# jizongFox/Self-paced-Contrastive-Learning

Hardware: AMD Instinct MI355X
Metric: pretrain slices/sec/node (UNet+InfoNCE, 224^2, bs=32/GPU) (higher is better)
Workload: dtype bf16; 1 GPU; BASELINE.json configs[1]: self-paced pretrain step, UNet base (max_channel=256) encoder to Conv5 + ProjectionHead(256,256,256) + SelfPacedSupConLoss(soft, partition labels, correct_grad) fwd+bwd + RAdam; slices_per_gpu=32, images_per_gpu_step=64, image=1x224x224, global_batch=32, parallelism=dp1, params=1311056, hipgraph=epocher, capture_steps=3

## Files before the change

include/spcl_hip.h:

```cpp
#ifndef SPCL_HIP_H
#define SPCL_HIP_H
#include <stddef.h>
#include <stdint.h>
#ifdef __cplusplus
extern "C" {
#endif

#define SPCL_F32 0
#define SPCL_BF16 1

#define SPCL_OK 0
#define SPCL_EINVAL (-1)
#define SPCL_ELAUNCH (-2)
#define SPCL_EUNSUPPORTED (-3)

#define SPCL_ABI_VERSION 24
int spcl_abi_version(void);
const char* spcl_last_error(void);

size_t spcl_supcon_workspace_bytes(int n, int d);
int spcl_supcon_forward(const float* z1, const float* z2, const float* labels, const float* mask, int n, int d,
                        float temperature, int sp_mode, float gamma, int correct_grad, float* ws, float* out,
                        void* stream);
int spcl_supcon_backward(const float* labels, const float* mask, int n, int d, float temperature, int sp_mode,
                         float gamma, const float* ws_fwd, float* ws_bwd, const float* out_fwd,
                         const float* grad_out, float* dz1, float* dz2, void* stream);
size_t spcl_supcon_bwd_workspace_bytes(int n, int d);
int spcl_supcon_unit_gradient_block(int n, int d, size_t* offset_floats, int* row_pitch);
int spcl_supcon_forward_heads(int K, const float* z1, const float* z2, size_t z_stride, const float* labels, int n,
                              int d, float temperature, int sp_mode, const float* gammas, int correct_grad, float* ws,
                              size_t ws_stride, float* out, void* stream);
int spcl_supcon_rows_supported(int n, int d);
int spcl_supcon_forward_rows(int K, const float* o1, const float* o2, size_t o_stride, const float* labels, int n, int d,
                             float temperature, int sp_mode, const float* gammas, int correct_grad, float* ws,
                             size_t ws_stride, float* out, void* stream);
int spcl_supcon_backward_heads(int K, const float* labels, int n, int d, float temperature, int sp_mode,
                               const float* gammas, const float* ws_fwd, size_t ws_stride, float* ws_bwd,
                               size_t wsb_stride, const float* out_fwd, const float* grad_out, float* dz1, float* dz2,
                               size_t z_stride, void* stream);
int spcl_supcon_materialize(const float* labels, const float* mask, int n, int d, float temperature, int sp_mode,
                            float gamma, const float* ws_fwd, float* sim_logits, float* sim_exp, float* pos_mask,
                            float* neg_mask, float* sp_mask, void* stream);

size_t spcl_supcon_xpos_workspace_bytes(int n, int d);
int spcl_supcon_xpos_forward(const float* z1, const float* z2, const float* labels, const float* mask, int n, int d,
                             float temperature, float* ws, float* out, void* stream);
int spcl_supcon_xpos_backward(const float* z1, const float* z2, int n, int d, float temperature, const float* ws,
                              const float* grad_out, float* dz1, float* dz2, void* stream);

size_t spcl_supcon_weighted_workspace_bytes(int n, int d);
int spcl_supcon_weighted_forward(const float* z1, const float* z2, const float* labels, const float* w11,
                                 const float* w22, const float* w12, int blocks, int mask_semantics, int in_mode, int n,
                                 int d, float temperature, float* ws, float* out, void* stream);
int spcl_supcon_weighted_backward(const float* z1, const float* z2, int n, int d, float temperature, float* ws,
                                  const float* grad_out, float* dz1, float* dz2, void* stream);
int spcl_supcon_weighted_materialize(const float* z1, const float* z2, const float* labels, const float* w11,
                                     const float* w22, const float* w12, int blocks, int mask_semantics, int n, int d,
                                     float temperature, float* ws, float* sim_logits, float* sim_exp, float* pos_weight,
                                     float* enable_mask, void* stream);

int spcl_proj_forward(const void* feat, int dtype, int N, int HW, int C, int Cs, const float* w1, const float* b1,
                      const float* w2, const float* b2, int hid, int out_dim, int normalize, float* pooled,
                      float* pre, float* o, float* z, void* stream);
int spcl_proj_backward(const float* dz, int dtype, int N, int HW, int C, int Cs, const float* w1, const float* w2,
                       int hid, int out_dim, int normalize, const float* pooled, const float* pre, const float* o,
                       float* dw1, float* db1, float* dw2, float* db2, float* scratch ,
                       void* dfeat, void* stream);

int spcl_proj_heads_forward(int K, const void* feat, int dtype, int N, int HW, int C, int Cs, const float* const* w1 ,
                            const float* const* b1 , const float* const* w2 , const float* const* b2 ,
                            int hid, int out_dim, int normalize, float* pooled, float* const* pre ,
                            float* const* o , float* const* z , void* stream);
int spcl_proj_heads_backward(int K, const float* const* dz , int dtype, int N, int HW, int C, int Cs,
                             const float* const* w1 , const float* const* w2 , int hid, int out_dim,
                             int normalize, const float* pooled, const float* const* pre ,
                             const float* const* o , float* const* dw1 , float* const* db1 ,
                             float* const* dw2 , float* const* db2 , float* scratch, void* dfeat, void* stream);
int spcl_proj_heads_backward_pooled(int K, const float* const* dz, int dtype, int N, int HW, int C, int Cs,
                                    const float* const* w1, const float* const* w2, int hid, int out_dim, int normalize,
                                    const float* pooled, const float* const* pre, const float* const* o, float* const* dw1,
                                    float* const* db1, float* const* dw2, float* const* db2, float* scratch, void* dfeat_nc,
                                    void* stream);


size_t spcl_conv_packed_elems(int Cin, int Cout, int kind, int dtype);
int spcl_conv_pack_weights(const float* w_oihw, int Cin, int Cout, int kind, int dtype, void* packed, void* stream);
int spcl_conv_pack_weights_both(const float* w_oihw, int Cin, int Cout, int dtype, void* packed_fwd,
                                void* packed_dgrad, void* stream);

int spcl_conv_pack_weights_block(const float* wa_oihw, int CinA, int CoutA, void* a_fwd, void* a_dgrad,
                                 const float* wb_oihw, int CinB, int CoutB, void* b_fwd, void* b_dgrad, int dtype,
                                 void* stream);
int spcl_conv_pack_weights_block_at(const float* wa_oihw, int CinA, int CoutA, void* a_fwd, void* a_dgrad,
                                    const float* wb_oihw, int CinB, int CoutB, void* b_fwd, void* b_dgrad, int dtype,
                                    int H, int W, void* stream);

#define SPCL_PACK_MULTI_MAX 24
typedef struct spcl_pack_item {
  const float* w_oihw;
// ... 72 lines not shown
size_t spcl_conv_wgrad_batched_workspace_bytes(const spcl_wgrad_item* items, int n);
int spcl_conv3x3_wgrad_batched(const spcl_wgrad_item* items, int n, int accumulate, float* partial, void* stream);

#define SPCL_WGRAD_TAILS_MAX 16
typedef struct spcl_wgrad_tail {
  const float* partial;
  float* dw;
  int kind;
  int nsplit, nblk_ci, nblk_co, CIB, COB, Cin, Cout;
} spcl_wgrad_tail;
int spcl_wgrad_tail_capture(spcl_wgrad_tail* slot);
int spcl_conv3x3_wgrad_batched_tails(const spcl_wgrad_item* items, int n, const spcl_wgrad_tail* tails, int ntails,
                                     int accumulate, float* partial, void* stream);
int spcl_bn_finalize(float* stats, int ntiles, int C, int CS, const float* gamma, const float* beta,
                     float momentum, float eps, float* running_mean, float* running_var,
                     int64_t* num_batches_tracked, float* mean, float* invstd, float* scale, float* shift,
                     void* stream);
int spcl_bn_eval_affine(int C, int CS, const float* gamma, const float* beta, const float* running_mean,
                        const float* running_var, float eps, float* mean, float* invstd, float* scale, float* shift,
                        void* stream);
#define SPCL_BN_EVAL_MAX 32
typedef struct {
  const float* gamma;
  const float* beta;
  const float* running_mean;
  const float* running_var;
  float* st;
  int C, CS;
  float eps;
} spcl_bn_eval_item;
int spcl_bn_eval_affine_multi(const spcl_bn_eval_item* items, int n, void* stream);

int spcl_bnrelu_pool_forward(const void* y, int dtype, int N, int H, int W, int CS, const float* scale,
                             const float* shift, void* act_out, void* pool_out, void* stream);
size_t spcl_bnrelu_bwd_workspace_bytes(int N, int H, int W, int CS);
int spcl_bnrelu_pool_backward(const void* y, const void* dact, const void* dpool, int dtype, int N, int H, int W,
                              int C, int CS, const float* mean, const float* invstd, const float* scale,
                              const float* shift, int training, float* ws, float* dgamma, float* dbeta, void* dy,
                              void* stream);
int spcl_bnrelu_up2_forward(const void* y, int dtype, int N, int H, int W, int CS, const float* scale, const float* shift,
                            void* up_out, void* stream);
int spcl_bnrelu_pool_forward_strided(const void* y, int dtype, int N, int H, int W, int CS, const float* scale,
                                     const float* shift, void* act_out, int act_stride, void* pool_out, void* stream);
int spcl_bnrelu_pool_backward_strided(const void* y, const void* dact, int dact_stride, const void* dpool, int dtype, int N,
                                      int H, int W, int C, int CS, const float* mean, const float* invstd,
                                      const float* scale, const float* shift, int training, float* ws, float* dgamma,
                                      float* dbeta, void* dy, void* stream);
int spcl_bnrelu_backward_up2(const void* y, const void* d_up, void* dact, int dtype, int N, int H, int W, int C, int CS,
                             const float* mean, const float* invstd, const float* scale, const float* shift, int training,
                             float* ws, float* dgamma, float* dbeta, void* dy, void* stream);
int spcl_bnrelu_backward_bcast(const void* y, const void* dact_nc, int dtype, int N, int H, int W, int C, int CS,
                               const float* mean, const float* invstd, const float* scale, const float* shift, int training,
                               float* ws, float* dgamma, float* dbeta, void* dy, void* stream);

size_t spcl_bnrelu_image_wgrad_workspace_bytes(int N, int H, int W, int CS);
int spcl_bnrelu_backward_image_wgrad(const void* y, const void* dact, const float* image, int dtype, int N, int H,
                                     int W, int C, int CS, const float* mean, const float* invstd, const float* scale,
                                     const float* shift, int training, float* ws, float* dgamma, float* dbeta,
                                     float* dw, void* stream);

int spcl_conv_dgrad_bnstats_supported(int dtype, int N, int H, int W, int CinK, int CoutS);
int spcl_conv3x3_dgrad_bnstats(const void* dy, int dtype, int N, int H, int W, int CinK, int CoutS, const void* w_packed,
                               void* g, const void* y2, const float* scale2, const float* shift2, const float* mean2,
                               float* rows2, void* stream);

int spcl_image_autocorr_rows(int N, int H, int W);
int spcl_image_autocorr(const float* image, int N, int H, int W, float* out, void* stream);
int spcl_conv_dgrad_bnstats_image_supported(int dtype, int N, int H, int W, int CinK, int CoutS);
int spcl_conv3x3_dgrad_bnstats_image(const void* dy, int dtype, int N, int H, int W, int CinK, int CoutS,
                                     const void* w_packed, void* g, const void* y2, const float* scale2,
                                     const float* shift2, const float* mean2, const float* image, float* rows11,
                                     void* stream);
int spcl_conv16_bwd_fused_supported(int dtype, int N, int H, int W, int CinK, int CoutS);
int spcl_conv16_bwd_fused_splits(int N, int H, int W);
int spcl_conv16_bwd_fused(const void* dy, int dtype, int N, int H, int W, const void* w_packed_dgrad, const void* y2,
                          const float* scale2, const float* shift2, const float* mean2, const float* image,
                          float* rows11, float* partial, float* dw_oihw, int Cin, int Cout, float* wg_rows,
                          const float* acorr, int nacorr, float* acorr16, void* stream);
int spcl_conv16_bwd_fused_image_supported(int dtype, int N, int H, int W, int CinK, int CoutS);
int spcl_conv16_bwd_fused_image(const void* dy, int dtype, int N, int H, int W, const void* w_packed_dgrad,
                                const void* w_packed_image, const float* scale2, const float* shift2, const float* mean2,
                                const float* image, float* rows11, float* partial, float* dw_oihw, int Cin, int Cout,
                                float* wg_rows, const float* acorr, int nacorr, float* acorr16, void* stream);
int spcl_bnrelu_backward_wgrows_image3(const float* wg_rows, int nwg, const float* acorr, int nacorr, const float* w_oihw,
                                       int N, int H, int W, int C, int CS, const float* mean, const float* invstd,
                                       const float* scale, int training, float* ws, float* dgamma, float* dbeta,
                                       float* dw, void* stream);
size_t spcl_bnrelu_image3_workspace_bytes(int CS);
int spcl_bnrelu_backward_rows_image3(const float* rows11, int nrows, const float* acorr, int nacorr, const float* w_oihw,
                                     int N, int H, int W, int C, int CS, const float* mean, const float* invstd,
                                     const float* scale, int training, float* ws, float* dgamma, float* dbeta, float* dw,
                                     void* stream);

int spcl_conv_dgrad_poolstats_supported(int dtype, int N, int H, int W, int CinK, int CoutS, int H2, int W2);
int spcl_conv3x3_dgrad_poolstats(const void* dy, int dtype, int N, int H, int W, int CinK, int CoutS, const void* w_packed,
                                 void* g, const void* y2, int H2, int W2, const float* scale2, const float* shift2,
                                 const float* mean2, float* rows2, void* stream);
int spcl_bnrelu_pool_backward_rows(const void* y, const void* dpool, const float* rows, int nrows, int dtype, int N, int H,
                                   int W, int C, int CS, const float* mean, const float* invstd, const float* scale,
                                   const float* shift, int training, float* ws, float* dgamma, float* dbeta, void* dy,
                                   void* stream);
int spcl_bnrelu_backward_rows(const void* y, const void* dact, const float* image, const float* rows, int nrows, int dtype,
                              int N, int H, int W, int C, int CS, const float* mean, const float* invstd,
                              const float* scale, const float* shift, int training, float* ws, float* dgamma,
                              float* dbeta, void* dy, float* dw, void* stream);


int spcl_conv1x1_forward(const void* x, int dtype, size_t npix, int C, int CS, int K, const float* w, const float* b,
                         float* out, void* stream);
size_t spcl_conv1x1_bwd_workspace_bytes(int C, int K);
int spcl_conv1x1_backward(const void* x, const float* dout, int dtype, size_t npix, int C, int CS, int K, const float* w,
                          void* dx, float* dw, float* db, float* ws, void* stream);
int spcl_conv1x1_forward_bn(const void* y, int dtype, size_t npix, int C, int CS, int K, const float* scale,
                            const float* shift, const float* w, const float* b, float* out, void* stream);
int spcl_conv1x1_bwd_rows(size_t npix);
int spcl_conv1x1_backward_bn(const void* y, const float* dout, int dtype, size_t npix, int C, int CS, int K,
                             const float* scale, const float* shift, const float* mean, const float* w, void* dact,
                             float* dw, float* db, float* ws, float* rows, void* stream);
int spcl_softmax_forward(const float* logits, size_t npix, int K, float* prob, void* stream);
int spcl_softmax_backward(const float* prob, const float* dprob, size_t npix, int K, float* dlogits, void* stream);
size_t spcl_kl_workspace_bytes(void);
int spcl_kl_div_forward(const float* prob, const float* target, size_t npix, int K, float eps, float* ws, float* loss,
                        void* stream);
int spcl_kl_div_backward(const float* prob, const float* target, size_t npix, int K, float eps, const float* grad_loss,
                         float* dprob, void* stream);
int spcl_sup_loss_forward(const float* logits, const int64_t* labels, int B, int per_sample, int K, float eps, float* ws,
                          float* loss, float* dlogits_unit, int64_t* inter_zeroed, int64_t* union_zeroed, void* stream);
int spcl_one_hot(const int64_t* labels, size_t npix, int K, float* out, void* stream);
int spcl_argmax_classes(const float* logits, size_t npix, int K, int64_t* out, void* stream);
int spcl_dice_counts(const int64_t* pred, const int64_t* target, int B, int per_sample, int C, int64_t* inter_zeroed,
                     int64_t* union_zeroed, void* stream);

size_t spcl_surface_workspace_bytes(int B, int H, int W, int n_report);
int spcl_surface_distances(const int64_t* pred, const int64_t* target, int B, int H, int W, int C, const int* report,
                           int n_report, double sy, double sx, double percentile, double* hd, double* mhd, double* asd,
                           uint8_t* empty, void* ws, size_t ws_bytes, void* stream);

size_t spcl_surface_3d_workspace_bytes(int V, int D, int H, int W, int n_report);
int spcl_surface_distances_3d(const int64_t* pred, const int64_t* target, int V, int D, int H, int W, int C, const int* report,
                              int n_report, double sz, double sy, double sx, double percentile, double* hd, double* mhd,
                              double* asd, uint8_t* empty, void* ws, size_t ws_bytes, void* stream);

int spcl_upsample2x_forward(const void* x, void* y, int dtype, int N, int H, int W, int CS, void* stream);
int spcl_upsample2x_backward(const void* dy, void* dx, int dtype, int N, int H, int W, int CS, void* stream);
int spcl_concat2_channels(const void* a, const void* b, void* out, int elem_size, size_t npix, int CA, int CB,
                          void* stream);
int spcl_split2_channels(const void* in, void* a, void* b, int elem_size, size_t npix, int CA, int CB, void* stream);

int spcl_radam_step(float* param, const float* grad, float* exp_avg, float* exp_avg_sq, size_t n, int64_t* step,
                    const float* lr, double beta1, double beta2, double eps, double weight_decay, float* coef,
                    void* stream);
int spcl_radam_step_scalars(float* param, const float* grad, float* exp_avg, float* exp_avg_sq, size_t n, int64_t* step,
                            const float* lr, double beta1, double beta2, double eps, double weight_decay, float* coef,
                            int k, const void* const* src, void* const* dst, const float* count, void* stream);
int spcl_radam_step_scaled(float* param, const float* grad, double grad_scale, float* exp_avg, float* exp_avg_sq, size_t n,
                           int64_t* step, const float* lr, double beta1, double beta2, double eps, double weight_decay,
                           float* coef, int k, const void* const* src, void* const* dst, const float* count, void* stream);
int spcl_radam_apply_staged(float* param, const float* grad, double grad_scale, float* exp_avg, float* exp_avg_sq, size_t n,
                            int64_t* step, const float* coef, double beta1, double beta2, double eps, double weight_decay,
                            int k, const void* const* src, void* const* dst, const float* count, void* stream);

int spcl_adam_step_scaled(float* param, const float* grad, double grad_scale, float* exp_avg, float* exp_avg_sq, size_t n,
                          int64_t* step, const float* lr, double beta1, double beta2, double eps, double weight_decay,
                          int decoupled, float* coef, int k, const void* const* src, void* const* dst, const float* count,
                          void* stream);
int spcl_adam_apply_staged(float* param, const float* grad, double grad_scale, float* exp_avg, float* exp_avg_sq, size_t n,
// ... 184 lines not shown
```

self-paced-contrastive-learning_amd/csrc/bn.hip:

```cpp
#include <mutex>
#include <type_traits>
#include "bn_acc.hpp"
#include "common.hpp"
#include "image_acorr.hpp"

namespace spcl {

typedef __attribute__((ext_vector_type(4))) uint32_t u32x4;
template <typename T> struct Chunk;
template <> struct Chunk<float> { static constexpr int EPC = 4; };
template <> struct Chunk<bf16_t> { static constexpr int EPC = 8; };

template <typename T> __device__ __forceinline__ void unpack(u32x4 raw, float* v);
template <> __device__ __forceinline__ void unpack<float>(u32x4 raw, float* v) {
#pragma unroll
  for (int e = 0; e < 4; ++e) v[e] = __uint_as_float(raw[e]);
}
template <> __device__ __forceinline__ void unpack<bf16_t>(u32x4 raw, float* v) {
#pragma unroll
  for (int e = 0; e < 4; ++e) {
    v[2 * e] = __uint_as_float(raw[e] << 16);
    v[2 * e + 1] = __uint_as_float(raw[e] & 0xffff0000u);
  }
}
template <typename T> __device__ __forceinline__ u32x4 pack(const float* v);
template <> __device__ __forceinline__ u32x4 pack<float>(const float* v) {
  return (u32x4){__float_as_uint(v[0]), __float_as_uint(v[1]), __float_as_uint(v[2]), __float_as_uint(v[3])};
}
template <> __device__ __forceinline__ u32x4 pack<bf16_t>(const float* v) {
  u32x4 o;
#pragma unroll
  for (int e = 0; e < 4; ++e) o[e] = (uint32_t)f32_to_bf16(v[2 * e]) | ((uint32_t)f32_to_bf16(v[2 * e + 1]) << 16);
  return o;
}

constexpr int BN_GROUP_TILES = 256;
constexpr int BN_DIRECT_TILES = 1024;
__host__ __device__ inline int bn_groups(int ntiles) {
  return ntiles <= BN_DIRECT_TILES ? 0 : (ntiles + BN_GROUP_TILES - 1) / BN_GROUP_TILES;
}

struct BnFinalArgs {
  const float* gamma;
  const float* beta;
  float momentum, eps;
  float* running_mean;
  float* running_var;
  int64_t* nbt;
  float* mean;
  float* invstd;
  float* scale;
  float* shift;
};

__device__ __forceinline__ void store_agent(double* p, double v) {
  __hip_atomic_store((unsigned long long*)p, __builtin_bit_cast(unsigned long long, v), __ATOMIC_RELAXED,
                     __HIP_MEMORY_SCOPE_AGENT);
}
__device__ __forceinline__ double load_agent(const double* p) {
  return __builtin_bit_cast(double, __hip_atomic_load((const unsigned long long*)p, __ATOMIC_RELAXED, __HIP_MEMORY_SCOPE_AGENT));
}

struct BnChan { float gamma, beta, rm, rv; };
__device__ __forceinline__ BnChan bn_prefetch_channel(int c, int C, const BnFinalArgs& f) {
  const int cc = c < C ? c : C - 1;
  const float* rm = f.running_mean != nullptr ? f.running_mean : f.gamma;
  const float* rv = f.running_var != nullptr ? f.running_var : f.gamma;
  BnChan ch;
  ch.gamma = f.gamma[cc];
  ch.beta = f.beta[cc];
  ch.rm = rm[cc];
  ch.rv = rv[cc];
  return ch;
}
__device__ __forceinline__ void bn_final_channel(int c, int C, double n, double s1, double s2, const BnFinalArgs& f,
                                                 const BnChan& ch);
__device__ __forceinline__ double shfl_xor_f64(double v, int m) {
  const unsigned long long u = __builtin_bit_cast(unsigned long long, v);
  const unsigned lo = (unsigned)__shfl_xor((int)(unsigned)u, m, 64), hi = (unsigned)__shfl_xor((int)(unsigned)(u >> 32), m, 64);
  return __builtin_bit_cast(double, ((unsigned long long)hi << 32) | lo);
}
template <int CW>
__device__ __forceinline__ void bn_fold_lanes(double& n, double& s1, double& s2, double (*red)[1024 / 64][CW]) {
  static_assert(CW == 16, "four row lanes per wave");
  const int c16 = threadIdx.x % CW, wave = threadIdx.x >> 6, nw = blockDim.x >> 6;
  n += shfl_xor_f64(n, 16); s1 += shfl_xor_f64(s1, 16); s2 += shfl_xor_f64(s2, 16);
  n += shfl_xor_f64(n, 32); s1 += shfl_xor_f64(s1, 32); s2 += shfl_xor_f64(s2, 32);
// ... 52 lines not shown
    if (threadIdx.x == 0) __hip_atomic_store(tickets + blockIdx.x, 0u, __ATOMIC_RELAXED, __HIP_MEMORY_SCOPE_AGENT);
    n = 0.0; s1 = 0.0; s2 = 0.0;
    for (int r = tl; r < (int)gridDim.y; r += TL) {
      const double* p = partial + (size_t)r * 3 * CS + c;
      n += load_agent(p); s1 += load_agent(p + CS); s2 += load_agent(p + 2 * CS);
    }
    __syncthreads();
    bn_fold_lanes<CW>(n, s1, s2, red);
    if (tl == 0) bn_final_channel(c, C, n, s1, s2, f, SPCL_BN_PREFETCH ? ch : bn_prefetch_channel(c, C, f));
    return;
  }
  if (tl != 0) return;
  if (!FINAL) {
    double* q = partial + (size_t)blockIdx.y * 3 * CS + c;
    q[0] = n; q[CS] = s1; q[2 * CS] = s2;
    return;
  }
  bn_final_channel(c, C, n, s1, s2, f, SPCL_BN_PREFETCH ? ch : bn_prefetch_channel(c, C, f));
}

__device__ __forceinline__ void bn_final_channel(int c, int C, double n, double s1, double s2, const BnFinalArgs& f,
                                                 const BnChan& ch) {
  if (c >= C) {
    f.mean[c] = 0.f; f.invstd[c] = 0.f; f.scale[c] = 0.f; f.shift[c] = 0.f;
    return;
  }
  const double mu = s1 / n;
  const double m2 = fmax(s2 - s1 * mu, 0.0);
  const double var = m2 / n;
  const float is = 1.0f / sqrtf((float)var + f.eps);
  const float sc = ch.gamma * is;
  f.mean[c] = (float)mu;
  f.invstd[c] = is;
  f.scale[c] = sc;
  f.shift[c] = ch.beta - (float)mu * sc;
  if (f.running_mean != nullptr) f.running_mean[c] = (1.f - f.momentum) * ch.rm + f.momentum * (float)mu;
  if (f.running_var != nullptr) {
    const double unbiased = n > 1.0 ? m2 / (n - 1.0) : var;
    f.running_var[c] = (1.f - f.momentum) * ch.rv + f.momentum * (float)unbiased;
  }
  if (f.nbt != nullptr && c == 0) f.nbt[0] += 1;
}

__global__ __launch_bounds__(256) void bn_eval_affine_kernel(int C, int CS, const float* __restrict__ gamma,
                                                             const float* __restrict__ beta,
                                                             const float* __restrict__ rm, const float* __restrict__ rv,
                                                             float eps, float* mean, float* invstd, float* scale,
                                                             float* shift) {
  const int c = blockIdx.x * blockDim.x + threadIdx.x;
  if (c >= CS) return;
  if (c >= C) { mean[c] = 0.f; invstd[c] = 0.f; scale[c] = 0.f; shift[c] = 0.f; return; }
  const float is = 1.0f / sqrtf(rv[c] + eps);
  const float sc = gamma[c] * is;
  mean[c] = rm[c];
  invstd[c] = is;
  scale[c] = sc;
  shift[c] = beta[c] - rm[c] * sc;
}

struct BnEvalItems {
  spcl_bn_eval_item it[SPCL_BN_EVAL_MAX];
  int blk_end[SPCL_BN_EVAL_MAX];
};
__global__ __launch_bounds__(256) void bn_eval_affine_multi_kernel(BnEvalItems p, int n) {
  int i = 0;
  for (int k = 0; k < n; ++k) i += (int)blockIdx.x >= p.blk_end[k] ? 1 : 0;
  if (i >= n) return;
  const spcl_bn_eval_item& q = p.it[i];
  const int c = ((int)blockIdx.x - (i > 0 ? p.blk_end[i - 1] : 0)) * 256 + threadIdx.x;
  if (c >= q.CS) return;
  float* mean = q.st;
  float* invstd = q.st + q.CS;
  float* scale = q.st + 2 * q.CS;
  float* shift = q.st + 3 * q.CS;
  if (c >= q.C) { mean[c] = 0.f; invstd[c] = 0.f; scale[c] = 0.f; shift[c] = 0.f; return; }
  const float is = 1.0f / sqrtf(q.running_var[c] + q.eps);
  const float sc = q.gamma[c] * is;
  mean[c] = q.running_mean[c];
  invstd[c] = is;
  scale[c] = sc;
  shift[c] = q.beta[c] - q.running_mean[c] * sc;
}

template <typename T> struct Word;
template <> struct Word<float> {
  static constexpr int EPW = 1;
  static __device__ __forceinline__ float get(uint32_t w, int) { return __uint_as_float(w); }
  static __device__ __forceinline__ uint32_t make(const float* v) { return __float_as_uint(v[0]); }
  static __device__ __forceinline__ uint32_t merge(const uint32_t* s) { return s[0]; }
};
template <> struct Word<bf16_t> {
  static constexpr int EPW = 2;
  static __device__ __forceinline__ float get(uint32_t w, int h) {
    return __uint_as_float(h ? (w & 0xffff0000u) : (w << 16));
  }
  static __device__ __forceinline__ uint32_t make(const float* v) {
    return (uint32_t)f32_to_bf16(v[0]) | ((uint32_t)f32_to_bf16(v[1]) << 16);
  }
  static __device__ __forceinline__ uint32_t merge(const uint32_t* s) { return (s[0] & 0x0000ffffu) | (s[1] & 0xffff0000u); }
};

template <int EPC> __device__ __forceinline__ void load_coef(float* dst, const float* src, int cc) {
#pragma unroll
  for (int e = 0; e < EPC; e += 4) *(f32x4*)&dst[e] = *(const f32x4*)(src + cc * EPC + e);
}

template <int EPC>
__device__ __forceinline__ void acc_coef_fwd(const BnAccFwd& bn, int cc, float* sc, float* sh) {
  __shared__ float cl[2][256];
  const int c = threadIdx.x;
  if (c < bn.CS) {
    BnAccFwdRaw raw;
    raw.load(bn, c);
    float a, b;
    bn_acc_fwd_channel(bn, raw, c, a, b, blockIdx.x == 0);
    cl[0][c] = a;
    cl[1][c] = b;
  }
  __syncthreads();
#pragma unroll
  for (int e = 0; e < EPC; ++e) {
    sc[e] = cl[0][cc * EPC + e];
    sh[e] = cl[1][cc * EPC + e];
  }
}
template <int EPC>
__device__ __forceinline__ void acc_coef_bwd(const BnAccBwd& bw, int cc, float* A, float* B) {
  __shared__ float cl[2][256];
  const int c = threadIdx.x;
  if (c < bw.CS) {
    BnAccBwdRaw raw;
    raw.load(bw, c);
    float a, b;
    bn_acc_bwd_channel(bw, raw, c, a, b, blockIdx.x == 0);
    cl[0][c] = a;
    cl[1][c] = b;
  }
  __syncthreads();
#pragma unroll
  for (int e = 0; e < EPC; ++e) {
    A[e] = cl[0][cc * EPC + e];
    B[e] = cl[1][cc * EPC + e];
  }
}

constexpr int STREAM_UNROLL = 2;
constexpr int IMG_WGRAD_WG = 2048;

template <typename T>
__global__ __launch_bounds__(256, 6) void bnrelu_fwd_lin_kernel(const T* __restrict__ y, size_t npix, int CS,
                                                             const float* __restrict__ scale,
                                                             const float* __restrict__ shift, T* __restrict__ act,
                                                             int AS ,
                                                             BnAccFwd bn = BnAccFwd{}) {
  constexpr int EPC = Chunk<T>::EPC, U = STREAM_UNROLL;
  const int CPC = CS / EPC, PL = 256 / CPC;
  const int cc = threadIdx.x % CPC, pl = threadIdx.x / CPC;
  float sc[EPC], sh[EPC];
  if (bn.acc != nullptr) acc_coef_fwd<EPC>(bn, cc, sc, sh);
  if (pl >= PL) return;
  if (bn.acc == nullptr) {
    load_coef<EPC>(sc, scale, cc);
    load_coef<EPC>(sh, shift, cc);
  }
  const size_t stride = (size_t)gridDim.x * PL;
  for (size_t p = (size_t)blockIdx.x * PL + pl; p < npix; p += U * stride) {
    u32x4 r[U];
#pragma unroll
    for (int u = 0; u < U; ++u)
      if (p + u * stride < npix) r[u] = *(const u32x4*)(y + (p + u * stride) * CS + cc * EPC);
#pragma unroll
    for (int u = 0; u < U; ++u) {
      if (p + u * stride >= npix) break;
      float v[EPC];
      unpack<T>(r[u], v);
#pragma unroll
      for (int e = 0; e < EPC; ++e) v[e] = fmaxf(fmaf(sc[e], v[e], sh[e]), 0.f);
      *(u32x4*)(act + (p + u * stride) * AS + cc * EPC) = pack<T>(v);
    }
  }
}

template <typename T>
// ... 461 lines not shown
    g += (k == best) ? dp : 0.f;
    dz[k] = z[k] > 0.f ? g : 0.f;
  }
}

#ifndef SPCL_BWD_POOL_MAXW
#define SPCL_BWD_POOL_MAXW 0
#endif
#if SPCL_BWD_POOL_MAXW
#define BWD_POOL_WPE __attribute__((amdgpu_waves_per_eu(3, SPCL_BWD_POOL_MAXW)))
#else
#define BWD_POOL_WPE
#endif
template <typename T, bool APPLY, bool FAST, bool ACC = false>
__global__ __launch_bounds__(256, 3) BWD_POOL_WPE void bnrelu_bwd_pool_kernel(const T* __restrict__ y, const T* __restrict__ dact,
                                                              const T* __restrict__ dpool, int N, int H, int W, int CS,
                                                              const float* __restrict__ mean,
                                                              const float* __restrict__ invstd,
                                                              const float* __restrict__ scale,
                                                              const float* __restrict__ shift,
                                                              const float* __restrict__ ab, float* __restrict__ partial,
                                                              T* __restrict__ dy, int GS = 0 ,
                                                              BnAccBwd bw = BnAccBwd{}) {
  constexpr int EPC = Chunk<T>::EPC, EPW = Word<T>::EPW;
  __shared__ float red[APPLY ? 1 : 256][2 * EPC + 1];
  const int CPC = CS / EPC, PL = 256 / CPC;
  const int cc = threadIdx.x % CPC, pl = threadIdx.x / CPC;
  const int PH = (H + 1) / 2, PW = (W + 1) / 2, OH = H / 2, OW = W / 2;
  const bool has_g = !FAST && dact != nullptr;
  float s1[EPC], s2[EPC];
#pragma unroll
  for (int e = 0; e < EPC; ++e) s1[e] = s2[e] = 0.f;
  float c0[EPC], c1[EPC];
  constexpr bool from_acc = APPLY && ACC;
  if (from_acc) acc_coef_bwd<EPC>(bw, cc, c0, c1);
  if (pl < PL) {
    float sc[EPC], sh[EPC];
    load_coef<EPC>(sc, scale, cc);
    load_coef<EPC>(sh, shift, cc);
    if (!from_acc) {
      load_coef<EPC>(c0, APPLY ? ab : mean, cc);
      load_coef<EPC>(c1, APPLY ? ab + CS : invstd, cc);
    }
    const int rows = N * PH;
    for (int r = blockIdx.x; r < rows; r += gridDim.x) {
      const int n = r / PH, oy = r - n * PH;
      const size_t row0 = (size_t)n * H + 2 * oy;
      for (int ox = pl; ox < PW; ox += PL) {
        Window<T> w;
        w.template load<FAST>(y, row0, oy, ox, H, W, CS, cc);
        u32x4 rg[4], rdp = {0u, 0u, 0u, 0u};
        if (has_g) {
          const size_t g00 = (row0 * W + 2 * ox) * GS + cc * EPC;
          const size_t goff[4] = {g00, g00 + GS, g00 + (size_t)W * GS, g00 + (size_t)W * GS + GS};
#pragma unroll
          for (int k = 0; k < 4; ++k) {
            rg[k] = (u32x4){0u, 0u, 0u, 0u};
            if (w.valid[k]) rg[k] = *(const u32x4*)(dact + goff[k]);
          }
        }
        const bool complete = FAST || (dpool != nullptr && oy < OH && ox < OW);
        if (complete) rdp = *(const u32x4*)(dpool + (((size_t)n * OH + oy) * OW + ox) * CS + cc * EPC);
        if (APPLY && FAST) __builtin_amdgcn_sched_barrier(0);
        u32x4 out[4];
#pragma unroll
        for (int wi = 0; wi < 4; ++wi) {
          float o[4][EPW];
#pragma unroll
          for (int h = 0; h < EPW; ++h) {
            const int e = wi * EPW + h;
            if (!APPLY && !has_g) {
              float zb = -1.f, yb = 0.f;
#pragma unroll
              for (int k = 0; k < 4; ++k) {
                const float yv = Word<T>::get(w.ry[k][wi], h);
                pool_first_max(k, w.valid[k] ? fmaf(sc[e], yv, sh[e]) : -1.f, yv, zb, yb);
              }
              const float dzb = (complete && zb > 0.f) ? Word<T>::get(rdp[wi], h) : 0.f;
              s1[e] += dzb;
              s2[e] = fmaf(dzb, yb - c0[e], s2[e]);
              continue;
            }
            if (APPLY && FAST) {
              float yk[4], z[4];
#pragma unroll
              for (int k = 0; k < 4; ++k) {
                yk[k] = Word<T>::get(w.ry[k][wi], h);
                z[k] = fmaf(sc[e], yk[k], sh[e]);
              }
              float m = fmaxf(z[0], 0.f);
              const bool s1 = z[1] > m;
              m = fmaxf(m, z[1]);
              const bool s2 = z[2] > m;
              m = fmaxf(m, z[2]);
              const bool s3 = z[3] > m;
              const bool b[4] = {z[0] > 0.f && !s1 && !s2 && !s3, s1 && !s2 && !s3, s2 && !s3, s3};
              const float dp = Word<T>::get(rdp[wi], h);
#pragma unroll
              for (int k = 0; k < 4; ++k) o[k][h] = fmaf(sc[e], b[k] ? dp : 0.f, fmaf(c0[e], yk[k], c1[e]));
              continue;
            }
            float yk[4], dz[4];
            window_dz<T>(w, rg, has_g, rdp, complete, wi, h, sc[e], sh[e], yk, dz);
#pragma unroll
            for (int k = 0; k < 4; ++k) {
              if (APPLY) o[k][h] = fmaf(sc[e], dz[k], fmaf(c0[e], yk[k], c1[e]));
              else {
                s1[e] += dz[k];
                s2[e] = fmaf(dz[k], yk[k] - c0[e], s2[e]);
              }
            }
          }
          if (APPLY) {
#pragma unroll
            for (int k = 0; k < 4; ++k) out[k][wi] = Word<T>::make(o[k]);
          }
        }
        if (APPLY) {
#pragma unroll
          for (int k = 0; k < 4; ++k)
            if (w.valid[k]) *(u32x4*)(dy + w.off[k]) = out[k];
        }
      }
    }
    if (!APPLY) {
#pragma unroll
      for (int e = 0; e < EPC; ++e) s2[e] *= bw.acc != nullptr ? 1.f : c1[e];
    }
  }
  if (!APPLY) wg_reduce_partials<T, EPC>(s1, s2, CS, CPC, PL, partial, red, const_cast<long long*>(bw.acc));
}

struct Image3Args {
  const float* acorr;
  int nacorr;
  const float* w_oihw;
  float* dw;
};
__device__ __forceinline__ int acorr_index(int a, int b) {
  return a * 9 - a * (a - 1) / 2 + (b - a);
}
__global__ __launch_bounds__(256) void bnrelu_bwd_fin_kernel(const float* __restrict__ partial, int nwg, int C, int CS,
                                                             float M, int training, const float* __restrict__ mean,
                                                             const float* __restrict__ invstd,
                                                             const float* __restrict__ scale,
                                                             float* __restrict__ dgamma, float* __restrict__ dbeta,
                                                             float* __restrict__ ab, float* __restrict__ zero_fill,
                                                             int nzero, int s2_centered, int rs, Image3Args im,
                                                             int transposed = 0) {
  __shared__ float red[11][4];
  __shared__ double racc4[4][64];
  __shared__ double racc[54];
  __shared__ float coef[2];
  const int c = blockIdx.x % CS, grp = blockIdx.x / CS;
  const bool split = gridDim.x == 3u * (unsigned)CS;
  const int t0 = split ? 3 * grp : 0, ntap = split ? 3 : 9;
  if (blockIdx.x == 0)
    for (int z = threadIdx.x; z < nzero; z += 256) zero_fill[z] = 0.f;
  const int lane = threadIdx.x & 63, wave = threadIdx.x >> 6;
  const float c_invstd = invstd[c], c_scale = scale[c], c_mean = mean[c];
  const bool img3 = im.acorr != nullptr;
  __shared__ float wsh[9];
  if (img3 && threadIdx.x < 9 && c < C)
    wsh[threadIdx.x] = bf16_to_f32(f32_to_bf16(im.w_oihw[c * 9 + threadIdx.x]));
  float s1 = 0.f, s2 = 0.f;
  float st[9];
#pragma unroll
  for (int t = 0; t < 9; ++t) st[t] = 0.f;
  auto walk = [&](auto ntap_c) {
    constexpr int NTAP = decltype(ntap_c)::value;
    if (transposed) {
#pragma unroll 4
      for (int w = threadIdx.x; w < nwg; w += 256) {
        s1 += partial[((size_t)0 * CS + c) * nwg + w];
        s2 += partial[((size_t)1 * CS + c) * nwg + w];
#pragma unroll
        for (int t = 0; t < NTAP; ++t) st[t] += partial[((size_t)(2 + t0 + t) * CS + c) * nwg + w];
      }
    } else {
#pragma unroll 4
      for (int w = threadIdx.x; w < nwg; w += 256) {
        s1 += partial[((size_t)w * rs + 0) * CS + c];
// ... 46 lines not shown
    coef[1] = B;
  }
  if (!img3) return;
  __syncthreads();
  __shared__ double wrp[9][9];
  if (threadIdx.x < 81) {
    const int t = threadIdx.x / 9, u = threadIdx.x - 9 * t;
    wrp[t][u] = (double)wsh[u] * racc[u <= t ? acorr_index(u, t) : acorr_index(t, u)];
  }
  __syncthreads();
  if ((int)threadIdx.x >= t0 && (int)threadIdx.x < t0 + ntap && c < C) {
    const int t = threadIdx.x;
    const double S1 = (double)((red[2 + t][0] + red[2 + t][1]) + (red[2 + t][2] + red[2 + t][3]));
    double wr = 0.0;
#pragma unroll
    for (int u = 0; u < 9; ++u) wr += wrp[t][u];
    im.dw[c * 9 + t] = (float)((double)c_scale * S1 + (double)coef[0] * wr + (double)coef[1] * racc[45 + t]);
  }
}

__global__ __launch_bounds__(256) void image_autocorr_kernel(const float* __restrict__ img, int H, int W,
                                                             float* __restrict__ out) {
  image_autocorr_body(img, H, W, out, blockIdx.x);
}

constexpr int ACORR_FOLD = 16;
__global__ __launch_bounds__(256) void bwd_rows_group_kernel(const float* __restrict__ rows, int nrows, int G, int CS,
                                                             float* __restrict__ out, int rs ,
                                                             int nwg = 0x7fffffff,
                                                             const float* __restrict__ acorr_in = nullptr,
                                                             int nacorr = 0, float* __restrict__ acorr_out = nullptr,
                                                             int transposed = 0) {
  if ((int)blockIdx.x >= nwg) {
    const int j = blockIdx.x - nwg, k = threadIdx.x;
    if (k < 64) {
      float s = 0.f;
#pragma unroll 8
      for (int w = j; w < nacorr; w += ACORR_FOLD) s += acorr_in[(size_t)w * 64 + k];
      acorr_out[(size_t)j * 64 + k] = s;
    }
    return;
  }
  const int w = blockIdx.x;
  for (int o = threadIdx.x; o < rs * CS; o += 256) {
    float s = 0.f;
#pragma unroll 8
    for (int k = 0; k < G; ++k) {
      const int r = w * G + k;
      if (r < nrows) s += rows[(size_t)r * rs * CS + o];
    }
    if (transposed) out[(size_t)o * (nwg == 0x7fffffff ? (int)gridDim.x : nwg) + w] = s;
    else out[(size_t)w * rs * CS + o] = s;
  }
}

__global__ __launch_bounds__(256) void bwd_rows_acc_kernel(const float* __restrict__ rows, int nrows, int G, int CS,
                                                           long long* __restrict__ acc) {
  __shared__ float part[256];
  const int w = blockIdx.x, NW4 = 4 * CS;
  const int NP = NW4 >= 256 ? 1 : 256 / NW4;
  for (int o0 = 0; o0 < NW4; o0 += 256) {
    const int o = o0 + (int)(threadIdx.x % (NW4 < 256 ? NW4 : 256)), p = NW4 < 256 ? (int)threadIdx.x / NW4 : 0;
    const int c = o >> 2, which = (o >> 1) & 1, limb = o & 1;
    float s = 0.f;
    if (o < NW4 && p < NP) {
#pragma unroll 8
      for (int k = p; k < G; k += NP) {
        const int r = w * G + k;
        if (r < nrows) s += rows[((size_t)r * 2 + which) * CS + c];
      }
    }
    if (NP > 1) {
      part[threadIdx.x] = s;
      __syncthreads();
      if (p == 0 && o < NW4) {
        for (int q = 1; q < NP; ++q) s += part[q * NW4 + o];
      }
      __syncthreads();
    }
    if (p == 0 && o < NW4) bn_acc_add_word(acc, CS, w & (BN_ACC_REPLICAS - 1), c, which, limb, s);
  }
}

template <typename T>
__global__ __launch_bounds__(256, 6) void bnrelu_bwd_apply_lin_kernel(const T* __restrict__ y, const T* __restrict__ g,
                                                                   size_t npix, int CS,
                                                                   const float* __restrict__ scale,
                                                                   const float* __restrict__ shift,
                                                                   const float* __restrict__ ab, T* __restrict__ dy,
                                                                   int GS, BnAccBwd bw = BnAccBwd{}) {
  constexpr int EPC = Chunk<T>::EPC, EPW = Word<T>::EPW, U = STREAM_UNROLL;
  const int CPC = CS / EPC, PL = 256 / CPC;
  const int cc = threadIdx.x % CPC, pl = threadIdx.x / CPC;
  float sc[EPC], sh[EPC], A[EPC], B[EPC];
  if (bw.acc != nullptr) acc_coef_bwd<EPC>(bw, cc, A, B);
  if (pl >= PL) return;
  load_coef<EPC>(sc, scale, cc);
  load_coef<EPC>(sh, shift, cc);
  if (bw.acc == nullptr) {
    load_coef<EPC>(A, ab, cc);
    load_coef<EPC>(B, ab + CS, cc);
  }
  const size_t stride = (size_t)gridDim.x * PL;
  for (size_t p = (size_t)blockIdx.x * PL + pl; p < npix; p += U * stride) {
    u32x4 ry[U], rg[U];
#pragma unroll
    for (int u = 0; u < U; ++u)
      if (p + u * stride < npix) {
        ry[u] = *(const u32x4*)(y + (p + u * stride) * CS + cc * EPC);
        rg[u] = *(const u32x4*)(g + (p + u * stride) * GS + cc * EPC);
      }
#pragma unroll
    for (int u = 0; u < U; ++u) {
      if (p + u * stride >= npix) break;
      u32x4 out;
#pragma unroll
      for (int wi = 0; wi < 4; ++wi) {
        float o[EPW];
#pragma unroll
        for (int h = 0; h < EPW; ++h) {
          const int e = wi * EPW + h;
          const float yv = Word<T>::get(ry[u][wi], h);
          const float dz = fmaf(sc[e], yv, sh[e]) > 0.f ? Word<T>::get(rg[u][wi], h) : 0.f;
          o[h] = fmaf(sc[e], dz, fmaf(A[e], yv, B[e]));
        }
        out[wi] = Word<T>::make(o);
      }
      *(u32x4*)(dy + (p + u * stride) * CS + cc * EPC) = out;
    }
  }
}

template <typename T> struct Quad;
template <> struct Quad<float> {
  typedef u32x4 raw_t;
  static __device__ __forceinline__ float get(raw_t r, int e) { return __uint_as_float(r[e]); }
};
template <> struct Quad<bf16_t> {
  typedef __attribute__((ext_vector_type(2))) uint32_t raw_t;
  static __device__ __forceinline__ float get(raw_t r, int e) {
    return __uint_as_float((e & 1) ? (r[e >> 1] & 0xffff0000u) : (r[e >> 1] << 16));
  }
};

template <typename T>
__global__ __launch_bounds__(256, 5) void bnrelu_bwd_image_wgrad_kernel(const T* __restrict__ y, const T* __restrict__ g,
                                                                     const float* __restrict__ img, int N, int H,
                                                                     int W, int CS, const float* __restrict__ scale,
                                                                     const float* __restrict__ shift,
                                                                     const float* __restrict__ ab,
                                                                     const float* __restrict__ zrow ,
                                                                     float* __restrict__ wpart ) {
  typedef typename Quad<T>::raw_t raw_t;
  constexpr int U = 2;
  extern __shared__ float redw[];
  const int QPP = CS / 4, PL = 256 / QPP;
  const int q = threadIdx.x % QPP, pl = threadIdx.x / QPP;
  float acc[9][4];
#pragma unroll
  for (int t = 0; t < 9; ++t)
#pragma unroll
    for (int e = 0; e < 4; ++e) acc[t][e] = 0.f;
  float sc[4], sh[4], A[4], B[4];
  load_coef<4>(sc, scale, q);
  load_coef<4>(sh, shift, q);
  load_coef<4>(A, ab, q);
// ... 144 lines not shown
}

enum class BwdWs { Plain, ImageWgrad, Image3 };
struct BwdWsLayout {
  size_t partial = 0, ab, wpart, zrow, afold, total;
  BwdWsLayout(BwdWs kind, int CS, int W = 0) {
    ab = (size_t)BWD_MAX_WG * (kind == BwdWs::Image3 ? 11 : 2) * CS;
    wpart = afold = ab + 2 * (size_t)CS;
    zrow = wpart + (size_t)IMG_WGRAD_WG * 9 * CS;
    total = kind == BwdWs::ImageWgrad ? zrow + (size_t)W : kind == BwdWs::Image3 ? afold + ACORR_FOLD * 64 : wpart;
  }
  size_t bytes() const { return total * sizeof(float); }
};

enum class BnGrad { Full, Pooled, PooledFull, PerImage, Up2 };
enum class BnSums { Reduce, Rows, Filled, Fill };
enum class BnOut { Dy, ImageWgrad };
struct BnBwdArgs {
  const void* y = nullptr;
  int N = 0, H = 0, W = 0, C = 0, CS = 0;
  BnGrad grad = BnGrad::Full;
  const void *dact = nullptr, *dpool = nullptr, *d_up = nullptr;
  int dact_stride = 0;
  BnSums sums = BnSums::Reduce;
  const float* rows = nullptr;
  int nrows = 0, training = 0;
  long long* acc = nullptr;
  float* ws = nullptr;
  const float *mean = nullptr, *invstd = nullptr, *scale = nullptr, *shift = nullptr;
  float *dgamma = nullptr, *dbeta = nullptr;
  BnOut out = BnOut::Dy;
  void* dy = nullptr;
  const float* img = nullptr;
  float* dw = nullptr;
  hipStream_t st = nullptr;

  static BnGrad arrives(const void* dact, const void* dpool) {
    return dpool == nullptr ? BnGrad::Full : dact == nullptr ? BnGrad::Pooled : BnGrad::PooledFull;
  }
  bool pooled() const { return grad == BnGrad::Pooled || grad == BnGrad::PooledFull; }
  bool whole_windows() const { return grad == BnGrad::Pooled && H % 2 == 0 && W % 2 == 0; }
  size_t npix() const { return (size_t)N * H * W; }
  int prows() const { return N * ((H + 1) / 2); }
  int gstride() const { return dact_stride > 0 ? dact_stride : CS; }
  int stream_wg() const { return acc != nullptr ? acc_stream_wg() : STREAM_MAX_WG; }
  double grad_tensors() const { return (grad != BnGrad::Pooled ? 1.0 : 0.0) + (pooled() ? 0.25 : 0.0); }
  BnAccBwd block() const {
    if (acc == nullptr) return BnAccBwd{};
    return BnAccBwd{acc, mean , dgamma, dbeta, (float)npix(), training, C, CS};
  }
};

struct BwdSums {
  const float* fin_src = nullptr;
  int nwg = 0, fin_transposed = 0;
  int bsplit = 1;
};

template <typename T, bool APPLY>
static void bnrelu_bwd_pool_launch(const BnBwdArgs& a, int grid, const float* ab, float* partial, const BnAccBwd& bw) {
  const bool fast = a.whole_windows();
  auto go = [&](auto FAST, auto ACC) {
    SPCL_LAUNCH((bnrelu_bwd_pool_kernel<T, APPLY, decltype(FAST)::value, decltype(ACC)::value>), dim3(grid), dim3(256), 0, a.st,
                (const T*)a.y, (const T*)a.dact, (const T*)a.dpool, a.N, a.H, a.W, a.CS, a.mean, a.invstd, a.scale, a.shift, ab,
                partial, APPLY ? (T*)a.dy : (T*)nullptr, fast ? 0 : a.gstride(), bw);
  };
  if constexpr (APPLY) {
    if (bw.acc != nullptr) return fast ? go(yes, yes) : go(no, yes);
  }
  fast ? go(yes, no) : go(no, no);
}

template <typename T>
static BwdSums bnrelu_bwd_sums(const BnBwdArgs& a, float* partial) {
  constexpr int rs = 2;
  const int PL = 256 / (a.CS / Chunk<T>::EPC);
  const double tb = (double)a.npix() * a.CS * sizeof(T);
  BwdSums s{partial};
  prof_cost(tb + tb * a.grad_tensors(), 0.0);
  if (a.sums == BnSums::Filled) return s;
  if (a.sums == BnSums::Rows) {
    static const int fin_rows = lab_env("SPCL_BWD_FIN_MAX_ROWS", BWD_MAX_WG);
    if (a.acc != nullptr) {
      const int G = (a.nrows + 511) / 512;
      s.nwg = (a.nrows + G - 1) / G;
      SPCL_LAUNCH(bwd_rows_acc_kernel, dim3(s.nwg), dim3(256), 0, a.st, a.rows, a.nrows, G, a.CS, a.acc);
    } else if (a.nrows <= fin_rows) {
      s.fin_src = a.rows;
      s.nwg = a.nrows;
    } else {
      const int G = (a.nrows + BWD_MAX_WG - 1) / BWD_MAX_WG;
      s.nwg = (a.nrows + G - 1) / G;
      SPCL_LAUNCH(bwd_rows_group_kernel, dim3(s.nwg), dim3(256), 0, a.st, a.rows, a.nrows, G, a.CS, partial, rs, s.nwg,
                  (const float*)nullptr, 0, (float*)nullptr, 1);
      s.fin_transposed = 1;
    }
    return s;
  }
  long long* const fill = a.sums == BnSums::Fill ? a.acc : nullptr;
  const int red_wg = fill != nullptr ? a.stream_wg() : BWD_MAX_WG;
  switch (a.grad) {
    case BnGrad::Pooled:
    case BnGrad::PooledFull:
      s.nwg = a.prows() < red_wg ? a.prows() : red_wg;
      bnrelu_bwd_pool_launch<T, false>(a, s.nwg, nullptr, partial, fill != nullptr ? a.block() : BnAccBwd{});
      break;
    case BnGrad::PerImage: {
      static const int env_split = lab_env("SPCL_BCAST_SPLIT_MAX", 4);
      s.bsplit = (a.H * a.W + PL - 1) / PL;
      if (env_split > 0 && s.bsplit > env_split) s.bsplit = env_split;
      while (s.bsplit > 1 && a.N * s.bsplit > BWD_MAX_WG) s.bsplit = (s.bsplit + 1) / 2;
      s.nwg = a.N * s.bsplit;
      prof_cost(tb, 0.0);
      SPCL_LAUNCH((bnrelu_bwd_reduce_bcast_kernel<T>), dim3(s.nwg), dim3(256), 0, a.st, (const T*)a.y, (const T*)a.dact,
                  a.H * a.W, a.CS, s.bsplit, a.mean, a.invstd, a.scale, a.shift, partial, fill);
      break;
    }
    case BnGrad::Up2:
      s.nwg = stream_grid(a.npix(), PL, STREAM_UNROLL, red_wg);
      prof_cost(tb * 6.0, 0.0);
      SPCL_LAUNCH((bnrelu_bwd_reduce_up2_kernel<T>), dim3(s.nwg), dim3(256), 0, a.st, (const T*)a.y, (const T*)a.d_up,
                  (T*)a.dact, a.npix(), a.W, a.CS, a.mean, a.invstd, a.scale, a.shift, partial, fill);
      break;
    case BnGrad::Full:
      s.nwg = stream_grid(a.npix(), PL, STREAM_UNROLL, red_wg);
      SPCL_LAUNCH((bnrelu_bwd_reduce_lin_kernel<T>), dim3(s.nwg), dim3(256), 0, a.st, (const T*)a.y, (const T*)a.dact, a.npix(),
                  a.CS, a.mean, a.invstd, a.scale, a.shift, partial, a.gstride(), fill);
      break;
  }
  return s;
}

static void bnrelu_bwd_finalize(const BnBwdArgs& a, const BwdSums& s, float* ab, float* zrow) {
  if (a.acc != nullptr) return;
  const bool image = a.out == BnOut::ImageWgrad;
  SPCL_LAUNCH(bnrelu_bwd_fin_kernel, dim3(a.CS), dim3(256), 0, a.st, s.fin_src, s.nwg, a.C, a.CS, (float)a.npix(), a.training,
              a.mean, a.invstd, a.scale, a.dgamma, a.dbeta, ab, image ? zrow : (float*)nullptr, image ? a.W : 0,
              a.sums == BnSums::Rows ? 1 : 0, 2, Image3Args{nullptr, 0, nullptr, nullptr}, s.fin_transposed);
}

template <typename T>
static void bnrelu_bwd_apply(const BnBwdArgs& a, const BwdSums& s, const float* ab, float* wpart, const float* zrow) {
  const int PL = 256 / (a.CS / Chunk<T>::EPC);
  const double tb = (double)a.npix() * a.CS * sizeof(T);
  const BnAccBwd bw = a.block();
  prof_cost(2.0 * tb + tb * a.grad_tensors(), 0.0);
  if (a.out == BnOut::ImageWgrad) {
    spcl_wgrad_tail* tail = take_tail_capture();
    static const int want = lab_env("SPCL_IMGWG_WG", 1280);
    const int cap = want < IMG_WGRAD_WG ? (want > 0 ? want : 1) : IMG_WGRAD_WG;
    const int g = a.N * a.H < cap ? a.N * a.H : cap;
    prof_cost(2.0 * tb + (double)a.npix() * 4, 2.0 * 9 * a.npix() * a.C);
    SPCL_LAUNCH((bnrelu_bwd_image_wgrad_kernel<T>), dim3(g), dim3(256), 4 * 9 * a.CS * sizeof(float), a.st, (const T*)a.y,
                (const T*)a.dact, a.img, a.N, a.H, a.W, a.CS, a.scale, a.shift, ab, zrow, wpart);
    if (tail != nullptr) {
      tail->partial = wpart; tail->dw = a.dw; tail->kind = 1; tail->nsplit = g; tail->nblk_ci = tail->nblk_co = 1;
      tail->CIB = 1; tail->COB = a.CS; tail->Cin = 1; tail->Cout = a.C;
    } else {
      SPCL_LAUNCH(image_wgrad_final_kernel, dim3(9), dim3(256), 0, a.st, (const float*)wpart, g, a.C, a.CS, a.dw);
    }
  } else if (a.pooled()) {
    bnrelu_bwd_pool_launch<T, true>(a, a.prows() < a.stream_wg() ? a.prows() : a.stream_wg(), ab, nullptr, bw);
  } else if (a.grad == BnGrad::PerImage) {
    prof_cost(2.0 * tb, 0.0);
    SPCL_LAUNCH((bnrelu_bwd_apply_bcast_kernel<T>), dim3(a.N * s.bsplit), dim3(256), 0, a.st, (const T*)a.y, (const T*)a.dact,
                a.H * a.W, a.CS, s.bsplit, a.scale, a.shift, ab, (T*)a.dy, bw);
  } else {
    SPCL_LAUNCH((bnrelu_bwd_apply_lin_kernel<T>), dim3(stream_grid(a.npix(), PL, STREAM_UNROLL, a.stream_wg())), dim3(256), 0,
                a.st, (const T*)a.y, (const T*)a.dact, a.npix(), a.CS, a.scale, a.shift, ab, (T*)a.dy, a.gstride(), bw);
// ... 443 lines not shown
```

self-paced-contrastive-learning_amd/csrc/bn_acc.hpp:

```cpp
#pragma once
#include "common.hpp"

namespace spcl {

#ifndef SPCL_ACC_REPLICAS
#define SPCL_ACC_REPLICAS 8
#endif
constexpr int BN_ACC_REPLICAS = SPCL_ACC_REPLICAS;
constexpr int BN_ACC_FLAG_WORDS = 4;
constexpr double BN_ACC_HI = 1024.0, BN_ACC_HI_INV = 1.0 / 1024.0;
constexpr double BN_ACC_LO = 1152921504606846976.0 , BN_ACC_LO_INV = 1.0 / 1152921504606846976.0;
constexpr float BN_ACC_MAX = 1099511627776.0f;
#ifndef SPCL_ACC_FWD_TILES
#define SPCL_ACC_FWD_TILES 4096
#endif
constexpr int BN_ACC_MAX_TILES_FWD = SPCL_ACC_FWD_TILES;
constexpr int BN_ACC_MAX_TILES_BWD = 4096;

__host__ __device__ inline size_t bn_acc_words(int CS) { return (size_t)BN_ACC_REPLICAS * CS * 4 + BN_ACC_FLAG_WORDS; }

struct BnAccFwd {
  const long long* acc;
  const float* gamma;
  const float* beta;
  float* running_mean;
  float* running_var;
  long long* nbt;
  float* st;
  float momentum, eps, count;
  int C, CS;
  double inv_count;
};

struct BnAccBwd {
  const long long* acc;
  const float* st;
  float* dgamma;
  float* dbeta;
  float count;
  int training, C, CS;
};

#ifdef __HIPCC__
__device__ __forceinline__ void bn_acc_atomic_add(long long* p, long long v) {
  (void)__hip_atomic_fetch_add(p, v, __ATOMIC_RELAXED, __HIP_MEMORY_SCOPE_AGENT);
}

__device__ __forceinline__ void bn_acc_split(float v, long long& hi, long long& lo, bool& ok) {
  ok = fabsf(v) < BN_ACC_MAX;
  const double d = ok ? (double)v : 0.0;
  const double h = rint(d * BN_ACC_HI);
  const double l = rint(fma(h, -BN_ACC_HI_INV, d) * BN_ACC_LO);
  hi = (long long)h;
  lo = (long long)l;
}

__device__ __forceinline__ void bn_acc_add_row16(long long* acc, int CS, int replica, int cb, int r16, f32x4 s1, f32x4 s2,
                                                 bool active = true) {
  const int q = r16 & 3, which = (r16 >> 2) & 1, limb = r16 >> 3;
  float v = which ? s2[0] : s1[0];
#pragma unroll
  for (int r = 1; r < 4; ++r) v = q == r ? (which ? s2[r] : s1[r]) : v;
  long long hi, lo;
  bool ok;
  bn_acc_split(v, hi, lo, ok);
  if (!active) return;
  long long* row = acc + ((size_t)replica * CS + cb + q) * 4;
  bn_acc_atomic_add(row + which * 2 + limb, limb ? lo : hi);
  if (!ok) bn_acc_atomic_add(acc + (size_t)BN_ACC_REPLICAS * CS * 4, 1);
}

__device__ __forceinline__ void bn_acc_add_word(long long* acc, int CS, int replica, int c, int which, int limb, float v) {
  long long hi, lo;
  bool ok;
  bn_acc_split(v, hi, lo, ok);
  bn_acc_atomic_add(acc + ((size_t)replica * CS + c) * 4 + which * 2 + limb, limb ? lo : hi);
  if (!ok) bn_acc_atomic_add(acc + (size_t)BN_ACC_REPLICAS * CS * 4, 1);
}

typedef __attribute__((ext_vector_type(2))) long long i64x2;
struct BnAccSums {
  long long h1, l1, h2, l2, flag;
  __device__ __forceinline__ void totals(double& t1, double& t2) const {
    t1 = fma((double)l1, BN_ACC_LO_INV, (double)h1 * BN_ACC_HI_INV);
    t2 = fma((double)l2, BN_ACC_LO_INV, (double)h2 * BN_ACC_HI_INV);
    if (flag != 0) t1 = t2 = __builtin_nan("");
  }
};
template <int RPT>
struct BnAccPart {
  i64x2 a[RPT], b[RPT];
  long long flag;
  __device__ __forceinline__ void load(const long long* acc, int CS, int c, int r0) {
#pragma unroll
    for (int r = 0; r < RPT; ++r) {
      const long long* row = acc + ((size_t)(r0 + r) * CS + c) * 4;
      a[r] = *(const i64x2*)row;
      b[r] = *(const i64x2*)(row + 2);
    }
    flag = acc[(size_t)BN_ACC_REPLICAS * CS * 4];
  }
  __device__ __forceinline__ BnAccSums sums() const {
    BnAccSums s{0, 0, 0, 0, flag};
#pragma unroll
    for (int r = 0; r < RPT; ++r) { s.h1 += a[r][0]; s.l1 += a[r][1]; s.h2 += b[r][0]; s.l2 += b[r][1]; }
    return s;
  }
};
typedef BnAccPart<BN_ACC_REPLICAS> BnAccRaw;

struct BnAccFwdParams {
  float g, b, rm, rv;
  __device__ __forceinline__ void load(const BnAccFwd& f, int c) {
    const int cc = c < f.C ? c : f.C - 1;
    g = f.gamma[cc];
    b = f.beta[cc];
    rm = (f.running_mean != nullptr ? f.running_mean : f.gamma)[cc];
    rv = (f.running_var != nullptr ? f.running_var : f.gamma)[cc];
  }
};
__device__ __forceinline__ void bn_acc_fwd_channel(const BnAccFwd& f, const BnAccSums& sums, const BnAccFwdParams& in, int c,
                                                   float& scale, float& shift, bool write) {
  if (c >= f.C) {
    scale = 0.f;
    shift = 0.f;
    if (write) { f.st[c] = 0.f; f.st[f.CS + c] = 0.f; f.st[2 * f.CS + c] = 0.f; f.st[3 * f.CS + c] = 0.f; }
// ... 74 lines not shown
```

self-paced-contrastive-learning_amd/csrc/conv16_bwd.hip:

```cpp
#include <stdio.h>
#include <stdlib.h>
#include <vector>
#include "conv_common.hpp"

namespace spcl {

struct Bwd16Args {
  const unsigned char* dy;
  const u32x4* wp;
  const unsigned char* y2;
  const u32x4* wp_img;
  const float* scale2;
  const float* shift2;
  const float* mean2;
  const float* img;
  float* rows11;
  float* wg_rows;
  int nwg;
  const float* acorr_in;
  int nacorr;
  float* acorr_out;
  float* partial;
  int N, H, W, tilesX, tilesY, ipw, xcd_remap;
  int dbg;
  unsigned long long* stamps;
};

constexpr int B16_TH = 14, B16_TW = 14, B16_HW = 16, B16_RP = 22, B16_PS = 32;
constexpr int B16_DY = 0, B16_DY_BYTES = (B16_TH + 2) * B16_RP * B16_PS;
constexpr int B16_IM = B16_DY_BYTES, B16_IM_BYTES = 1536;
constexpr int B16_XT = B16_IM + B16_IM_BYTES, B16_XT_ROW = 16 * 32, B16_XT_BYTES = B16_TH * B16_XT_ROW;
constexpr int B16_RED = B16_XT + B16_XT_BYTES;
constexpr int B16_ACC = B16_RED + 512;
constexpr int B16_TRASH = B16_ACC + 576;
constexpr int B16_LDS = B16_TRASH + 32;

#ifndef SPCL_CONV16_DBG_BUILD
#define SPCL_CONV16_DBG_BUILD 0
#endif
#define B16_DBG(a) (SPCL_CONV16_DBG_BUILD ? (a).dbg : 0)

__device__ __forceinline__ bf16x8 b16_tr_frag(unsigned addr) {
  const s16x4 lo = __builtin_amdgcn_ds_read_tr16_b64_v4i16((s16x4 __attribute__((address_space(3)))*)(uintptr_t)addr);
  const s16x4 hi =
      __builtin_amdgcn_ds_read_tr16_b64_v4i16((s16x4 __attribute__((address_space(3)))*)(uintptr_t)(addr + 8 * B16_PS));
  return __builtin_shufflevector(lo, hi, 0, 1, 2, 3, 4, 5, 6, 7);
}

__device__ __forceinline__ bf16x8 b16_tr_frag2(unsigned addr_lo, unsigned addr_hi) {
  const s16x4 lo = __builtin_amdgcn_ds_read_tr16_b64_v4i16((s16x4 __attribute__((address_space(3)))*)(uintptr_t)addr_lo);
  const s16x4 hi = __builtin_amdgcn_ds_read_tr16_b64_v4i16((s16x4 __attribute__((address_space(3)))*)(uintptr_t)addr_hi);
  return __builtin_shufflevector(lo, hi, 0, 1, 2, 3, 4, 5, 6, 7);
}

constexpr int b16_wpe(int NW) { return NW == 1 ? 2 : 3; }
template <bool SHIFTED, int NW, bool WGROWS>
__global__ __launch_bounds__(64 * NW) __attribute__((amdgpu_waves_per_eu(b16_wpe(NW)))) void conv16_bwd_kernel(Bwd16Args a) {
  constexpr int TH = B16_TH, TW = B16_TW, HW_ = B16_HW, RP = B16_RP, PS = B16_PS;
  constexpr int NPIX = TH * TW, NSTEPS = 5, NTHR = 64 * NW, ITER = 512 / NTHR, RPI = NTHR / 32;
  constexpr int MW = (13 + NW - 1) / NW, TPW = (9 + NW - 1) / NW;
  constexpr int SPX = (16 * NW) % TW, SPY = (16 * NW) / TW;
  extern __shared__ __attribute__((aligned(16))) unsigned char lds[];
  const unsigned lds_base = (unsigned)(uintptr_t)(unsigned char __attribute__((address_space(3)))*)lds;
  const int t0 = threadIdx.x;
  const int wave = NW == 1 ? 0 : __builtin_amdgcn_readfirstlane(t0 >> 6);
  if (WGROWS && (int)blockIdx.z * (int)(gridDim.x * gridDim.y) >= a.nwg) {
    const int nslice = gridDim.x * gridDim.y;
    if (t0 < 64) {
      for (int j = blockIdx.y * gridDim.x + blockIdx.x; j < 16; j += nslice) {
        float sacc = 0.f;
#pragma unroll 8
        for (int w = j; w < a.nacorr; w += 16) sacc += a.acorr_in[(size_t)w * 64 + t0];
        a.acorr_out[(size_t)j * 64 + t0] = sacc;
      }
    }
    return;
  }

  int tx = blockIdx.x, ty = blockIdx.y;
  {
    const int T = a.tilesX * a.tilesY;
    if (a.xcd_remap && (T & 7) == 0) {
      const int L = ty * a.tilesX + tx;
      const int L2 = (L & 7) * (T >> 3) + (L >> 3);
      ty = L2 / a.tilesX;
      tx = L2 - ty * a.tilesX;
    }
  }
  const int y0 = min(ty * TH, a.H - TH), x0 = min(tx * TW, a.W - TW);
  const int oy = ty * TH - y0, ox = tx * TW - x0;
  const bool interior = y0 > 0 && x0 > 0 && y0 + TH < a.H && x0 + TW < a.W;
  const bool shifted = SHIFTED && (oy | ox) != 0;
  const int rowb = 32;

  u32x4 wall[NSTEPS];
#pragma unroll
  for (int s = 0; s < NSTEPS; ++s) wall[s] = a.wp[s * 64 + (t0 & 63)];
  const f32x4 sc2 = *(const f32x4*)(a.scale2 + 4 * ((t0 & 63) >> 4)), sh2 = *(const f32x4*)(a.shift2 + 4 * ((t0 & 63) >> 4)),
              mu2 = *(const f32x4*)(a.mean2 + 4 * ((t0 & 63) >> 4));
  if (t0 < 4 * TH) *(u32x4*)(lds + B16_XT + (t0 >> 2) * B16_XT_ROW + TW * PS + (t0 & 3) * 16) = (u32x4){0u, 0u, 0u, 0u};
  if (t0 >= NTHR - 64)
    *(u32x4*)(lds + B16_DY + (((t0 & 63) >> 2) * RP + HW_) * PS + (t0 & 3) * 16) = (u32x4){0u, 0u, 0u, 0u};

  if (t0 < 48) {
    const int r = t0 & 15, k = t0 >> 4;
    ((bf16_t*)(lds + B16_IM))[(k == 0 ? 256 + 15 : (k == 1 ? 512 + 14 : 512 + 15)) + r * 16] = 0;
  }
  if (WGROWS)
// ... 245 lines not shown
    {
      int px = px0, py = py0;
#pragma unroll
      for (int j = 0; j < MW; ++j) {
        const bool ok = j < MW - 1 || 16 * (wave + NW * j) + r16 < NPIX;
        if (ok) *(uint2*)(lds + B16_XT + py * B16_XT_ROW + px * PS + g * 8) = dzp[j];
        px += SPX;
        py += SPY;
        if (px >= TW) {
          px -= TW;
          py += 1;
        }
      }
    }
    B16_STAMP(5)
    __syncthreads();
    B16_STAMP(1)
    if (wave == 0 && !(B16_DBG(a) & 8)) {
      const int tap = r16 < 9 ? r16 : 0, tky = tap / 3, tkx = tap - 3 * tky;
      const unsigned char* pb = lds + B16_IM + tkx * 512 + ((g >> 1) + tky) * 32 + (g & 1) * 8;
      f32x4* dp = (f32x4*)(lds + B16_ACC + (r16 * 16 + 4 * g) * 4);
      f32x4 D = (WGROWS && r16 < 9) ? *dp : (f32x4){0.f, 0.f, 0.f, 0.f};
#pragma unroll
      for (int ks = 0; ks < TH / 2; ++ks) {
        const bf16x8 af = b16_tr_frag(tr_x + ks * 2 * B16_XT_ROW);
        const uint2 b0 = *(const uint2*)(pb + ks * 64), b1 = *(const uint2*)(pb + ks * 64 + 16);
        const u32x4 bq = {b0.x, b0.y, b1.x, b1.y};
        D = __builtin_amdgcn_mfma_f32_16x16x32_bf16(af, __builtin_bit_cast(bf16x8, bq), D, 0, 0, 0);
      }
      if (WGROWS) {
        if (r16 < 9) *dp = D;
      } else if (r16 < 9) *(f32x4*)(a.rows11 + ((size_t)tile * 11 + 2 + r16) * 16 + 4 * g) = D;
    }
    B16_STAMP(6)
    if (NW > 1) __syncthreads();
  }

  if (stamp) {
    unsigned long long* o = a.stamps + ((size_t)(blockIdx.z * gridDim.y + blockIdx.y) * gridDim.x + blockIdx.x) * 8;
#pragma unroll
    for (int k = 0; k < 7; ++k) o[k] = tph[k];
  }
  const size_t wg = (size_t)(blockIdx.z * gridDim.y + blockIdx.y) * gridDim.x + blockIdx.x;
  if (WGROWS) {
    __syncthreads();
    for (int i = t0; i < 11 * 16; i += NTHR) {
      float tot;
      if (i < 32) {
        const float* red = (const float*)(lds + B16_RED) + i;
        tot = red[0];
#pragma unroll
        for (int w = 1; w < NW; ++w) tot += red[32 * w];
      } else {
        tot = ((const float*)(lds + B16_ACC))[i - 32];
      }
      a.wg_rows[(size_t)i * a.nwg + wg] = tot;
    }
  }
  float* out = a.partial + wg * (9 * 256);
#pragma unroll
  for (int j = 0; j < TPW; ++j) {
    const int tap = wave + NW * j;
    if (tap < 9) {
#pragma unroll
      for (int r = 0; r < 4; ++r) out[(tap * 16 + 4 * ((t0 & 63) >> 4) + r) * 16 + (t0 & 15)] = wacc[j][r];
    }
  }
}


#ifndef SPCL_CONV16_ROWS_WPE
#define SPCL_CONV16_ROWS_WPE 4
#endif
constexpr int r16_wpe(bool shifted) { return shifted && SPCL_CONV16_ROWS_WPE > 3 ? 3 : SPCL_CONV16_ROWS_WPE; }
constexpr int R16_RP = 18;
constexpr int R16_DY = 0, R16_DY_BYTES = (B16_TH + 2) * R16_RP * B16_PS;
constexpr int R16_IM = R16_DY_BYTES;
constexpr int R16_XT = R16_IM + B16_IM_BYTES;
constexpr int R16_RED = R16_XT + B16_XT_BYTES;
constexpr int R16_ACC = R16_RED + 512;
constexpr int R16_TRASH = R16_ACC + 576;
constexpr int R16_TAB = R16_TRASH + 32;
constexpr int B16_LDS_ROWS = R16_TAB + 128;

template <bool SHIFTED, bool WGROWS, bool RECOMP = false>
__global__ __launch_bounds__(128) __attribute__((amdgpu_waves_per_eu(r16_wpe(SHIFTED)))) void conv16_bwd_rows_kernel(Bwd16Args a) {
  static_assert(!(RECOMP && SHIFTED), "y2 from the image: whole 14 x 14 tiles");
  constexpr int NW = 2;
  constexpr int TH = B16_TH, TW = B16_TW, HW_ = B16_HW, RP = R16_RP, PS = B16_PS;
  constexpr int NSTEPS = 5, NTHR = 64 * NW, ITER = 512 / NTHR, RPI = NTHR / 32;
  constexpr int MW = TH / NW, TPW = (9 + NW - 1) / NW;
  static_assert(TH % NW == 0, "rows are dealt to the waves evenly");
  extern __shared__ __attribute__((aligned(16))) unsigned char lds[];
  const unsigned lds_base = (unsigned)(uintptr_t)(unsigned char __attribute__((address_space(3)))*)lds;
  const int t0 = threadIdx.x;
  const int wave = __builtin_amdgcn_readfirstlane(t0 >> 6);
  if (WGROWS && (int)blockIdx.z * (int)(gridDim.x * gridDim.y) >= a.nwg) {
    const int nslice = gridDim.x * gridDim.y;
    float* fold = (float*)lds;
    const int cq = t0 & 15, rl = t0 >> 4;
    for (int j = blockIdx.y * gridDim.x + blockIdx.x; j < 16; j += nslice) {
      f32x4 sacc = {0.f, 0.f, 0.f, 0.f};
#pragma unroll 16
      for (int w = j + 16 * rl; w < a.nacorr; w += 128) sacc += *(const f32x4*)(a.acorr_in + (size_t)w * 64 + 4 * cq);
      __syncthreads();
      *(f32x4*)(fold + rl * 64 + 4 * cq) = sacc;
      __syncthreads();
      if (t0 < 64) {
        float tot = fold[t0];
#pragma unroll
        for (int r = 1; r < 8; ++r) tot += fold[r * 64 + t0];
        a.acorr_out[(size_t)j * 64 + t0] = tot;
      }
    }
    return;
  }

  int tx = blockIdx.x, ty = blockIdx.y;
  {
    const int T = a.tilesX * a.tilesY;
    if (a.xcd_remap && (T & 7) == 0) {
      const int L = ty * a.tilesX + tx;
      const int L2 = (L & 7) * (T >> 3) + (L >> 3);
      ty = L2 / a.tilesX;
      tx = L2 - ty * a.tilesX;
    }
  }
  const int y0 = min(ty * TH, a.H - TH), x0 = min(tx * TW, a.W - TW);
  const int oy = ty * TH - y0, ox = tx * TW - x0;
  const bool interior = y0 > 0 && x0 > 0 && y0 + TH < a.H && x0 + TW < a.W;
  const bool shifted = SHIFTED && (oy | ox) != 0;

  if (t0 < 4 * TH) *(u32x4*)(lds + R16_XT + (t0 >> 2) * B16_XT_ROW + TW * PS + (t0 & 3) * 16) = (u32x4){0u, 0u, 0u, 0u};
  if (t0 >= NTHR - 64)
    *(u32x4*)(lds + R16_DY + (((t0 & 63) >> 2) * RP + HW_) * PS + (t0 & 3) * 16) = (u32x4){0u, 0u, 0u, 0u};
  if (t0 < 48) {
    const int r = t0 & 15, k = t0 >> 4;
    ((bf16_t*)(lds + R16_IM))[(k == 0 ? 256 + 15 : (k == 1 ? 512 + 14 : 512 + 15)) + r * 16] = 0;
  }
  if (t0 >= 64 && t0 < 64 + 20) {
    const int e = t0 - 64, gq = e / NSTEPS, s = e - gq * NSTEPS;
    int fc = 4 * s + gq;
    if (fc >= 18) fc = 0;
    const int tap = fc >> 1, c = fc & 1, ky = (tap * 11) >> 5, kx = tap - 3 * ky;
    ((unsigned*)(lds + R16_TAB))[gq * 8 + s] = (unsigned)((ky * RP + kx) * PS + c * 16);
  }
  if (WGROWS)
    for (int i = t0; i < (512 + 576) / 4; i += NTHR) ((float*)(lds + R16_RED))[i] = 0.f;
  f32x4 wacc[TPW];
#pragma unroll
  for (int j = 0; j < TPW; ++j) wacc[j] = (f32x4){0.f, 0.f, 0.f, 0.f};

  float imgv[256 / NTHR];
  u32x4 v[ITER];
  uint2 ypre[RECOMP ? 1 : MW];
  constexpr int PPT = 256 / NTHR;
  short wraw[3] = {0, 0, 0};
  if (RECOMP) {
    const int gq = min((t0 & 63) >> 4, 2);
    const bf16_t* wq = (const bf16_t*)a.wp_img;
#pragma unroll
    for (int kx = 0; kx < 3; ++kx) {
      const int tap = 3 * gq + kx;
      wraw[kx] = (short)wq[(size_t)(((tap >> 1) * 64) + (2 * (tap & 1)) * 16 + (t0 & 15)) * 8];
    }
  }
  auto rsrc = [](const void* p) { return __builtin_amdgcn_make_buffer_rsrc((void*)p, 0, 0x7fffffff, 0x00020000); };
  constexpr int OOB = (int)0x80000000u;
  auto issue_img = [&](const int n) {
    int t = t0;
    asm volatile("" : "+v"(t));
    const int hr = (t * PPT) >> 4, hc = (t * PPT) & 15;
    const int gy = y0 - 1 + hr;
    const __amdgpu_buffer_rsrc_t rs = rsrc(a.img + (size_t)n * a.H * a.W);
    const int rowo = (gy < 0 ? 0 : (gy >= a.H ? a.H - 1 : gy)) * a.W;
#pragma unroll
    for (int e = 0; e < PPT; ++e) {
      const int gx = x0 - 1 + hc + e;
      imgv[e] = __builtin_bit_cast(float, __builtin_amdgcn_raw_buffer_load_b32(rs, (rowo + (gx < 0 ? 0 : (gx >= a.W ? a.W - 1 : gx))) * 4, 0, 0));
    }
  };
  auto issue_halo = [&](const int n) {
    int t = t0;
    asm volatile("" : "+v"(t));
    const int ch = t & 1, q0 = t >> 1, hy0 = q0 / HW_, hx0 = q0 % HW_;
    const int voff = (hy0 * a.W + hx0) * 32 + ch * 16;
    const __amdgpu_buffer_rsrc_t rs = rsrc(a.dy + (((long)n * a.H + (y0 - 1)) * a.W + (x0 - 1)) * 32);
#pragma unroll
    for (int k = 0; k < ITER; ++k) {
      bool inb = true;
      if (!interior) {
        const int gy = y0 - 1 + hy0 + RPI * k, gx = x0 - 1 + hx0;
        inb = gy >= 0 && gy < a.H && gx >= 0 && gx < a.W;
      }
      v[k] = __builtin_bit_cast(u32x4, __builtin_amdgcn_raw_buffer_load_b128(rs, inb ? voff : OOB, RPI * k * a.W * 32, 0));
    }
  };
  auto issue_y2 = [&](const int n) {
    int t = t0;
    asm volatile("" : "+v"(t));
    const int r16 = t & 15, g = (t & 63) >> 4;
    const int voff = min(r16, TW - 1) * 32 + g * 8;
    const __amdgpu_buffer_rsrc_t rs = rsrc(a.y2 + (((size_t)n * a.H + y0 + wave) * a.W + x0) * 32);
#pragma unroll
    for (int j = 0; j < MW; ++j)
      ypre[j] = __builtin_bit_cast(uint2, __builtin_amdgcn_raw_buffer_load_b64(rs, voff, NW * j * a.W * 32, 0));
  };
  const __amdgpu_buffer_rsrc_t rs_wp = rsrc(a.wp), rs_sc = rsrc(a.scale2), rs_sh = rsrc(a.shift2), rs_mu = rsrc(a.mean2);

  const bool stamp = SPCL_CONV16_STAMPS_BUILD && a.stamps != nullptr && t0 == 0;
  unsigned long long tph[7] = {0, 0, 0, 0, 0, 0, 0}, tc = 0;
  const int n_first = blockIdx.z * a.ipw;
  if (stamp) tc = __builtin_amdgcn_s_memtime();
  if (n_first < a.N) {
    issue_img(n_first);
    issue_halo(n_first);
    if (!RECOMP) issue_y2(n_first);
  }
  uint2 wfp = {0u, 0u};
  if (RECOMP) {
    const bool real = ((t0 & 63) >> 4) < 3;
    wfp.x = real ? ((uint32_t)(unsigned short)wraw[0] | ((uint32_t)(unsigned short)wraw[1] << 16)) : 0u;
    wfp.y = real ? (uint32_t)(unsigned short)wraw[2] : 0u;
    asm volatile("" : "+v"(wfp.x), "+v"(wfp.y));
  }
  __syncthreads();
  uint2 dzp[MW];
  auto second_half = [&](const int n) {
    int t = t0;
    asm volatile("" : "+v"(t));
    const int lane = t & 63, r16 = t & 15, g = lane >> 4;
    const int tile = (n * a.tilesY + ty) * a.tilesX + tx;
    const unsigned xaddr = (unsigned)(R16_XT + wave * B16_XT_ROW + r16 * PS + (((g + (r16 >> 2)) & 3) << 3));
    B16_STAMP(3)
    __syncthreads();
    B16_STAMP(1)
    if (!WGROWS && t < 32) {
      const float* red = (const float*)(lds + R16_RED) + t;
      float tot = red[0];
#pragma unroll
      for (int w = 1; w < NW; ++w) tot += red[32 * w];
      a.rows11[(size_t)tile * 11 * 16 + t] = tot;
    }

    const unsigned tr_col = (unsigned)((4 * (g & 1) + (r16 >> 2)) * PS + (r16 & 3) * 8);
    const unsigned tr_x = lds_base + R16_XT + (g >> 1) * B16_XT_ROW + (4 * (g & 1) + (r16 >> 2)) * PS + ((((r16 & 3) + (g & 1)) & 3) << 3);
    const unsigned tr_xh = (tr_x + 8 * PS) ^ 16u;
    {
      unsigned ad[TPW];
#pragma unroll
      for (int j = 0; j < TPW; ++j) {
        const int tap = min(wave + NW * j, 8), ky = tap / 3, kx = tap - 3 * ky;
        ad[j] = lds_base + R16_DY + (g >> 1) * RP * PS + tr_col + (2 - ky) * RP * PS + (2 - kx) * PS;
      }
#pragma unroll
      for (int ks = 0; ks < TH / 2; ++ks) {
        const bf16x8 af = b16_tr_frag2(tr_x + ks * 2 * B16_XT_ROW, tr_xh + ks * 2 * B16_XT_ROW);
#pragma unroll
        for (int j = 0; j < TPW; ++j) {
          const bf16x8 bf = b16_tr_frag(ad[j] + ks * 2 * RP * PS);
          wacc[j] = __builtin_amdgcn_mfma_f32_16x16x32_bf16(af, bf, wacc[j], 0, 0, 0);
        }
        __builtin_amdgcn_sched_barrier(0);
      }
    }
    B16_STAMP(4)
    __syncthreads();
    B16_STAMP(1)

#pragma unroll
    for (int j = 0; j < MW; ++j) *(uint2*)(lds + xaddr + j * (NW * B16_XT_ROW)) = dzp[j];
    B16_STAMP(5)
    __syncthreads();
    B16_STAMP(1)
    if (wave == 0) {
      const int tap = r16 < 9 ? r16 : 0, tky = tap / 3, tkx = tap - 3 * tky;
      const unsigned char* pb = lds + R16_IM + tkx * 512 + ((g >> 1) + tky) * 32 + (g & 1) * 8;
      f32x4* dp = (f32x4*)(lds + R16_ACC + (r16 * 16 + 4 * g) * 4);
      f32x4 D = (WGROWS && r16 < 9) ? *dp : (f32x4){0.f, 0.f, 0.f, 0.f};
#pragma unroll
      for (int ks = 0; ks < TH / 2; ++ks) {
        const bf16x8 af = b16_tr_frag2(tr_x + ks * 2 * B16_XT_ROW, tr_xh + ks * 2 * B16_XT_ROW);
        const uint2 b0 = *(const uint2*)(pb + ks * 64), b1 = *(const uint2*)(pb + ks * 64 + 16);
        const u32x4 bq = {b0.x, b0.y, b1.x, b1.y};
        D = __builtin_amdgcn_mfma_f32_16x16x32_bf16(af, __builtin_bit_cast(bf16x8, bq), D, 0, 0, 0);
      }
      if (WGROWS) {
        if (r16 < 9) *dp = D;
      } else if (r16 < 9) *(f32x4*)(a.rows11 + ((size_t)tile * 11 + 2 + r16) * 16 + 4 * g) = D;
    }
    B16_STAMP(6)
    __syncthreads();
  };
  int n = n_first;
  if (n_first < a.N)
#pragma unroll 1
  for (int it = 0;; ++it, ++n) {
    int t = t0;
    asm volatile("" : "+v"(t));
    const int lane = t & 63, r16 = t & 15, g = lane >> 4;
    u32x4 wall[NSTEPS];
#pragma unroll
    for (int s = 0; s < NSTEPS; ++s)
      wall[s] = __builtin_bit_cast(u32x4, __builtin_amdgcn_raw_buffer_load_b128(rs_wp, lane * 16, s * 1024, 0));
    f32x4 sc2 = __builtin_bit_cast(f32x4, __builtin_amdgcn_raw_buffer_load_b128(rs_sc, g * 16, 0, 0));
    f32x4 sh2 = __builtin_bit_cast(f32x4, __builtin_amdgcn_raw_buffer_load_b128(rs_sh, g * 16, 0, 0));
    const f32x4 mu2 = __builtin_bit_cast(f32x4, __builtin_amdgcn_raw_buffer_load_b128(rs_mu, g * 16, 0, 0));
    if (r16 >= TW || (SHIFTED && r16 < ox)) {
      sc2 = (f32x4){0.f, 0.f, 0.f, 0.f};
      sh2 = (f32x4){-1.f, -1.f, -1.f, -1.f};
    }
    const u32x4 tabA = *(const u32x4*)(lds + R16_TAB + g * 32);
    const unsigned tabB = *(const unsigned*)(lds + R16_TAB + g * 32 + 16);
    {
      const int hr = (t * PPT) >> 4, hc = (t * PPT) & 15;
      const int gy = y0 - 1 + hr;
#pragma unroll
      for (int e = 0; e < PPT; ++e) {
        const int gx = x0 - 1 + hc + e;
        const float hv = (interior || (gy >= 0 && gy < a.H && gx >= 0 && gx < a.W)) ? imgv[e] : 0.f;
        const bf16_t hb = f32_to_bf16(hv);
        bf16_t* imb = (bf16_t*)(lds + R16_IM) + hr * 16 + hc + e;
        imb[0] = hb;
        if (hc + e >= 1) imb[256 - 1] = hb;
        if (hc + e >= 2) imb[512 - 2] = hb;
      }
    }
    {
      const int ch = t & 1, q0 = t >> 1, hy0 = q0 / HW_, hx0 = q0 % HW_;
      unsigned char* const lp = lds + R16_DY + (hy0 * RP + hx0) * PS + ch * 16;
#pragma unroll
      for (int k = 0; k < ITER; ++k) *(u32x4*)(lp + (RPI * k * RP) * PS) = v[k];
    }
    B16_STAMP(0)
    __syncthreads();
    B16_STAMP(1)

    f32x4 ssum = {0.f, 0.f, 0.f, 0.f}, ssq = {0.f, 0.f, 0.f, 0.f};
    const unsigned xaddr = (unsigned)(R16_XT + wave * B16_XT_ROW + r16 * PS + (((g + (r16 >> 2)) & 3) << 3));
    const int pc = min(r16, TW - 1);
    const unsigned yaddr = (unsigned)(R16_IM + (pc & 1) * 512 + ((g < 3 ? g : 0) + wave) * 32 + (pc & ~1) * 2);
    {
      const unsigned lb = (unsigned)(R16_DY + (wave * RP + r16) * PS);
      const unsigned offs[NSTEPS] = {tabA[0] + lb, tabA[1] + lb, tabA[2] + lb, tabA[3] + lb, tabB + lb};
#pragma unroll
      for (int j = 0; j < MW; ++j) {
        f32x4 acc = {0.f, 0.f, 0.f, 0.f};
#pragma unroll
        for (int s = 0; s < NSTEPS; ++s) {
          const u32x4 xf = *(const u32x4*)(lds + offs[s] + j * (NW * RP * PS));
          acc = mfma_chunk<bf16_t>(wall[s], xf, acc);
        }
        const bool keep_y = !shifted || wave + NW * j >= oy;
        uint2 yr;
        if (RECOMP) {
          const uint2 xv = {*(const uint32_t*)(lds + yaddr + j * (NW * 32)), *(const uint32_t*)(lds + yaddr + j * (NW * 32) + 4)};
          const f32x4 y = __builtin_amdgcn_mfma_f32_16x16x16bf16_1k(__builtin_bit_cast(s16x4, wfp), __builtin_bit_cast(s16x4, xv),
                                                                    (f32x4){0.f, 0.f, 0.f, 0.f}, 0, 0, 0);
          const f32x2 ylo = {y[0], y[1]}, yhi = {y[2], y[3]};
          yr.x = __builtin_bit_cast(uint32_t, __builtin_convertvector(ylo, bf16x2v));
          yr.y = __builtin_bit_cast(uint32_t, __builtin_convertvector(yhi, bf16x2v));
        } else {
          yr = ypre[j];
        }
        const float yv[4] = {__uint_as_float(yr.x << 16), __uint_as_float(yr.x & 0xffff0000u),
                             __uint_as_float(yr.y << 16), __uint_as_float(yr.y & 0xffff0000u)};
        const f32x2 glo = {acc[0], acc[1]}, ghi = {acc[2], acc[3]};
        const uint32_t g0 = __builtin_bit_cast(uint32_t, __builtin_convertvector(glo, bf16x2v));
        const uint32_t g1 = __builtin_bit_cast(uint32_t, __builtin_convertvector(ghi, bf16x2v));
        const float gv[4] = {__uint_as_float(g0 << 16), __uint_as_float(g0 & 0xffff0000u),
                             __uint_as_float(g1 << 16), __uint_as_float(g1 & 0xffff0000u)};
        float xv[4], dz[4];
#pragma unroll
        for (int r = 0; r < 4; ++r) {
          float z = fmaf(sc2[r], yv[r], sh2[r]);
          if (SHIFTED) z = keep_y ? z : -1.f;
          xv[r] = z;
          dz[r] = z > 0.f ? gv[r] : 0.f;
          ssum[r] += dz[r];
          ssq[r] = fmaf(dz[r], yv[r] - mu2[r], ssq[r]);
        }
        const f32x2 lo = {xv[0], xv[1]}, hi = {xv[2], xv[3]};
        uint2 w;
        w.x = relu_bf16x2(__builtin_bit_cast(uint32_t, __builtin_convertvector(lo, bf16x2v)));
        w.y = relu_bf16x2(__builtin_bit_cast(uint32_t, __builtin_convertvector(hi, bf16x2v)));
        *(uint2*)(lds + xaddr + j * (NW * B16_XT_ROW)) = w;
        dzp[j].x = (__float_as_uint(dz[0]) >> 16) | (__float_as_uint(dz[1]) & 0xffff0000u);
        dzp[j].y = (__float_as_uint(dz[2]) >> 16) | (__float_as_uint(dz[3]) & 0xffff0000u);
        asm volatile("" : "+v"(dzp[j].x), "+v"(dzp[j].y));
        __builtin_amdgcn_sched_barrier(0);
      }
    }
    B16_STAMP(2)
    {
      f32x4 o;
#pragma unroll
      for (int r = 0; r < 4; ++r) {
        const float s1 = row16_sum(ssum[r]), s2 = row16_sum(ssq[r]);
        o[r] = r16 == 0 ? s1 : s2;
      }
      if (r16 < 2) {
        f32x4* rp = (f32x4*)(lds + R16_RED + ((wave * 2 + r16) * 16 + 4 * g) * 4);
        *rp = WGROWS ? *rp + o : o;
      }
    }
    if (!(it + 1 < a.ipw && n + 1 < a.N)) break;
    issue_halo(n + 1);
    if (!RECOMP) issue_y2(n + 1);
    issue_img(n + 1);
    second_half(n);
  }
  if (n_first < a.N) second_half(n);

  if (stamp) {
    unsigned long long* o = a.stamps + ((size_t)(blockIdx.z * gridDim.y + blockIdx.y) * gridDim.x + blockIdx.x) * 8;
#pragma unroll
    for (int k = 0; k < 7; ++k) o[k] = tph[k];
  }
  const size_t wg = (size_t)(blockIdx.z * gridDim.y + blockIdx.y) * gridDim.x + blockIdx.x;
  if (WGROWS) {
    __syncthreads();
    for (int i = t0; i < 11 * 16; i += NTHR) {
      float tot;
      if (i < 32) {
        const float* red = (const float*)(lds + R16_RED) + i;
        tot = red[0];
#pragma unroll
        for (int w = 1; w < NW; ++w) tot += red[32 * w];
      } else {
        tot = ((const float*)(lds + R16_ACC))[i - 32];
      }
      a.wg_rows[(size_t)i * a.nwg + wg] = tot;
    }
  }
  float* out = a.partial + wg * (9 * 256);
#pragma unroll
  for (int j = 0; j < TPW; ++j) {
    const int tap = wave + NW * j;
    if (tap < 9) {
#pragma unroll
      for (int r = 0; r < 4; ++r) out[(tap * 16 + 4 * ((t0 & 63) >> 4) + r) * 16 + (t0 & 15)] = wacc[j][r];
    }
  }
}

int conv16_bwd_rowmap() {
  static const int env = lab_env("SPCL_CONV16_ROWMAP", 1);
  return env;
}

int conv16_bwd_nw() {
  static const int env = lab_env("SPCL_CONV16_NW", 2);
  return env == 1 || env == 4 ? env : 2;
}

int conv16_bwd_ipw(int N, int H, int W) {
  const int nw = conv16_bwd_nw();
  const int resident = 256 * (nw == 1 ? 8 : (nw == 2 ? (conv16_bwd_rowmap() ? 2 * SPCL_CONV16_ROWS_WPE : 6) : 3));
  const long tiles = (long)cdiv(H, B16_TH) * cdiv(W, B16_TW);
  static const int env_ipw = lab_env("SPCL_CONV16_IPW", 0);
  int ipw = env_ipw > 0 ? env_ipw : (int)((tiles * N + resident - 1) / resident);
  if (ipw < 1) ipw = 1;
  if (ipw > N) ipw = N;
  return ipw;
}

}

using namespace spcl;

extern "C" int spcl_conv16_bwd_fused_supported(int dtype, int N, int H, int W, int CinK, int CoutS) {
  static const bool off = lab_flag("SPCL_NO_CONV16_FUSED");
  if (off || CinK != 16 || CoutS != 16) return 0;
  return spcl_conv_dgrad_bnstats_image_supported(dtype, N, H, W, CinK, CoutS);
}

extern "C" int spcl_conv16_bwd_fused_splits(int N, int H, int W) {
  if (N <= 0 || H < B16_TH || W < B16_TW) return 0;
  const int ipw = conv16_bwd_ipw(N, H, W);
  return cdiv(H, B16_TH) * cdiv(W, B16_TW) * cdiv(N, ipw);
}

static int conv16_bwd_fused_impl(const void* dy, int dtype, int N, int H, int W, const void* w_packed_dgrad,
                                 const void* y2, const void* w_packed_image, const float* scale2, const float* shift2,
                                 const float* mean2, const float* image, float* rows11, float* partial, float* dw_oihw,
                                 int Cin, int Cout, float* wg_rows, const float* acorr, int nacorr, float* acorr16,
                                 void* stream) {
  SPCL_CHECK_ARG(dy && w_packed_dgrad && (y2 || w_packed_image) && scale2 && shift2 && mean2 && image && partial && dw_oihw,
                 "conv16_bwd_fused: null pointer");
  SPCL_CHECK_ARG((rows11 != nullptr) != (wg_rows != nullptr), "conv16_bwd_fused: exactly one of rows11 / wg_rows");
  SPCL_CHECK_ARG(wg_rows == nullptr || (acorr && acorr16 && nacorr > 0), "conv16_bwd_fused: wg_rows comes with the autocorrelation rows");
  SPCL_CHECK_ARG(Cin > 0 && Cin <= 16 && Cout > 0 && Cout <= 16, "conv16_bwd_fused: channel counts");
  if (y2 == nullptr) {
    if (!spcl_block1_kernels_take(dtype, N, H, W, 1, 16)) {
      set_error("conv16_bwd_fused_image: unsupported configuration (bf16, 16 -> 16 channels, H and W multiples of 14)");
      return SPCL_EUNSUPPORTED;
    }
  } else if (!spcl_conv16_bwd_fused_supported(dtype, N, H, W, 16, 16) &&
             !spcl_block1_kernels_take(dtype, N, H, W, 1, 16)) {
    set_error("conv16_bwd_fused: unsupported configuration (bf16, 16 -> 16 channels, 14 x 14 tiles)");
    return SPCL_EUNSUPPORTED;
  }
  hipStream_t st = (hipStream_t)stream;
  spcl_wgrad_tail* tail = take_tail_capture();
  Bwd16Args a;
  a.dy = (const unsigned char*)dy; a.wp = (const u32x4*)w_packed_dgrad; a.y2 = (const unsigned char*)y2;
  a.wp_img = (const u32x4*)w_packed_image;
  a.scale2 = scale2; a.shift2 = shift2; a.mean2 = mean2; a.img = image; a.rows11 = rows11; a.partial = partial;
  a.wg_rows = wg_rows; a.acorr_in = acorr; a.nacorr = nacorr; a.acorr_out = acorr16;
  a.N = N; a.H = H; a.W = W; a.tilesX = cdiv(W, B16_TW); a.tilesY = cdiv(H, B16_TH);
  a.ipw = conv16_bwd_ipw(N, H, W);
  static const int env_remap = lab_env("SPCL_CONV_XCD_REMAP", 1);
  a.xcd_remap = env_remap;
  a.dbg = lab_env("SPCL_CONV16_DBG", 0);
  const int nz = cdiv(N, a.ipw), nsplit = a.tilesX * a.tilesY * nz;
  a.nwg = nsplit;
  const double px = (double)N * H * W;
  prof_cost(px * 32.0 * (y2 != nullptr ? 2.0 : 1.0) + px * 4.0 + (double)nsplit * 9 * 256 * 4.0, 2.0 * px * 9.0 * 256 * 2.0 + 2.0 * px * 9.0 * 16);
  a.stamps = nullptr;
  const bool want_stamps = SPCL_CONV16_STAMPS_BUILD && lab_flag("SPCL_CONV16_STAMPS");
  const size_t nwg = (size_t)nsplit;
  if (want_stamps) {
    (void)hipMalloc(&a.stamps, nwg * 8 * sizeof(unsigned long long));
    (void)hipMemset(a.stamps, 0, nwg * 8 * sizeof(unsigned long long));
  }
  const int nw = conv16_bwd_nw();
  const bool even = H % B16_TH == 0 && W % B16_TW == 0, wgr = wg_rows != nullptr;
  const dim3 grid(a.tilesX, a.tilesY, nz + (wgr ? 1 : 0));
#define B16_LAUNCH(SH_, NW_, WG_) SPCL_LAUNCH((conv16_bwd_kernel<SH_, NW_, WG_>), grid, dim3(64 * NW_), B16_LDS, st, a)
#define B16_CASE(NW_)                                       \
  if (nw == NW_) {                                          \
    if (even && wgr) B16_LAUNCH(false, NW_, true);          \
    else if (even) B16_LAUNCH(false, NW_, false);           \
    else if (wgr) B16_LAUNCH(true, NW_, true);              \
    else B16_LAUNCH(true, NW_, false);                      \
  }
  if (y2 == nullptr) {
    if (wgr) SPCL_LAUNCH((conv16_bwd_rows_kernel<false, true, true>), grid, dim3(128), B16_LDS_ROWS, st, a);
    else SPCL_LAUNCH((conv16_bwd_rows_kernel<false, false, true>), grid, dim3(128), B16_LDS_ROWS, st, a);
  } else if (nw == 2 && conv16_bwd_rowmap()) {
#define B16_ROWS(SH_, WG_) SPCL_LAUNCH((conv16_bwd_rows_kernel<SH_, WG_>), grid, dim3(128), B16_LDS_ROWS, st, a)
    if (even && wgr) B16_ROWS(false, true);
    else if (even) B16_ROWS(false, false);
    else if (wgr) B16_ROWS(true, true);
    else B16_ROWS(true, false);
#undef B16_ROWS
  }
#if SPCL_LAB
  else if (y2 != nullptr) {
    B16_CASE(1) B16_CASE(2) B16_CASE(4)
  }
#endif
#undef B16_CASE
#undef B16_LAUNCH
  if (a.stamps != nullptr) {
    std::vector<unsigned long long> h(nwg * 8);
    (void)hipStreamSynchronize(st);
    (void)hipMemcpy(h.data(), a.stamps, h.size() * 8, hipMemcpyDeviceToHost);
    (void)hipFree(a.stamps);
    double ph[7] = {0, 0, 0, 0, 0, 0, 0};
    for (size_t i = 0; i < nwg; ++i)
      for (int k = 0; k < 7; ++k) ph[k] += (double)h[i * 8 + k];
    fprintf(stderr, "[conv16_bwd stamps] %zu workgroups x %d tiles | s_memtime ticks of wave 0 per TILE: staging %.0f, barriers %.0f, "
            "dgrad %.0f, pixel pass %.0f, wgrad %.0f, dz stores %.0f, tap sums %.0f\n", nwg, a.ipw, ph[0] / nwg / a.ipw,
            ph[1] / nwg / a.ipw, ph[2] / nwg / a.ipw, ph[3] / nwg / a.ipw, ph[4] / nwg / a.ipw, ph[5] / nwg / a.ipw,
            ph[6] / nwg / a.ipw);
  }
  if (tail != nullptr) {
    tail->partial = partial; tail->dw = dw_oihw; tail->kind = 0; tail->nsplit = nsplit; tail->nblk_ci = 1;
    tail->nblk_co = 1; tail->CIB = 16; tail->COB = 16; tail->Cin = Cin; tail->Cout = Cout;
  } else {
    launch_wgrad_reduce(partial, nsplit, 1, 1, 16, 16, Cin, Cout, dw_oihw, st);
  }
  SPCL_LAUNCH_CHECK("conv16_bwd_fused");
  return SPCL_OK;
}

extern "C" int spcl_conv16_bwd_fused(const void* dy, int dtype, int N, int H, int W, const void* w_packed_dgrad,
                                     const void* y2, const float* scale2, const float* shift2, const float* mean2,
                                     const float* image, float* rows11, float* partial, float* dw_oihw, int Cin, int Cout,
                                     float* wg_rows, const float* acorr, int nacorr, float* acorr16, void* stream) {
  SPCL_CHECK_ARG(y2 != nullptr, "conv16_bwd_fused: null pointer");
  return conv16_bwd_fused_impl(dy, dtype, N, H, W, w_packed_dgrad, y2, nullptr, scale2, shift2, mean2, image, rows11, partial,
                               dw_oihw, Cin, Cout, wg_rows, acorr, nacorr, acorr16, stream);
}

extern "C" int spcl_conv16_bwd_fused_image_supported(int dtype, int N, int H, int W, int CinK, int CoutS) {
  return (dtype == SPCL_BF16 && CinK == 16 && CoutS == 16 && N > 0 && H >= B16_TH && W >= B16_TW && H % B16_TH == 0 &&
          W % B16_TW == 0 && conv16_bwd_nw() == 2 && conv16_bwd_rowmap() && (double)H * W * 32.0 < 2147483648.0)
             ? 1 : 0;
}

extern "C" int spcl_conv16_bwd_fused_image(const void* dy, int dtype, int N, int H, int W, const void* w_packed_dgrad,
                                           const void* w_packed_image, const float* scale2, const float* shift2,
                                           const float* mean2, const float* image, float* rows11, float* partial,
                                           float* dw_oihw, int Cin, int Cout, float* wg_rows, const float* acorr, int nacorr,
                                           float* acorr16, void* stream) {
  SPCL_CHECK_ARG(w_packed_image != nullptr, "conv16_bwd_fused_image: null pointer");
  return conv16_bwd_fused_impl(dy, dtype, N, H, W, w_packed_dgrad, nullptr, w_packed_image, scale2, shift2, mean2, image, rows11,
                               partial, dw_oihw, Cin, Cout, wg_rows, acorr, nacorr, acorr16, stream);
}
```

self-paced-contrastive-learning_amd/functional.py:

```python
from __future__ import annotations

import ctypes
import math
import os
from ctypes import c_double, c_float, c_int

import torch

from . import native as _n

SP_NONE, SP_HARD, SP_SOFT = 0, 1, 2


def take_grad_sink(param, needed: bool = True):
    if not needed or param is None:
        return None
    sink = getattr(param, "_grad_sink", None)
    if sink is None or not getattr(param, "_grad_sink_armed", False):
        return None
    if sink.shape != param.shape or sink.dtype != torch.float32 or not sink.is_contiguous() or sink.device != param.device:
        return None
    param._grad_sink_armed = False
    return sink

# ... 875 lines not shown
    _PREPACKED_ACORR.clear()
    _EVAL_AFFINE.clear()


def prepare_eval_affines(bns):
    _EVAL_AFFINE.clear()
    bns = [bn for bn in bns if bn.running_mean is not None and bn.running_mean.is_cuda and bn.weight is not None]
    for i in range(0, len(bns), _n.BN_EVAL_MAX):
        part = bns[i:i + _n.BN_EVAL_MAX]
        dev = part[0].running_mean.device
        sizes = [_ru16(bn.num_features) for bn in part]
        buf = torch.empty(4 * sum(sizes), dtype=torch.float32, device=dev)
        items, keep, off = [], [], 0
        for bn, cs in zip(part, sizes):
            g, b = bn.weight.detach().contiguous().float(), bn.bias.detach().contiguous().float()
            st = buf[off:off + 4 * cs].view(4, cs)
            off += 4 * cs
            items.append(_n.BnEvalItem(g.data_ptr(), b.data_ptr(), bn.running_mean.data_ptr(), bn.running_var.data_ptr(),
                                       st.data_ptr(), bn.num_features, cs, float(bn.eps)))
            keep.append((g, b))
            _EVAL_AFFINE[(bn.running_mean.data_ptr(), cs)] = st
        arr = (_n.BnEvalItem * len(items))(*items)
        _n.call("spcl_bn_eval_affine_multi", arr, len(items), _n.stream())


def prepack_weights(layers, dtype, image=None):
    _PREPACKED.clear()
    _PREPACKED_ACORR.clear()
    if not _PREPACK or not layers:
        return
    dtc = _n.dtype_code(dtype)
    dev = layers[0][0].device
    sizes = []
    for w, H, W in layers:
        co, ci = w.shape[0], w.shape[1]
        sizes.append((_n.call("spcl_conv_packed_elems", ci, co, 0, dtc), _n.call("spcl_conv_packed_elems", ci, co, 1, dtc)))
    for i in range(0, len(layers), _n.PACK_MULTI_MAX):
        part, psz = layers[i:i + _n.PACK_MULTI_MAX], sizes[i:i + _n.PACK_MULTI_MAX]
        buf = torch.empty(sum(a + b for a, b in psz), dtype=dtype, device=dev)
        items, keep, off = [], [], 0
        for (w, H, W), (n0, n1) in zip(part, psz):
            wc = w.detach().contiguous().float()
            p0, p1 = buf[off:off + n0], buf[off + n0:off + n0 + n1]
            off += n0 + n1
            items.append(_n.PackItem(wc.data_ptr(), p0.data_ptr(), p1.data_ptr(), w.shape[1], w.shape[0],
                                     int(H) if _PACK_AT else 0, int(W) if _PACK_AT else 0))
            keep.append(wc)
            _PREPACKED[(w.data_ptr(), w._version, dtc, int(H), int(W))] = (p0, p1)
        arr = (_n.PackItem * len(items))(*items)
        if image is not None and i == 0 and _acorr_in_conv_rows(dtc, *[int(v) for v in image.shape[:3]]) > 0:
            image = None
        zero = _acc_arena_take_dirty(dev) if i == 0 else None
        zbytes = ctypes.c_size_t(zero.numel() * 8 if zero is not None else 0)
        if image is not None and i == 0:
            N, H, W = int(image.shape[0]), int(image.shape[1]), int(image.shape[2])
            acorr = torch.empty(_n.call("spcl_image_autocorr_rows", N, H, W), 64, dtype=torch.float32, device=dev)
            _n.call("spcl_conv_pack_weights_multi_zero", arr, len(items), dtc, _n.ptr(image), N, H, W, _n.ptr(acorr),
                    _n.ptr(zero), zbytes, _n.stream())
            _PREPACKED_ACORR[(image.data_ptr(), image._version)] = acorr
        else:
            _n.call("spcl_conv_pack_weights_multi_zero", arr, len(items), dtc, None, 0, 0, 0, None, _n.ptr(zero), zbytes,
                    _n.stream())


def _acorr_in_conv_rows(dt_code, N, H, W, cin=1, cout_s=16):
    return _n.call("spcl_conv3x3_forward_image_acorr_rows", dt_code, N, H, W, cin, cout_s)


def _conv_image_acorr(x_store, dt_code, dtype, N, H, W, cin_s, cout_s, wp, want_stats, rows, store=True):
    dev = x_store.device
    y = torch.empty(N, H, W, cout_s, dtype=dtype, device=dev) if store else None
    stats = None
    if want_stats:
        nt = _n.call("spcl_conv_stat_rows", dt_code, N, H, W, 16, cout_s)
        stats = torch.empty(_n.call("spcl_bn_stats_elems", nt, cout_s), dtype=torch.float32, device=dev)
        stats.ntiles = nt
    acorr = torch.empty(rows, 64, dtype=torch.float32, device=dev)
    _n.call("spcl_conv3x3_forward_image_acorr", _n.ptr(x_store), dt_code, N, H, W, cin_s, cout_s, _n.ptr(wp), _n.ptr(y),
            _n.ptr(stats), _n.ptr(acorr), _n.stream())
    return y, stats, acorr


_BLOCK1_RECOMPUTE = os.environ.get("SPCL_BLOCK1_RECOMPUTE", "1") != "0"


def _conv_from_image(image, y_image, dt_code, dtype, N, H, W, cout_s, wp_image, scale, shift, wp, want_stats):
    dev = image.device
    y = torch.empty(N, H, W, cout_s, dtype=dtype, device=dev)
    stats = None
    if want_stats:
        nt = N * (H // 14) * (W // 14)
        stats = torch.empty(_n.call("spcl_bn_stats_elems", nt, cout_s), dtype=torch.float32, device=dev)
        stats.ntiles = nt
    _n.call("spcl_conv3x3_forward_from_image", _n.ptr(image), _n.ptr(y_image), dt_code, N, H, W, cout_s, _n.ptr(wp_image),
            _n.ptr(scale), _n.ptr(shift), _n.ptr(wp), _n.ptr(y), _n.ptr(stats), _n.stream())
    return y, stats


def take_prepacked(w, dtc, H, W):
    return _PREPACKED.pop((w.data_ptr(), w._version, dtc, int(H), int(W)), None)


def _conv(x_store, dt_code, dtype, N, H, W, cin_s, cin_k, cout_s, wp, in_mode, scale, shift, want_stats):
    dev = x_store.device
    y = torch.empty(N, H, W, cout_s, dtype=dtype, device=dev)
    stats = None
    if want_stats:
        nt = _n.call("spcl_conv_stat_rows", dt_code, N, H, W, cin_k, cout_s)
        stats = torch.empty(_n.call("spcl_bn_stats_elems", nt, cout_s), dtype=torch.float32, device=dev)
        stats.ntiles = nt
    _n.call("spcl_conv3x3_forward", _n.ptr(x_store), dt_code, N, H, W, cin_s, cin_k, cout_s, _n.ptr(wp), in_mode,
            _n.ptr(scale), _n.ptr(shift), _n.ptr(y), _n.ptr(stats), _n.stream())
    return y, stats


def _conv_cat(xa, xb, dt_code, dtype, N, H, W, chalf, cout_s, wp, want_stats, xb_scale=None, xb_shift=None):
    dev = xa.device
    y = torch.empty(N, H, W, cout_s, dtype=dtype, device=dev)
    stats = None
    if want_stats:
        nt = _n.call("spcl_conv_stat_rows", dt_code, N, H, W, 2 * chalf, cout_s)
        stats = torch.empty(_n.call("spcl_bn_stats_elems", nt, cout_s), dtype=torch.float32, device=dev)
        stats.ntiles = nt
    _n.call("spcl_conv3x3_forward_cat", _n.ptr(xa), _n.ptr(xb), dt_code, N, H, W, chalf, cout_s, _n.ptr(wp),
            _n.ptr(xb_scale), _n.ptr(xb_shift), _n.ptr(y), _n.ptr(stats), _n.stream())
    return y, stats


_BN_ACC = os.environ.get("SPCL_BN_ACC", "1") != "0"
_ACC_ARENA = {"buf": None, "off": 0, "used": 0, "need": 0, "dirty": False}


def bn_acc_arena_begin(device):
    a = _ACC_ARENA
    a["need"], a["used"], a["off"] = a["used"], 0, 0
    a["buf"] = torch.empty(a["need"], dtype=torch.int64, device=device) if (a["need"] > 0 and _BN_ACC) else None
    a["dirty"] = a["buf"] is not None


def _acc_arena_take_dirty(device):
    a = _ACC_ARENA
    if a["dirty"] and a["buf"] is not None and a["buf"].device == device:
        a["dirty"] = False
        return a["buf"]
    return None


def bn_acc_block(cs, device):
    words = _n.call("spcl_bn_acc_elems", int(cs))
    a = _ACC_ARENA
    buf = a["buf"]
    if buf is not None and a["dirty"]:
        buf.zero_()
        a["dirty"] = False
    if buf is None or buf.device != device or a["off"] + words > buf.numel():
        buf = a["buf"] = torch.zeros(max(words, 1 << 15), dtype=torch.int64, device=device)
        a["off"] = 0
    blk = buf[a["off"]:a["off"] + words]
    a["off"] += words
    a["used"] += words
    return blk


def _bn_acc_desc(acc, cfg: "BlockCfg", C, cs, gamma, beta, which, count, st, keep):
    g, b = gamma.detach().contiguous().float(), beta.detach().contiguous().float()
    rm, rv, nbt = cfg.buffers[which]
# ... 237 lines not shown
    queue = sink_queue(sinks[0])
    if queue is not None and _TAILS:
        if queue.capture_tail(sinks[0], (ws, dact), launch):
            dw = None
    else:
        launch()
    return dw, dgamma, dbeta


def _image_wgrad_fusable(cfg, cin, cout_s):
    return cfg.image_input and cin == 1 and cout_s <= 256 and cout_s & (cout_s - 1) == 0


def _dgrad_bnstats(dy, wp_t, y2, st2, dt_code, dtype, N, H, W, cin_k, cout_s):
    if not _n.call("spcl_conv_dgrad_bnstats_supported", dt_code, N, H, W, cin_k, cout_s):
        return None
    dev = dy.device
    nt = _n.call("spcl_conv_stat_rows", dt_code, N, H, W, cin_k, cout_s)
    g = torch.empty(N, H, W, cout_s, dtype=dtype, device=dev)
    rows = torch.empty(nt * 2 * cout_s, dtype=torch.float32, device=dev)
    _n.call("spcl_conv3x3_dgrad_bnstats", _n.ptr(dy), dt_code, N, H, W, cin_k, cout_s, _n.ptr(wp_t), _n.ptr(g),
            _n.ptr(y2), _n.ptr(st2[2]), _n.ptr(st2[3]), _n.ptr(st2[0]), _n.ptr(rows), _n.stream())
    rows.ntiles = nt
    return g, rows


def _bnrelu_bwd_rows(y, dact, image, rows, dt_code, dtype, N, H, W, C, cs, st, training, sinks):
    dev = y.device
    nbytes = _n.call("spcl_bnrelu_image_wgrad_workspace_bytes" if image is not None else
                     "spcl_bnrelu_bwd_workspace_bytes", N, H, W, cs)
    ws = torch.empty(nbytes // 4, dtype=torch.float32, device=dev)
    if image is not None:
        first = _grad_buffer(sinks[0], (C, 1, 3, 3), dev)
        dgamma, dbeta = _grad_buffer(sinks[1], (C,), dev), _grad_buffer(sinks[2], (C,), dev)
        dy, dw = None, first
    else:
        first = torch.empty(N, H, W, cs, dtype=dtype, device=dev)
        dgamma, dbeta = _grad_buffer(sinks[0], (C,), dev), _grad_buffer(sinks[1], (C,), dev)
        dy, dw = first, None
    def launch():
        _n.call("spcl_bnrelu_backward_rows", _n.ptr(y), _n.ptr(dact), _n.ptr(image), _n.ptr(rows), rows.ntiles, dt_code,
                N, H, W, C, cs, _n.ptr(st[0]), _n.ptr(st[1]), _n.ptr(st[2]), _n.ptr(st[3]), int(training), _n.ptr(ws),
                _n.ptr(dgamma), _n.ptr(dbeta), _n.ptr(dy), _n.ptr(dw), _n.stream())

    queue = sink_queue(sinks[0]) if image is not None else None
    if queue is not None and _TAILS:
        if queue.capture_tail(sinks[0], (ws, dact), launch):
            first = None
    else:
        launch()
    return first, dgamma, dbeta


_IMAGE3 = os.environ.get("SPCL_IMAGE3", "1") != "0"


def _image3_supported(cfg, cin, dt_code, N, H, W, cout_s):
    return bool(_IMAGE3 and cfg.image_input and cin == 1 and cfg.dtype == torch.bfloat16 and W <= 256 and
                _n.call("spcl_conv_dgrad_bnstats_image_supported", dt_code, N, H, W, cout_s, cout_s))


def _image_autocorr(image, N, H, W):
    rows = _n.call("spcl_image_autocorr_rows", N, H, W)
    out = torch.empty(rows, 64, dtype=torch.float32, device=image.device)
    _n.call("spcl_image_autocorr", _n.ptr(image), N, H, W, _n.ptr(out), _n.stream())
    return out


def _dgrad_bnstats_image(dy, wp_t, y2, st2, image, dt_code, dtype, N, H, W, cs, want_g=False):
    dev = dy.device
    nt = _n.call("spcl_conv_stat_rows", dt_code, N, H, W, cs, cs)
    g = torch.empty(N, H, W, cs, dtype=dtype, device=dev) if want_g else None
    rows = torch.empty(nt * 11 * cs, dtype=torch.float32, device=dev)
    _n.call("spcl_conv3x3_dgrad_bnstats_image", _n.ptr(dy), dt_code, N, H, W, cs, cs, _n.ptr(wp_t), _n.ptr(g), _n.ptr(y2),
            _n.ptr(st2[2]), _n.ptr(st2[3]), _n.ptr(st2[0]), _n.ptr(image), _n.ptr(rows), _n.stream())
    rows.ntiles = nt
    return g, rows


_CONV16_FUSED = os.environ.get("SPCL_CONV16_FUSED", "1") != "0"
_CONV16_WGROWS = os.environ.get("SPCL_CONV16_WGROWS", "1") != "0"


def _conv16_bwd_fused(dy, wp_t, y2, st2, image, dt_code, N, H, W, cin, cout, cs, sink, acorr=None, wp_image=None):
    dev = dy.device
    if y2 is None and wp_image is None:
        raise RuntimeError("conv16 backward: neither the first convolution's output nor its packed weights")
    nsplit = _n.call("spcl_conv16_bwd_fused_splits", N, H, W)
    if acorr is not None:
        rows = torch.empty(11 * cs * nsplit, dtype=torch.float32, device=dev)
        rows.wg, rows.acorr16 = nsplit, torch.empty(16, 64, dtype=torch.float32, device=dev)
    else:
        nt = _n.call("spcl_conv_stat_rows", dt_code, N, H, W, cs, cs)
        rows = torch.empty(nt * 11 * cs, dtype=torch.float32, device=dev)
        rows.ntiles, rows.wg = nt, 0
    ws = torch.empty(nsplit * 9 * 256, dtype=torch.float32, device=dev)
    dw = _grad_buffer(sink, (cout, cin, 3, 3), dev)

    def launch():
        _n.call("spcl_conv16_bwd_fused" if y2 is not None else "spcl_conv16_bwd_fused_image", _n.ptr(dy), dt_code, N, H, W,
                _n.ptr(wp_t), _n.ptr(y2 if y2 is not None else wp_image), _n.ptr(st2[2]),
                _n.ptr(st2[3]), _n.ptr(st2[0]), _n.ptr(image), _n.ptr(rows) if not rows.wg else None, _n.ptr(ws), _n.ptr(dw),
                cin, cout, _n.ptr(rows) if rows.wg else None, _n.ptr(acorr), 0 if acorr is None else acorr.shape[0],
                _n.ptr(rows.acorr16) if rows.wg else None, _n.stream())

    queue = sink_queue(sink)
    if queue is not None and _TAILS:
        if queue.capture_tail(sink, (ws, dy, y2, image, rows, wp_image), launch):
            return None, rows
        return dw, rows
    launch()
    return dw, rows


def _bnrelu_bwd_rows_image3(rows, acorr, w, N, H, W, C, cs, st, training, sinks):
    dev = rows.device
    ws = torch.empty(_n.call("spcl_bnrelu_image3_workspace_bytes", cs) // 4, dtype=torch.float32, device=dev)
    dw = _grad_buffer(sinks[0], (C, 1, 3, 3), dev)
    dgamma, dbeta = _grad_buffer(sinks[1], (C,), dev), _grad_buffer(sinks[2], (C,), dev)
    wc = w.detach().contiguous().float()
    if getattr(rows, "wg", 0):
        _n.call("spcl_bnrelu_backward_wgrows_image3", _n.ptr(rows), rows.wg, _n.ptr(rows.acorr16), 16, _n.ptr(wc), N, H, W, C,
                cs, _n.ptr(st[0]), _n.ptr(st[1]), _n.ptr(st[2]), int(training), _n.ptr(ws), _n.ptr(dgamma), _n.ptr(dbeta),
                _n.ptr(dw), _n.stream())
        return dw, dgamma, dbeta
    _n.call("spcl_bnrelu_backward_rows_image3", _n.ptr(rows), rows.ntiles, _n.ptr(acorr), acorr.shape[0], _n.ptr(wc), N, H,
            W, C, cs, _n.ptr(st[0]), _n.ptr(st[1]), _n.ptr(st[2]), int(training), _n.ptr(ws), _n.ptr(dgamma), _n.ptr(dbeta),
            _n.ptr(dw), _n.stream())
    return dw, dgamma, dbeta


def _bnrelu_pool_bwd_rows(y, dpool, rows, dt_code, dtype, N, H, W, C, cs, st, training, sinks):
    dev = y.device
    ws = torch.empty(_n.call("spcl_bnrelu_bwd_workspace_bytes", N, H, W, cs) // 4, dtype=torch.float32, device=dev)
    dgamma = _grad_buffer(sinks[0], (C,), dev)
    dbeta = _grad_buffer(sinks[1], (C,), dev)
    dy = torch.empty(N, H, W, cs, dtype=dtype, device=dev)
    _n.call("spcl_bnrelu_pool_backward_rows", _n.ptr(y), _n.ptr(dpool), _n.ptr(rows), rows.ntiles, dt_code, N, H, W, C, cs,
            _n.ptr(st[0]), _n.ptr(st[1]), _n.ptr(st[2]), _n.ptr(st[3]), int(training), _n.ptr(ws), _n.ptr(dgamma),
            _n.ptr(dbeta), _n.ptr(dy), _n.stream())
    return dy, dgamma, dbeta


ACC_ROWS = object()


def _bnrelu_bwd_fill(y, dact, dpool, dt_code, dtype, N, H, W, C, cs, st, training, sinks, acc, dact_stride=0, d_up=None):
    dev = y.device
    dgamma = _grad_buffer(sinks[0], (C,), dev)
    dbeta = _grad_buffer(sinks[1], (C,), dev)
    dy = torch.empty(N, H, W, cs, dtype=dtype, device=dev)
    if d_up is not None:
        assert dact is None and dpool is None
        dact = torch.empty(N, H, W, cs, dtype=dtype, device=dev)
    _n.call("spcl_bnrelu_backward_fill_acc", _n.ptr(y), _n.ptr(dact), int(dact_stride), _n.ptr(dpool), _n.ptr(d_up), dt_code,
            N, H, W, C, cs, _n.ptr(st), int(training), _n.ptr(acc), _n.ptr(dgamma), _n.ptr(dbeta), _n.ptr(dy), _n.stream())
    return dy, dgamma, dbeta


def _bnrelu_bwd_rows_acc(y, dact, dpool, rows, dt_code, dtype, N, H, W, C, cs, st, training, sinks, acc):
    dev = y.device
    dgamma = _grad_buffer(sinks[0], (C,), dev)
    dbeta = _grad_buffer(sinks[1], (C,), dev)
    dy = torch.empty(N, H, W, cs, dtype=dtype, device=dev)
    _n.call("spcl_bnrelu_backward_rows_acc", _n.ptr(y), _n.ptr(dact), _n.ptr(dpool), _n.ptr(rows), rows.ntiles, dt_code, N, H, W,
            C, cs, _n.ptr(st), int(training), _n.ptr(acc), _n.ptr(dgamma), _n.ptr(dbeta), _n.ptr(dy), _n.stream())
    return dy, dgamma, dbeta


def _take_acc(ctx, name):
    acc = getattr(ctx, name, None)
    setattr(ctx, name, None)
    return acc


def _dgrad_bnstats_acc(dy, wp_t, y2, st2, dt_code, dtype, N, H, W, cin_k, cout_s, acc):
    g = torch.empty(N, H, W, cout_s, dtype=dtype, device=dy.device)
    _n.call("spcl_conv3x3_dgrad_bnstats_acc", _n.ptr(dy), dt_code, N, H, W, cin_k, cout_s, _n.ptr(wp_t), _n.ptr(g), _n.ptr(y2),
            _n.ptr(st2[2]), _n.ptr(st2[3]), _n.ptr(st2[0]), _n.ptr(acc), _n.stream())
    return g


def _bnrelu_bwd_acc(y, dact, dpool, dact_nc, dt_code, dtype, N, H, W, C, cs, st, training, sinks, acc):
    dev = y.device
    dgamma = _grad_buffer(sinks[0], (C,), dev)
    dbeta = _grad_buffer(sinks[1], (C,), dev)
    dy = torch.empty(N, H, W, cs, dtype=dtype, device=dev)
    assert st.is_contiguous() and tuple(st.shape) == (4, cs)
    _n.call("spcl_bnrelu_backward_acc", _n.ptr(y), _n.ptr(dact), _n.ptr(dpool), _n.ptr(dact_nc), dt_code, N, H, W, C, cs,
            _n.ptr(st), int(training), _n.ptr(acc), _n.ptr(dgamma), _n.ptr(dbeta), _n.ptr(dy), _n.stream())
    return dy, dgamma, dbeta
# ... 119 lines not shown
                        None, _n.ptr(pool), _n.ptr(ymax), _n.stream())
            else:
                _n.call("spcl_bnrelu_pool_forward_acc", _n.ptr(yb), dtc, N, H, W, cout_s, ctypes.byref(bn_b), _n.ptr(act),
                        _n.ptr(pool), _n.stream())
        elif lazy:
            act, pool = yb, None
            cfg.link_act = ActLink(yb, stb, N, H, W, cout, cout_s)
        elif ctx.up2:
            act = torch.empty(N, 2 * H, 2 * W, cout_s, dtype=dtype, device=dev)
            pool = None
            _n.call("spcl_bnrelu_up2_forward", _n.ptr(yb), dtc, N, H, W, cout_s, _n.ptr(stb[2]), _n.ptr(stb[3]), _n.ptr(act),
                    _n.stream())
        else:
            act = _act_buffer(cfg, N, H, W, cout_s, dtype, dev) if cfg.need_act else None
            pool = torch.empty(N, H // 2, W // 2, cout_s, dtype=dtype, device=dev) if cfg.need_pool else None
            if want_ymax:
                ymax = torch.empty_like(pool)
                _n.call("spcl_bnrelu_pool_forward_ymax", _n.ptr(yb), dtc, N, H, W, cout_s, _n.ptr(stb[2]), _n.ptr(stb[3]), None,
                        None, _n.ptr(pool), _n.ptr(ymax), _n.stream())
            else:
                _bnrelu_fwd(yb, dtc, N, H, W, cout_s, stb[2], stb[3], act, pool)
        ctx.save_for_backward(xs, ya, yb, sta, stb, wa, wb)
        ctx.x2s = x2s
        ctx.params = (wa, ga, ba, wb, gb, bb)
        ctx.packed_t = (wpa_t, wpb_t)
        ctx.cfg = cfg
        if need_bwd and pool is not None and act is None and cfg.training and dtype == torch.bfloat16:
            cfg.link_out = PoolLink(yb, stb, N, H, W, cout_s, ctx.acc_bwd_b, ymax)
        ctx.meta = (N, cin, H, W, cout, cout_s, cin_s, cin_k, mode_a, x.dtype)
        outs = []
        outs.append(nhwc_to_logical(act, cout) if act is not None else None)
        outs.append(nhwc_to_logical(pool, cout) if pool is not None else None)
        return tuple(outs)

    @staticmethod
    def backward(ctx, d_act, d_pool):
        xs, ya, yb, sta, stb, wa, wb = ctx.saved_tensors
        cfg = ctx.cfg
        N, cin, H, W, cout, cout_s, cin_s, cin_k, mode_a, xdt = ctx.meta
        dtype = cfg.dtype
        dtc = _n.dtype_code(dtype)
        g_nc = broadcast_rows(d_act, dtype) if (_BCAST and d_pool is None and d_act is not None and not ctx.up2
                                                  and d_act.shape[1] == cout_s) else None
        d_up = None
        ul = getattr(cfg, "up_link", None)
        if ul is not None and ul.d_up is not None:
            du, holder = ul.d_up, ul.holder
            same = (d_act is not None and d_pool is None and d_act.data_ptr() == ul.dx_ptr and d_act.dtype == holder.dtype
                    and holder._version == ul.version and nhwc_channel_slice(d_act, dtype) is None
                    and to_nhwc_padded(d_act, dtype).data_ptr() == ul.dx_ptr)
            dirty = holder._version != ul.version
            ul.d_up, ul.dx_ptr, ul.holder = None, 0, None
            if same:
                d_up, d_act = du, None
            else:
                gs = torch.empty(N, H, W, cout_s, dtype=dtype, device=du.device)
                _n.call("spcl_upsample2x_backward", _n.ptr(du), _n.ptr(gs), dtc, N, H, W, cout_s, _n.stream())
                gl = nhwc_to_logical(gs, cout)
                d_act = gl if d_act is None else d_act.to(gl.dtype) + gl
                if dirty:
                    holder.zero_()
        elif ctx.up2 and d_act is not None:
            du = to_nhwc_padded(d_act, dtype)
            if _UP2_BWD_FUSED and d_pool is None:
                d_up, d_act = du, None
            else:
                dsum = torch.empty(N, H, W, cout_s, dtype=dtype, device=du.device)
                _n.call("spcl_upsample2x_backward", _n.ptr(du), _n.ptr(dsum), dtc, N, H, W, cout_s, _n.stream())
                d_act = nhwc_to_logical(dsum, cout)
        da_stride = 0
        da_sl = nhwc_channel_slice(d_act, dtype) if (d_act is not None and g_nc is None) else None
        if da_sl is not None:
            da_s, da_stride = da_sl
        else:
            da_s = to_nhwc_padded(d_act, dtype) if (d_act is not None and g_nc is None) else None
        dp_s = to_nhwc_padded(d_pool, dtype) if d_pool is not None else None
        if da_s is None and dp_s is None and g_nc is None and d_up is None:
            return (None,) * 9
        x2s = ctx.x2s
        ng = ctx.needs_input_grad
        sk = tuple(take_grad_sink(p, ng[i + 1]) for i, p in enumerate(ctx.params))
        lk = cfg.link_out
        la = getattr(cfg, "link_act", None)
        if la is not None and da_s is not None and dp_s is None and da_stride == 0 and la.fresh(da_s.data_ptr()):
            dyb, dgb, dbb = _bnrelu_bwd_rows(yb, da_s, None, la.rows, dtc, dtype, N, H, W, cout, cout_s, stb, cfg.training,
                                             sk[4:6])
        elif g_nc is not None:
            acc = _take_acc(ctx, "acc_bwd_b")
            if acc is not None:
                dyb, dgb, dbb = _bnrelu_bwd_acc(yb, None, None, g_nc, dtc, dtype, N, H, W, cout, cout_s, stb, cfg.training,
                                                sk[4:6], acc)
            else:
                dyb, dgb, dbb = _bnrelu_bwd_bcast(yb, g_nc, dtc, dtype, N, H, W, cout, cout_s, stb, cfg.training, sk[4:6])
        elif lk is not None and da_s is None and dp_s is not None and lk.fresh(dp_s.data_ptr()):
            if lk.rows is ACC_ROWS:
                dyb, dgb, dbb = _bnrelu_bwd_acc(yb, None, dp_s, None, dtc, dtype, N, H, W, cout, cout_s, stb, cfg.training,
                                                sk[4:6], _take_acc(ctx, "acc_bwd_b"))
            else:
                acc = _take_acc(ctx, "acc_bwd_b") if (_ACC_FILL and H % 2 == 0 and W % 2 == 0 and cout_s <= 256) else None
                if acc is not None:
                    dyb, dgb, dbb = _bnrelu_bwd_rows_acc(yb, None, dp_s, lk.rows, dtc, dtype, N, H, W, cout, cout_s, stb,
                                                         cfg.training, sk[4:6], acc)
                else:
                    dyb, dgb, dbb = _bnrelu_pool_bwd_rows(yb, dp_s, lk.rows, dtc, dtype, N, H, W, cout, cout_s, stb,
                                                          cfg.training, sk[4:6])
        else:
            acc = _take_acc(ctx, "acc_bwd_b") if _ACC_FILL else None
            if acc is not None and lk is not None and lk.rows is ACC_ROWS:
                acc = None
            if acc is not None:
                dyb, dgb, dbb = _bnrelu_bwd_fill(yb, da_s, dp_s, dtc, dtype, N, H, W, cout, cout_s, stb, cfg.training, sk[4:6],
                                                 acc, dact_stride=da_stride, d_up=d_up)
            else:
                dyb, dgb, dbb = _bnrelu_bwd(yb, da_s, dp_s, dtc, dtype, N, H, W, cout, cout_s, stb, cfg.training, sk[4:6],
                                            dact_stride=da_stride, d_up=d_up)
        if lk is not None:
            lk.rows, lk.dx_ptr, lk.holder = None, 0, None
        if la is not None:
            la.rows, la.dx_ptr, la.holder = None, 0, None
        wpa_t, wpb_t = ctx.packed_t
        if wpb_t is None:
            wpb_t = _pack(wb, 1, dtc, dtype)
        image3 = ctx.acorr is not None
        one_pass = (image3 and (_CONV16_FUSED or ya is None) and ctx.needs_input_grad[4] and cout == cout_s
                    and _n.call("spcl_conv16_bwd_fused_supported", dtc, N, H, W, cout_s, cout_s))
        if ya is None and not one_pass:
            raise RuntimeError("image block backward: the first convolution's output was not stored and the one-pass kernel "
                               "that forms it again is not available")
        if one_pass:
            dwb, rows16 = _conv16_bwd_fused(dyb, wpb_t, ya, sta, xs, dtc, N, H, W, cout, cout, cout_s, sk[3],
                                            acorr=ctx.acorr if _CONV16_WGROWS else None, wp_image=ctx.wpa_fwd)
        else:
            dwb = _wgrad(ya, dyb, dtc, N, H, W, cout, cout_s, cout_s, cout, cout_s, 1, sta[2], sta[3], sk[3]) \
                if ctx.needs_input_grad[4] else None
        if one_pass:
            fused = (None, rows16)
        elif image3:
            fused = _dgrad_bnstats_image(dyb, wpb_t, ya, sta, xs, dtc, dtype, N, H, W, cout_s)
        else:
            acc = _take_acc(ctx, "acc_bwd_a")
            if acc is not None:
                fused = (_dgrad_bnstats_acc(dyb, wpb_t, ya, sta, dtc, dtype, N, H, W, cout_s, cout_s, acc), (ACC_ROWS, acc))
            else:
                fused = _dgrad_bnstats(dyb, wpb_t, ya, sta, dtc, dtype, N, H, W, cout_s, cout_s) \
                    if dtype == torch.bfloat16 else None
        if fused is not None:
            daa, rows = fused
        else:
            daa, _ = _conv(dyb, dtc, dtype, N, H, W, cout_s, cout_s, cout_s, wpb_t, 0, None, None, False)
        image_fused = ctx.needs_input_grad[1] and not ctx.needs_input_grad[0] and _image_wgrad_fusable(cfg, cin, cout_s)
        if image3:
            dya = None
            dwa, dga, dba = _bnrelu_bwd_rows_image3(rows, ctx.acorr, wa, N, H, W, cout, cout_s, sta, cfg.training, sk[0:3])
        elif image_fused:
            dya = None
            if fused is not None:
                dwa, dga, dba = _bnrelu_bwd_rows(ya, daa, xs, rows, dtc, dtype, N, H, W, cout, cout_s, sta, cfg.training,
                                                 sk[0:3])
            else:
                dwa, dga, dba = _bnrelu_bwd_image_wgrad(ya, daa, xs, dtc, N, H, W, cout, cout_s, sta, cfg.training,
                                                        sk[0:3])
        else:
            if fused is not None and isinstance(rows, tuple) and rows[0] is ACC_ROWS:
                dya, dga, dba = _bnrelu_bwd_acc(ya, daa, None, None, dtc, dtype, N, H, W, cout, cout_s, sta, cfg.training,
                                                sk[1:3], rows[1])
            elif fused is not None:
                acc = _take_acc(ctx, "acc_rows_a")
                if acc is not None:
                    dya, dga, dba = _bnrelu_bwd_rows_acc(ya, daa, None, rows, dtc, dtype, N, H, W, cout, cout_s, sta,
                                                         cfg.training, sk[1:3], acc)
                else:
                    dya, dga, dba = _bnrelu_bwd_rows(ya, daa, None, rows, dtc, dtype, N, H, W, cout, cout_s, sta,
                                                     cfg.training, sk[1:3])
            else:
                dya, dga, dba = _bnrelu_bwd(ya, daa, None, dtc, dtype, N, H, W, cout, cout_s, sta, cfg.training,
                                            sk[1:3])
            if not ctx.needs_input_grad[1]:
                dwa = None
            elif x2s is not None:
                dwa = _wgrad_cat(xs, x2s, dya, dtc, N, H, W, cin // 2, cout, cout_s, sk[0], *ctx.x2_coef)
            else:
                dwa = _wgrad(xs, dya, dtc, N, H, W, cin, cin_s, cin_k, cout, cout_s, mode_a, None, None, sk[0])
        dx = dx2 = None
        if ctx.needs_input_grad[0] or (x2s is not None and ctx.needs_input_grad[8]):
            if cfg.image_input:
                raise NotImplementedError("gradient w.r.t. the input image is not on the hot path")
            if wpa_t is None:
                wpa_t = _pack(wa, 1, dtc, dtype)
            li = cfg.link_in
            dxs = None
            if (li is not None and dtype == torch.bfloat16 and li.cout_s == cin_s and li.N == N
                    and _n.call("spcl_conv_dgrad_poolstats_supported", dtc, N, H, W, cout_s, cin_s, li.H, li.W)):
                dxs = torch.empty(N, H, W, cin_s, dtype=dtype, device=dya.device)
                ym = li.ymax if (li.ymax is not None and tuple(li.ymax.shape) == (N, H, W, cin_s)) else None
                if (li.acc is not None and _n.call("spcl_conv_dgrad_poolstats_acc_supported", dtc, N, H, W, cout_s, cin_s,
                                                   li.H, li.W)):
                    acc_in, li.acc = li.acc, None
                    if ym is not None and _n.call("spcl_conv_dgrad_poolmax_acc_supported", dtc, N, H, W, cout_s, cin_s):
                        _n.call("spcl_conv3x3_dgrad_poolmax_acc", _n.ptr(dya), dtc, N, H, W, cout_s, cin_s, _n.ptr(wpa_t),
                                _n.ptr(dxs), _n.ptr(ym), _n.ptr(li.stb[2]), _n.ptr(li.stb[3]), _n.ptr(li.stb[0]),
                                _n.ptr(acc_in), _n.stream())
                    else:
                        _n.call("spcl_conv3x3_dgrad_poolstats_acc", _n.ptr(dya), dtc, N, H, W, cout_s, cin_s, _n.ptr(wpa_t),
                                _n.ptr(dxs), _n.ptr(li.yb), li.H, li.W, _n.ptr(li.stb[2]), _n.ptr(li.stb[3]),
                                _n.ptr(li.stb[0]), _n.ptr(acc_in), _n.stream())
                    rows = ACC_ROWS
                else:
                    nt = _n.call("spcl_conv_stat_rows", dtc, N, H, W, cout_s, cin_s)
                    rows = torch.empty(nt * 2 * cin_s, dtype=torch.float32, device=dya.device)
                    if ym is not None and _n.call("spcl_conv_dgrad_poolmax_supported", dtc, N, H, W, cout_s, cin_s):
                        _n.call("spcl_conv3x3_dgrad_poolmax", _n.ptr(dya), dtc, N, H, W, cout_s, cin_s, _n.ptr(wpa_t),
                                _n.ptr(dxs), _n.ptr(ym), _n.ptr(li.stb[2]), _n.ptr(li.stb[3]), _n.ptr(li.stb[0]),
                                _n.ptr(rows), _n.stream())
                    else:
# ... 1415 lines not shown
```

self-paced-contrastive-learning_amd/native.py:

```python
from __future__ import annotations

import ctypes
import os
from ctypes import c_char_p, c_double, c_float, c_int, c_long, c_size_t, c_void_p

import torch

HERE = os.path.dirname(os.path.abspath(__file__))
LIB_PATH = os.path.join(HERE, "lib", "libspcl_hip.so")
SPCL_F32, SPCL_BF16 = 0, 1

_lib = None

_P = c_void_p
_SIGNATURES = {
    "spcl_abi_version": (c_int, []),
    "spcl_last_error": (c_char_p, []),
    "spcl_supcon_workspace_bytes": (c_size_t, [c_int, c_int]),
    "spcl_supcon_forward": (c_int, [_P, _P, _P, _P, c_int, c_int, c_float, c_int, c_float, c_int, _P, _P, _P]),
    "spcl_supcon_backward": (c_int, [_P, _P, c_int, c_int, c_float, c_int, c_float, _P, _P, _P, _P, _P, _P, _P]),
    "spcl_supcon_bwd_workspace_bytes": (c_size_t, [c_int, c_int]),
    "spcl_supcon_unit_gradient_block": (c_int, [c_int, c_int, _P, _P]),
    "spcl_supcon_materialize": (c_int, [_P, _P, c_int, c_int, c_float, c_int, c_float, _P, _P, _P, _P, _P, _P, _P]),
    "spcl_supcon_xpos_workspace_bytes": (c_size_t, [c_int, c_int]),
# ... 21 lines not shown
    "spcl_l2norm_rows_backward": (c_int, [_P, _P, c_size_t, c_int, _P, _P]),
    "spcl_conv_packed_elems": (c_size_t, [c_int, c_int, c_int, c_int]),
    "spcl_conv_pack_weights": (c_int, [_P, c_int, c_int, c_int, c_int, _P, _P]),
    "spcl_conv_pack_weights_both": (c_int, [_P, c_int, c_int, c_int, _P, _P, _P]),
    "spcl_conv_pack_weights_block": (c_int, [_P, c_int, c_int, _P, _P, _P, c_int, c_int, _P, _P, c_int, _P]),
    "spcl_conv_pack_weights_block_at": (c_int, [_P, c_int, c_int, _P, _P, _P, c_int, c_int, _P, _P, c_int, c_int, c_int, _P]),
    "spcl_conv_pack_weights_multi": (c_int, [_P, c_int, c_int, _P]),
    "spcl_conv_pack_weights_multi_acorr": (c_int, [_P, c_int, c_int, _P, c_int, c_int, c_int, _P, _P]),
    "spcl_conv_pack_weights_multi_zero": (c_int, [_P, c_int, c_int, _P, c_int, c_int, c_int, _P, _P, c_size_t, _P]),
    "spcl_conv_num_tiles": (c_int, [c_int, c_int, c_int]),
    "spcl_conv_stat_rows": (c_int, [c_int, c_int, c_int, c_int, c_int, c_int]),
    "spcl_conv_set_gemm": (None, [c_int]),
    "spcl_conv_set_f32_split": (None, [c_int]),
    "spcl_conv_get_f32_split": (c_int, []),
    "spcl_conv_cat_supported": (c_int, [c_int, c_int, c_int, c_int, c_int, c_int]),
    "spcl_conv3x3_forward_cat": (c_int, [_P, _P, c_int, c_int, c_int, c_int, c_int, c_int, _P, _P, _P, _P, _P, _P]),
    "spcl_conv_split_supported": (c_int, [c_int, c_int, c_int, c_int, c_int, c_int]),
    "spcl_conv3x3_forward_split": (c_int, [_P, c_int, c_int, c_int, c_int, c_int, c_int, _P, _P, _P, _P]),
    "spcl_conv_split_bnstats_supported": (c_int, [c_int, c_int, c_int, c_int, c_int, c_int]),
    "spcl_conv3x3_dgrad_split_bnstats": (c_int, [_P, c_int, c_int, c_int, c_int, c_int, c_int, _P, _P, _P, _P, _P, _P, _P, _P,
                                                 _P]),
    "spcl_conv_up2_supported": (c_int, [c_int, c_int, c_int, c_int, c_int, c_int]),
    "spcl_conv3x3_forward_up2": (c_int, [_P, c_int, c_int, c_int, c_int, c_int, c_int, _P, _P, _P, _P]),
    "spcl_conv3x3_wgrad_up2": (c_int, [_P, _P, c_int, c_int, c_int, c_int, c_int, c_int, c_int, _P, _P, _P]),
    "spcl_conv3x3_wgrad_cat": (c_int, [_P, _P, _P, c_int, c_int, c_int, c_int, c_int, c_int, c_int, _P, _P, _P, _P, _P]),
    "spcl_bn_stats_elems": (c_size_t, [c_int, c_int]),
    "spcl_conv3x3_forward": (c_int, [_P, c_int, c_int, c_int, c_int, c_int, c_int, c_int, _P, c_int, _P, _P, _P, _P,
                                     _P]),
    "spcl_supcon_forward_heads": (c_int, [c_int, _P, _P, c_size_t, _P, c_int, c_int, c_float, c_int, _P, c_int, _P,
                                          c_size_t, _P, _P]),
    "spcl_supcon_rows_supported": (c_int, [c_int, c_int]),
    "spcl_supcon_forward_rows": (c_int, [c_int, _P, _P, c_size_t, _P, c_int, c_int, c_float, c_int, _P, c_int, _P,
                                         c_size_t, _P, _P]),
    "spcl_supcon_backward_heads": (c_int, [c_int, _P, c_int, c_int, c_float, c_int, _P, _P, c_size_t, _P, c_size_t, _P,
                                           _P, _P, _P, c_size_t, _P]),
    "spcl_conv_wgrad_workspace_bytes": (c_size_t, [c_int, c_int, c_int, c_int, c_int]),
    "spcl_conv3x3_wgrad": (c_int, [_P, _P, c_int, c_int, c_int, c_int, c_int, c_int, c_int, c_int, c_int, c_int, _P,
                                   _P, _P, _P, _P]),
    "spcl_conv_wgrad_batched_supported": (c_int, [c_int, c_int, c_int, c_int, c_int, c_int]),
    "spcl_conv_wgrad_batched_workspace_bytes": (c_size_t, [_P, c_int]),
    "spcl_conv3x3_wgrad_batched": (c_int, [_P, c_int, c_int, _P, _P]),
    "spcl_wgrad_tail_capture": (c_int, [_P]),
    "spcl_conv3x3_wgrad_batched_tails": (c_int, [_P, c_int, _P, c_int, c_int, _P, _P]),
    "spcl_bn_finalize": (c_int, [_P, c_int, c_int, c_int, _P, _P, c_float, c_float, _P, _P, _P, _P, _P, _P, _P, _P]),
    "spcl_bn_eval_affine": (c_int, [c_int, c_int, _P, _P, _P, _P, c_float, _P, _P, _P, _P, _P]),
    "spcl_bn_eval_affine_multi": (c_int, [_P, c_int, _P]),
    "spcl_bnrelu_pool_forward": (c_int, [_P, c_int, c_int, c_int, c_int, c_int, _P, _P, _P, _P, _P]),
    "spcl_bnrelu_up2_forward": (c_int, [_P, c_int, c_int, c_int, c_int, c_int, _P, _P, _P, _P]),
    "spcl_bnrelu_pool_forward_strided": (c_int, [_P, c_int, c_int, c_int, c_int, c_int, _P, _P, _P, c_int, _P, _P]),
    "spcl_bnrelu_pool_backward_strided": (c_int, [_P, _P, c_int, _P, c_int, c_int, c_int, c_int, c_int, c_int, _P, _P, _P,
                                                  _P, c_int, _P, _P, _P, _P, _P]),
    "spcl_bnrelu_bwd_workspace_bytes": (c_size_t, [c_int, c_int, c_int, c_int]),
    "spcl_bnrelu_pool_backward": (c_int, [_P, _P, _P, c_int, c_int, c_int, c_int, c_int, c_int, _P, _P, _P, _P,
                                          c_int, _P, _P, _P, _P, _P]),
    "spcl_bnrelu_backward_up2": (c_int, [_P, _P, _P, c_int, c_int, c_int, c_int, c_int, c_int, _P, _P, _P, _P, c_int, _P, _P, _P, _P,
                                         _P]),
    "spcl_bnrelu_backward_bcast": (c_int, [_P, _P, c_int, c_int, c_int, c_int, c_int, c_int, _P, _P, _P, _P, c_int, _P, _P,
                                           _P, _P, _P]),
    "spcl_bnrelu_image_wgrad_workspace_bytes": (c_size_t, [c_int, c_int, c_int, c_int]),
    "spcl_bnrelu_backward_image_wgrad": (c_int, [_P, _P, _P, c_int, c_int, c_int, c_int, c_int, c_int, _P, _P, _P, _P,
                                                 c_int, _P, _P, _P, _P, _P]),
    "spcl_accumulate_scalars": (c_int, [c_int, _P, _P, _P, _P]),
    "spcl_stage_bytes": (c_int, [_P, _P, c_size_t, _P]),
    "spcl_conv_dgrad_bnstats_supported": (c_int, [c_int, c_int, c_int, c_int, c_int, c_int]),
    "spcl_conv3x3_dgrad_bnstats": (c_int, [_P, c_int, c_int, c_int, c_int, c_int, c_int, _P, _P, _P, _P, _P, _P, _P, _P]),
    "spcl_conv_dgrad_poolstats_supported": (c_int, [c_int, c_int, c_int, c_int, c_int, c_int, c_int, c_int]),
    "spcl_conv3x3_dgrad_poolstats": (c_int, [_P, c_int, c_int, c_int, c_int, c_int, c_int, _P, _P, _P, c_int, c_int, _P, _P,
                                             _P, _P, _P]),
    "spcl_bnrelu_pool_backward_rows": (c_int, [_P, _P, _P, c_int, c_int, c_int, c_int, c_int, c_int, c_int, _P, _P, _P, _P,
                                               c_int, _P, _P, _P, _P, _P]),
    "spcl_bnrelu_backward_rows": (c_int, [_P, _P, _P, _P, c_int, c_int, c_int, c_int, c_int, c_int, c_int, _P, _P, _P, _P,
                                          c_int, _P, _P, _P, _P, _P, _P]),
    "spcl_image_autocorr_rows": (c_int, [c_int, c_int, c_int]),
    "spcl_image_autocorr": (c_int, [_P, c_int, c_int, c_int, _P, _P]),
    "spcl_conv_dgrad_bnstats_image_supported": (c_int, [c_int, c_int, c_int, c_int, c_int, c_int]),
    "spcl_conv3x3_forward_image_acorr_rows": (c_int, [c_int, c_int, c_int, c_int, c_int, c_int]),
    "spcl_conv3x3_forward_image_acorr": (c_int, [_P, c_int, c_int, c_int, c_int, c_int, c_int, _P, _P, _P, _P, _P]),
    "spcl_block1_recompute_supported": (c_int, [c_int, c_int, c_int, c_int, c_int, c_int]),
    "spcl_block1_kernels_take": (c_int, [c_int, c_int, c_int, c_int, c_int, c_int]),
    "spcl_conv3x3_forward_from_image": (c_int, [_P, _P, c_int, c_int, c_int, c_int, c_int, _P, _P, _P, _P, _P, _P, _P]),
    "spcl_conv16_bwd_fused_image_supported": (c_int, [c_int, c_int, c_int, c_int, c_int, c_int]),
    "spcl_conv16_bwd_fused_image": (c_int, [_P, c_int, c_int, c_int, c_int, _P, _P, _P, _P, _P, _P, _P, _P, _P, c_int, c_int,
                                            _P, _P, c_int, _P, _P]),
    "spcl_conv16_bwd_fused_supported": (c_int, [c_int, c_int, c_int, c_int, c_int, c_int]),
    "spcl_conv16_bwd_fused_splits": (c_int, [c_int, c_int, c_int]),
    "spcl_conv16_bwd_fused": (c_int, [_P, c_int, c_int, c_int, c_int, _P, _P, _P, _P, _P, _P, _P, _P, _P, c_int, c_int,
                                      _P, _P, c_int, _P, _P]),
    "spcl_bnrelu_backward_wgrows_image3": (c_int, [_P, c_int, _P, c_int, _P, c_int, c_int, c_int, c_int, c_int, _P, _P, _P,
                                                   c_int, _P, _P, _P, _P, _P]),
    "spcl_conv3x3_dgrad_bnstats_image": (c_int, [_P, c_int, c_int, c_int, c_int, c_int, c_int, _P, _P, _P, _P, _P, _P, _P,
                                                 _P, _P]),
    "spcl_bnrelu_image3_workspace_bytes": (c_size_t, [c_int]),
    "spcl_bnrelu_backward_rows_image3": (c_int, [_P, c_int, _P, c_int, _P, c_int, c_int, c_int, c_int, c_int, _P, _P, _P,
                                                 c_int, _P, _P, _P, _P, _P]),
    "spcl_conv1x1_forward": (c_int, [_P, c_int, c_size_t, c_int, c_int, c_int, _P, _P, _P, _P]),
    "spcl_conv1x1_bwd_workspace_bytes": (c_size_t, [c_int, c_int]),
    "spcl_conv1x1_backward": (c_int, [_P, _P, c_int, c_size_t, c_int, c_int, c_int, _P, _P, _P, _P, _P, _P]),
    "spcl_conv1x1_forward_bn": (c_int, [_P, c_int, c_size_t, c_int, c_int, c_int, _P, _P, _P, _P, _P, _P]),
    "spcl_conv1x1_bwd_rows": (c_int, [c_size_t]),
    "spcl_conv1x1_backward_bn": (c_int, [_P, _P, c_int, c_size_t, c_int, c_int, c_int, _P, _P, _P, _P, _P, _P, _P, _P, _P, _P]),
    "spcl_softmax_forward": (c_int, [_P, c_size_t, c_int, _P, _P]),
    "spcl_softmax_backward": (c_int, [_P, _P, c_size_t, c_int, _P, _P]),
    "spcl_kl_workspace_bytes": (c_size_t, []),
    "spcl_kl_div_forward": (c_int, [_P, _P, c_size_t, c_int, c_float, _P, _P, _P]),
    "spcl_kl_div_backward": (c_int, [_P, _P, c_size_t, c_int, c_float, _P, _P, _P]),
    "spcl_sup_loss_forward": (c_int, [_P, _P, c_int, c_int, c_int, c_float, _P, _P, _P, _P, _P, _P]),
    "spcl_one_hot": (c_int, [_P, c_size_t, c_int, _P, _P]),
    "spcl_argmax_classes": (c_int, [_P, c_size_t, c_int, _P, _P]),
    "spcl_dice_counts": (c_int, [_P, _P, c_int, c_int, c_int, _P, _P, _P]),
    "spcl_surface_workspace_bytes": (c_size_t, [c_int, c_int, c_int, c_int]),
    "spcl_surface_distances": (c_int, [_P, _P, c_int, c_int, c_int, c_int, _P, c_int, c_double, c_double, c_double, _P, _P, _P,
                                       _P, _P, c_size_t, _P]),
    "spcl_surface_3d_workspace_bytes": (c_size_t, [c_int, c_int, c_int, c_int, c_int]),
    "spcl_surface_distances_3d": (c_int, [_P, _P, c_int, c_int, c_int, c_int, c_int, _P, c_int, c_double, c_double, c_double,
                                          c_double, _P, _P, _P, _P, _P, c_size_t, _P]),
    "spcl_upsample2x_forward": (c_int, [_P, _P, c_int, c_int, c_int, c_int, c_int, _P]),
    "spcl_upsample2x_backward": (c_int, [_P, _P, c_int, c_int, c_int, c_int, c_int, _P]),
    "spcl_concat2_channels": (c_int, [_P, _P, _P, c_int, c_size_t, c_int, c_int, _P]),
    "spcl_split2_channels": (c_int, [_P, _P, _P, c_int, c_size_t, c_int, c_int, _P]),
    "spcl_augment_views": (c_int, [_P, c_int, c_int, c_int, _P, c_int, _P, c_int, c_int, _P]),
    "spcl_augment_views_recipe": (c_int, [_P, _P, c_int, c_int, c_int, _P, c_int, _P, _P, c_int, c_int, c_int, _P]),
    "spcl_augment_views_recipe_workspace_bytes": (c_size_t, [c_int, c_int, c_int]),
    "spcl_rows_linear_forward": (c_int, [_P, c_int, c_long, c_int, _P, _P, c_int, c_int, c_int, _P, _P]),
    "spcl_rows_linear_forward_act": (c_int, [_P, c_int, c_long, _P, _P, c_int, c_int, c_int, _P, c_int, _P]),
    "spcl_adaptive_avgpool2d_backward_act": (c_int, [_P, _P, c_int, c_int, c_int, c_int, c_int, c_int, c_int, _P, _P]),
    "spcl_rows_linear_backward_input": (c_int, [_P, c_int, _P, _P, c_int, c_int, c_int, _P, c_int, c_long, _P]),
    "spcl_rows_linear_backward_weight_workspace_bytes": (c_size_t, [c_int, c_int, c_int]),
    "spcl_rows_linear_backward_weight": (c_int, [_P, c_int, _P, c_int, c_long, c_int, c_int, c_int, c_int, _P, c_size_t, _P, _P, _P]),
    "spcl_augment_views_recipe_ws": (c_int, [_P, _P, c_int, c_int, c_int, _P, c_int, _P, _P, c_int, c_int, c_int, _P, c_size_t,
                                             _P]),
    "spcl_resize_bilinear_pil": (c_int, [_P, c_int, c_int, c_int, _P, _P, c_int, _P, _P, c_int, _P, _P, c_int, c_int, _P]),
    "spcl_resize_nearest_pil": (c_int, [_P, c_int, c_int, c_int, _P, _P, _P, c_int, c_int, _P]),
    "spcl_augment_views_pil": (c_int, [_P, c_int, c_int, c_int, _P, c_int, _P, c_int, c_int, _P]),
    "spcl_flip_batch": (c_int, [_P, _P, c_int, c_int, c_int, c_int, c_int, _P, _P]),
    "spcl_flip_pair": (c_int, [_P, _P, _P, c_int, c_int, c_int, c_int, c_int, _P, _P]),
    "spcl_flip_pair_stage": (c_int, [_P, _P, _P, c_int, c_int, c_int, c_int, c_int, _P, _P, c_size_t, c_size_t, _P]),
    "spcl_profile_enable": (c_int, [c_int]),
    "spcl_profile_count": (c_int, []),
    "spcl_profile_get": (c_int, [c_int, c_char_p, c_int, _P, _P, _P]),
    "spcl_radam_step": (c_int, [_P, _P, _P, _P, c_size_t, _P, _P, c_double, c_double, c_double, c_double, _P, _P]),
    "spcl_radam_step_scalars": (c_int, [_P, _P, _P, _P, c_size_t, _P, _P, c_double, c_double, c_double, c_double, _P,
                                        c_int, _P, _P, _P, _P]),
    "spcl_radam_step_scaled": (c_int, [_P, _P, c_double, _P, _P, c_size_t, _P, _P, c_double, c_double, c_double, c_double,
                                       _P, c_int, _P, _P, _P, _P]),
    "spcl_bnrelu_gap_supported": (c_int, [c_int, c_int, c_int, c_int, c_int]),
    "spcl_bnrelu_gap_forward": (c_int, [_P, c_int, c_int, c_int, c_int, c_int, c_int, _P, _P, _P, _P, _P, _P]),
    "spcl_bnrelu_backward_fill_acc": (c_int, [_P, _P, c_int, _P, _P, c_int, c_int, c_int, c_int, c_int, c_int, _P, c_int, _P, _P,
                                              _P, _P, _P]),
    "spcl_copy_pair": (c_int, [_P, _P, c_size_t, _P, _P, c_size_t, _P]),
    "spcl_bnrelu_backward_rows_acc": (c_int, [_P, _P, _P, _P, c_int, c_int, c_int, c_int, c_int, c_int, c_int, _P, c_int, _P, _P,
                                              _P, _P, _P]),
    "spcl_radam_apply_staged": (c_int, [_P, _P, c_double, _P, _P, c_size_t, _P, _P, c_double, c_double, c_double, c_double,
                                        c_int, _P, _P, _P, _P]),
    "spcl_adam_step_scaled": (c_int, [_P, _P, c_double, _P, _P, c_size_t, _P, _P, c_double, c_double, c_double, c_double,
                                      c_int, _P, c_int, _P, _P, _P, _P]),
    "spcl_adam_apply_staged": (c_int, [_P, _P, c_double, _P, _P, c_size_t, _P, _P, c_double, c_double, c_double, c_double,
                                       c_int, c_int, _P, _P, _P, _P]),
    "spcl_sgd_step_scaled": (c_int, [_P, _P, c_double, _P, c_size_t, _P, _P, c_double, c_double, c_double, c_int, _P, c_int,
                                     _P, _P, _P, _P]),
    "spcl_sgd_apply_staged": (c_int, [_P, _P, c_double, _P, c_size_t, _P, _P, c_double, c_double, c_double, c_int, c_int, _P,
                                      _P, _P, _P]),
    "spcl_bn_acc_elems": (c_size_t, [c_int]),
    "spcl_conv_bn_acc_supported": (c_int, [c_int, c_int, c_int, c_int, c_int, c_int, c_int, c_int]),
    "spcl_conv3x3_forward_acc": (c_int, [_P, c_int, c_int, c_int, c_int, c_int, c_int, _P, _P, _P, _P, _P, _P, _P, _P]),
    "spcl_bnrelu_pool_forward_acc": (c_int, [_P, c_int, c_int, c_int, c_int, c_int, _P, _P, _P, _P]),
    "spcl_conv_dgrad_bnstats_acc_supported": (c_int, [c_int, c_int, c_int, c_int, c_int, c_int]),
# ... 6 lines not shown
    "spcl_conv3x3_dgrad_poolmax": (c_int, [_P, c_int, c_int, c_int, c_int, c_int, c_int, _P, _P, _P, _P, _P, _P, _P, _P]),
    "spcl_conv_dgrad_poolmax_acc_supported": (c_int, [c_int, c_int, c_int, c_int, c_int, c_int]),
    "spcl_conv3x3_dgrad_poolmax_acc": (c_int, [_P, c_int, c_int, c_int, c_int, c_int, c_int, _P, _P, _P, _P, _P, _P, _P, _P]),
    "spcl_bnrelu_backward_acc": (c_int, [_P, _P, _P, _P, c_int, c_int, c_int, c_int, c_int, c_int, _P, c_int, _P, _P, _P, _P,
                                         _P]),
    "spcl_iic_joint_workspace_bytes": (c_size_t, [c_int, c_int, c_int]),
    "spcl_iic_joint_forward": (c_int, [_P, _P, c_long, c_int, c_int, c_int, c_int, c_int, c_int, _P, _P, _P]),
    "spcl_iic_loss_workspace_bytes": (c_size_t, [c_int, c_int]),
    "spcl_iic_loss": (c_int, [_P, _P, c_int, c_int, c_int, c_int, c_float, _P, _P, _P, _P, _P, c_size_t, _P]),
    "spcl_iic_joint_backward": (c_int, [_P, _P, c_long, c_int, c_int, c_int, c_int, c_int, c_int, _P, _P, _P, _P, _P, _P]),
    "spcl_consistency_workspace_bytes": (c_size_t, [c_int, c_int, c_int]),
    "spcl_consistency_softmax_mse": (c_int, [_P, _P, c_int, c_int, c_int, c_int, _P, c_float, _P, _P, _P, c_size_t, _P]),
    "spcl_iic_patch_plan": (c_int, [c_int, c_int, c_int, c_int, c_int, c_int, _P, _P, _P]),
    "spcl_iic_patch_forward": (c_int, [_P, _P, c_int, c_int, c_int, c_int, c_int, c_int, _P, c_float, _P, _P, _P, _P, _P,
                                       c_size_t, _P]),
    "spcl_iic_patch_backward": (c_int, [_P, _P, c_int, c_int, c_int, c_int, c_int, c_int, _P, _P, _P, _P, _P, _P]),
    "spcl_ema_update": (c_int, [_P, _P, c_size_t, c_double, c_double, _P]),
    "spcl_mt_softmax_mse_workspace_bytes": (c_size_t, [c_int, c_int, c_int]),
    "spcl_mt_softmax_mse": (c_int, [_P, _P, c_int, c_int, c_int, c_int, _P, c_int, c_float, _P, _P, _P, c_size_t, _P]),
    "spcl_entropy_softmax_workspace_bytes": (c_size_t, [c_int, c_int, c_int]),
    "spcl_entropy_softmax": (c_int, [_P, c_int, c_int, c_int, c_int, c_float, c_float, _P, _P, _P, c_size_t, _P]),
    "spcl_ucmt_workspace_bytes": (c_size_t, [c_int, c_int, c_int]),
    "spcl_ucmt_softmax_mse": (c_int, [_P, _P, c_int, _P, c_int, c_int, c_int, c_int, _P, c_float, c_float, c_float, _P, _P, _P,
                                      _P, _P, c_size_t, _P]),
    "spcl_mixup_images": (c_int, [_P, _P, _P, c_int, c_size_t, c_float, c_float, _P, _P]),
    "spcl_mixup_kl_workspace_bytes": (c_size_t, [c_int, c_int, c_int]),
    "spcl_mixup_kl_onehot": (c_int, [_P, _P, _P, _P, c_int, c_int, c_int, c_int, c_float, c_float, c_float, c_float, _P, _P, _P,
                                     c_size_t, _P]),
    "spcl_patch4s2_rows_forward": (c_int, [_P, c_int, c_long, c_long, c_long, c_long, _P, c_int, c_long, c_long, c_long, c_long,
                                           c_int, c_int, c_int, c_int, _P, _P, _P, _P]),
    "spcl_patch4s2_rows_backward": (c_int, [_P, _P, c_int, c_int, c_int, c_int, c_int, c_int, _P, _P, _P, _P]),
    "spcl_rows_bn_workspace_bytes": (c_size_t, [c_int, c_int]),
    "spcl_rows_bn_forward": (c_int, [_P, c_int, c_int, _P, _P, c_float, c_float, _P, _P, _P, _P, c_size_t, _P]),
    "spcl_rows_bn_eval_affine": (c_int, [_P, _P, _P, _P, c_float, c_int, _P, _P]),
    "spcl_rows_bn_backward": (c_int, [_P, _P, c_int, c_int, _P, _P, c_int, _P, _P, _P, _P, c_size_t, _P]),
    "spcl_discr_head_workspace_bytes": (c_size_t, [c_int, c_int, c_int, c_int]),
    "spcl_discr_head_forward": (c_int, [_P, c_int, c_int, c_int, c_int, _P, _P, _P, c_int, _P, _P, _P, _P, _P, c_size_t, _P]),
    "spcl_discr_head_backward": (c_int, [_P, c_int, c_int, c_int, c_int, _P, _P, _P, _P, _P, _P, _P, _P, c_size_t, _P]),
    "spcl_mine_pairs_forward": (c_int, [_P, _P, c_int, c_int, c_int, c_int, c_int, _P, _P, _P]),
    "spcl_mine_pairs_backward": (c_int, [_P, _P, _P, c_int, c_int, c_int, c_int, c_int, _P, _P]),
    "spcl_mine_head_workspace_bytes": (c_size_t, [c_int, c_int, c_int, c_int]),
    "spcl_mine_head_forward": (c_int, [_P, _P, c_int, c_int, c_int, c_int, c_int, _P, _P, _P, _P, _P, _P, _P, c_size_t, _P]),
    "spcl_mine_head_backward": (c_int, [_P, _P, _P, _P, _P, c_int, c_int, c_int, c_int, c_int, _P, _P, _P, _P, _P]),
    "spcl_pica_workspace_bytes": (c_size_t, [c_int]),
    "spcl_pica_seg_loss": (c_int, [_P, _P, c_int, c_int, c_int, c_double, c_float, _P, _P, _P, _P, _P, c_size_t, _P]),
    "spcl_pica_global_loss": (c_int, [_P, _P, c_long, c_int, c_int, c_int, c_float, c_float, _P, _P, _P, _P, _P, _P, c_size_t,
                                      _P]),
}


class WgradItem(ctypes.Structure):
    _fields_ = [("x", c_void_p), ("dy", c_void_p), ("in_scale", c_void_p), ("in_shift", c_void_p),
                ("dw_oihw", c_void_p), ("N", c_int), ("H", c_int), ("W", c_int), ("Cin", c_int), ("CinS", c_int),
                ("Cout", c_int), ("CoutS", c_int), ("in_mode", c_int), ("x2", c_void_p), ("x_up2", c_int)]


class PackItem(ctypes.Structure):
    _fields_ = [("w_oihw", c_void_p), ("fwd", c_void_p), ("dgrad", c_void_p), ("Cin", c_int), ("Cout", c_int),
                ("H", c_int), ("W", c_int)]


BN_EVAL_MAX = 32


class BnEvalItem(ctypes.Structure):
    _fields_ = [("gamma", c_void_p), ("beta", c_void_p), ("running_mean", c_void_p), ("running_var", c_void_p),
                ("st", c_void_p), ("C", c_int), ("CS", c_int), ("eps", c_float)]


class BnAcc(ctypes.Structure):
    _fields_ = [("acc", c_void_p), ("gamma", c_void_p), ("beta", c_void_p), ("running_mean", c_void_p),
                ("running_var", c_void_p), ("num_batches_tracked", c_void_p), ("st", c_void_p), ("momentum", c_float),
                ("eps", c_float), ("count", c_float), ("C", c_int), ("CS", c_int)]


PACK_MULTI_MAX = 24


class WgradTail(ctypes.Structure):
    _fields_ = [("partial", c_void_p), ("dw", c_void_p), ("kind", c_int), ("nsplit", c_int), ("nblk_ci", c_int),
                ("nblk_co", c_int), ("CIB", c_int), ("COB", c_int), ("Cin", c_int), ("Cout", c_int)]


ABI_VERSION = 24
WGRAD_BATCH_MAX = 16
WGRAD_TAILS_MAX = 16
_NO_STATUS = ("spcl_abi_version", "spcl_block1_recompute_supported", "spcl_block1_kernels_take", "spcl_conv16_bwd_fused_image_supported", "spcl_conv3x3_forward_image_acorr_rows", "spcl_image_autocorr_rows", "spcl_conv_dgrad_bnstats_image_supported", "spcl_conv16_bwd_fused_supported", "spcl_conv16_bwd_fused_splits", "spcl_conv_num_tiles", "spcl_conv_stat_rows", "spcl_conv_set_gemm", "spcl_conv_set_f32_split", "spcl_conv_get_f32_split", "spcl_supcon_unit_gradient_block", "spcl_conv_cat_supported", "spcl_conv_up2_supported", "spcl_conv_split_supported", "spcl_conv_split_bnstats_supported", "spcl_conv1x1_bwd_rows", "spcl_profile_count", "spcl_conv_dgrad_bnstats_supported", "spcl_conv_dgrad_poolstats_supported",
              "spcl_conv_wgrad_batched_supported", "spcl_conv_bn_acc_supported", "spcl_conv_dgrad_bnstats_acc_supported",
              "spcl_conv_dgrad_poolstats_acc_supported", "spcl_supcon_rows_supported", "spcl_bnrelu_gap_supported",
              "spcl_conv_dgrad_poolmax_supported", "spcl_conv_dgrad_poolmax_acc_supported")


class NativeLibraryError(RuntimeError):
    pass


def lib():
    global _lib
    if _lib is None:
        if not os.path.exists(LIB_PATH):
            raise NativeLibraryError(
                f"{LIB_PATH} is missing: build it with `python self-paced-contrastive-learning_amd/build.py` "
                "(there is no CPU / eager fallback for the hot path)")
        L = ctypes.CDLL(LIB_PATH)
        L.spcl_abi_version.restype, L.spcl_abi_version.argtypes = c_int, []
        have = L.spcl_abi_version()
        if have != ABI_VERSION:
            raise NativeLibraryError(
                f"{LIB_PATH} has C-ABI version {have}, this binding was written for {ABI_VERSION} (include/spcl_hip.h "
                "SPCL_ABI_VERSION): a stale build -- rebuild with `python self-paced-contrastive-learning_amd/build.py`")
        for name, (res, args) in _SIGNATURES.items():
            fn = getattr(L, name, None)
            if fn is None:
                continue
            fn.restype, fn.argtypes = res, args
        _lib = L
    return _lib


def call(name: str, *args):
    L = lib()
    fn = getattr(L, name, None)
    if fn is None:
        raise NativeLibraryError(f"libspcl_hip.so does not export {name}")
    rc = fn(*args)
    if fn.restype is c_int and name not in _NO_STATUS and rc != 0:
        raise RuntimeError(f"{name} failed ({rc}): {L.spcl_last_error().decode()}")
    return rc


def require_gpu(*tensors):
    for t in tensors:
        if t is None:
            continue
        if not t.is_cuda:
            raise RuntimeError("self-paced-contrastive-learning_amd runs on MI355X only: got a CPU tensor "
                               "(the HIP path has no CPU fallback)")


def ptr(t):
    return None if t is None else c_void_p(t.data_ptr())


def stream():
    return c_void_p(torch.cuda.current_stream().cuda_stream)


def ptr_array(tensors):
    return (c_void_p * len(tensors))(*[None if t is None else t.data_ptr() for t in tensors])


def dtype_code(dt: torch.dtype) -> int:
    if dt == torch.float32:
        return SPCL_F32
    if dt == torch.bfloat16:
        return SPCL_BF16
    raise TypeError(f"unsupported activation dtype {dt}")
```

Baseline: 31660 slices/s.

## Fuse BN-ReLU-maxpool backward into the first-block conv16 backward kernel

Adds a POOLDY variant of the conv16 backward kernel that rebuilds the gradient of the first conv block directly from the stored activation y and the max-pool gradient. It does this per tile in LDS, using BN coefficients computed in the kernel prologue from the accumulated statistics, instead of first writing a full dy tensor in a separate BN/ReLU/pool backward pass. This removes one full-resolution write and read of dy, plus a kernel launch, at 224x224. In exchange the conv kernel does more loads per tile (four y values plus dpool for each pool window), uses more registers, and has a different occupancy hint.

After: 32100 slices/s, median of 6. +1.4%, better.

```diff
diff --git a/include/spcl_hip.h b/include/spcl_hip.h
--- a/include/spcl_hip.h
+++ b/include/spcl_hip.h
@@ -14,7 +14,7 @@
 #define SPCL_ELAUNCH (-2)
 #define SPCL_EUNSUPPORTED (-3)
 
-#define SPCL_ABI_VERSION 24
+#define SPCL_ABI_VERSION 25
 int spcl_abi_version(void);
 const char* spcl_last_error(void);
 
@@ -253,6 +253,13 @@
                                 const void* w_packed_image, const float* scale2, const float* shift2, const float* mean2,
                                 const float* image, float* rows11, float* partial, float* dw_oihw, int Cin, int Cout,
                                 float* wg_rows, const float* acorr, int nacorr, float* acorr16, void* stream);
+int spcl_conv16_bwd_fused_image_pooled_supported(int dtype, int N, int H, int W, int CinK, int CoutS, int training);
+int spcl_conv16_bwd_fused_image_pooled(const void* y, const void* dpool, const float* rows, int nrows, int dtype, int N, int H,
+                                       int W, const float* st4, int training, long long* acc, float* dgamma, float* dbeta,
+                                       const void* w_packed_dgrad, const void* w_packed_image, const float* scale2,
+                                       const float* shift2, const float* mean2, const float* image, float* rows11,
+                                       float* partial, float* dw_oihw, int Cin, int Cout, float* wg_rows, const float* acorr,
+                                       int nacorr, float* acorr16, void* stream);
 int spcl_bnrelu_backward_wgrows_image3(const float* wg_rows, int nwg, const float* acorr, int nacorr, const float* w_oihw,
                                        int N, int H, int W, int C, int CS, const float* mean, const float* invstd,
                                        const float* scale, int training, float* ws, float* dgamma, float* dbeta,
diff --git a/self-paced-contrastive-learning_amd/csrc/bn.hip b/self-paced-contrastive-learning_amd/csrc/bn.hip
--- a/self-paced-contrastive-learning_amd/csrc/bn.hip
+++ b/self-paced-contrastive-learning_amd/csrc/bn.hip
@@ -3,6 +3,7 @@
 #include "bn_acc.hpp"
 #include "common.hpp"
 #include "image_acorr.hpp"
+#include "pool_dy.hpp"
 
 namespace spcl {
 
@@ -221,23 +222,6 @@
   shift[c] = q.beta[c] - q.running_mean[c] * sc;
 }
 
-template <typename T> struct Word;
-template <> struct Word<float> {
-  static constexpr int EPW = 1;
-  static __device__ __forceinline__ float get(uint32_t w, int) { return __uint_as_float(w); }
-  static __device__ __forceinline__ uint32_t make(const float* v) { return __float_as_uint(v[0]); }
-  static __device__ __forceinline__ uint32_t merge(const uint32_t* s) { return s[0]; }
-};
-template <> struct Word<bf16_t> {
-  static constexpr int EPW = 2;
-  static __device__ __forceinline__ float get(uint32_t w, int h) {
-    return __uint_as_float(h ? (w & 0xffff0000u) : (w << 16));
-  }
-  static __device__ __forceinline__ uint32_t make(const float* v) {
-    return (uint32_t)f32_to_bf16(v[0]) | ((uint32_t)f32_to_bf16(v[1]) << 16);
-  }
-  static __device__ __forceinline__ uint32_t merge(const uint32_t* s) { return (s[0] & 0x0000ffffu) | (s[1] & 0xffff0000u); }
-};
 
 template <int EPC> __device__ __forceinline__ void load_coef(float* dst, const float* src, int cc) {
 #pragma unroll
@@ -865,22 +849,7 @@
               continue;
             }
             if (APPLY && FAST) {
-              float yk[4], z[4];
-#pragma unroll
-              for (int k = 0; k < 4; ++k) {
-                yk[k] = Word<T>::get(w.ry[k][wi], h);
-                z[k] = fmaf(sc[e], yk[k], sh[e]);
-              }
-              float m = fmaxf(z[0], 0.f);
-              const bool s1 = z[1] > m;
-              m = fmaxf(m, z[1]);
-              const bool s2 = z[2] > m;
-              m = fmaxf(m, z[2]);
-              const bool s3 = z[3] > m;
-              const bool b[4] = {z[0] > 0.f && !s1 && !s2 && !s3, s1 && !s2 && !s3, s2 && !s3, s3};
-              const float dp = Word<T>::get(rdp[wi], h);
-#pragma unroll
-              for (int k = 0; k < 4; ++k) o[k][h] = fmaf(sc[e], b[k] ? dp : 0.f, fmaf(c0[e], yk[k], c1[e]));
+              SPCL_POOL_WINDOW_DY(T, w.ry, rdp, wi, h, sc[e], sh[e], c0[e], c1[e], o)
               continue;
             }
             float yk[4], dz[4];
@@ -1093,6 +1062,13 @@
   }
 }
 
+int launch_bwd_rows_acc(const float* rows, int nrows, int CS, long long* acc, hipStream_t st) {
+  const int G = (nrows + 511) / 512;
+  const int nwg = (nrows + G - 1) / G;
+  SPCL_LAUNCH(bwd_rows_acc_kernel, dim3(nwg), dim3(256), 0, st, rows, nrows, G, CS, acc);
+  return nwg;
+}
+
 template <typename T>
 __global__ __launch_bounds__(256, 6) void bnrelu_bwd_apply_lin_kernel(const T* __restrict__ y, const T* __restrict__ g,
                                                                    size_t npix, int CS,
@@ -1403,9 +1379,7 @@
   if (a.sums == BnSums::Rows) {
     static const int fin_rows = lab_env("SPCL_BWD_FIN_MAX_ROWS", BWD_MAX_WG);
     if (a.acc != nullptr) {
-      const int G = (a.nrows + 511) / 512;
-      s.nwg = (a.nrows + G - 1) / G;
-      SPCL_LAUNCH(bwd_rows_acc_kernel, dim3(s.nwg), dim3(256), 0, a.st, a.rows, a.nrows, G, a.CS, a.acc);
+      s.nwg = launch_bwd_rows_acc(a.rows, a.nrows, a.CS, a.acc, a.st);
     } else if (a.nrows <= fin_rows) {
       s.fin_src = a.rows;
       s.nwg = a.nrows;
diff --git a/self-paced-contrastive-learning_amd/csrc/bn_acc.hpp b/self-paced-contrastive-learning_amd/csrc/bn_acc.hpp
--- a/self-paced-contrastive-learning_amd/csrc/bn_acc.hpp
+++ b/self-paced-contrastive-learning_amd/csrc/bn_acc.hpp
@@ -42,6 +42,8 @@
 };
 
 #ifdef __HIPCC__
+int launch_bwd_rows_acc(const float* rows, int nrows, int CS, long long* acc, hipStream_t st);
+
 __device__ __forceinline__ void bn_acc_atomic_add(long long* p, long long v) {
   (void)__hip_atomic_fetch_add(p, v, __ATOMIC_RELAXED, __HIP_MEMORY_SCOPE_AGENT);
 }
diff --git a/self-paced-contrastive-learning_amd/csrc/conv16_bwd.hip b/self-paced-contrastive-learning_amd/csrc/conv16_bwd.hip
--- a/self-paced-contrastive-learning_amd/csrc/conv16_bwd.hip
+++ b/self-paced-contrastive-learning_amd/csrc/conv16_bwd.hip
@@ -1,7 +1,9 @@
 #include <stdio.h>
 #include <stdlib.h>
 #include <vector>
+#include "bn_acc.hpp"
 #include "conv_common.hpp"
+#include "pool_dy.hpp"
 
 namespace spcl {
 
@@ -24,6 +26,9 @@
   int N, H, W, tilesX, tilesY, ipw, xcd_remap;
   int dbg;
   unsigned long long* stamps;
+  const unsigned char* yb;
+  const unsigned char* dpool;
+  BnAccBwd bw;
 };
 
 constexpr int B16_TH = 14, B16_TW = 14, B16_HW = 16, B16_RP = 22, B16_PS = 32;
@@ -435,10 +440,13 @@
 constexpr int R16_TRASH = R16_ACC + 576;
 constexpr int R16_TAB = R16_TRASH + 32;
 constexpr int B16_LDS_ROWS = R16_TAB + 128;
-
-template <bool SHIFTED, bool WGROWS, bool RECOMP = false>
-__global__ __launch_bounds__(128) __attribute__((amdgpu_waves_per_eu(r16_wpe(SHIFTED)))) void conv16_bwd_rows_kernel(Bwd16Args a) {
+constexpr int R16_CF = B16_LDS_ROWS;
+constexpr int B16_LDS_POOLDY = R16_CF + 256;
+
+template <bool SHIFTED, bool WGROWS, bool RECOMP = false, bool POOLDY = false>
+__global__ __launch_bounds__(128) __attribute__((amdgpu_waves_per_eu(r16_wpe(SHIFTED || (POOLDY && !WGROWS))))) void conv16_bwd_rows_kernel(Bwd16Args a) {
   static_assert(!(RECOMP && SHIFTED), "y2 from the image: whole 14 x 14 tiles");
+  static_assert(!POOLDY || RECOMP, "dy from y and dpool: whole 14 x 14 tiles of the recomputing form (even H, W)");
   constexpr int NW = 2;
   constexpr int TH = B16_TH, TW = B16_TW, HW_ = B16_HW, RP = R16_RP, PS = B16_PS;
   constexpr int NSTEPS = 5, NTHR = 64 * NW, ITER = 512 / NTHR, RPI = NTHR / 32;
@@ -500,12 +508,24 @@
   }
   if (WGROWS)
     for (int i = t0; i < (512 + 576) / 4; i += NTHR) ((float*)(lds + R16_RED))[i] = 0.f;
+  if (POOLDY && t0 < 16) {
+    BnAccBwdRaw raw;
+    raw.load(a.bw, t0);
+    float ca, cb;
+    bn_acc_bwd_channel(a.bw, raw, t0, ca, cb, (blockIdx.x | blockIdx.y | blockIdx.z) == 0);
+    float* cf = (float*)(lds + R16_CF);
+    cf[t0] = ca;
+    cf[16 + t0] = cb;
+    cf[32 + t0] = raw.scale;
+    cf[48 + t0] = a.bw.st[3 * a.bw.CS + t0];
+  }
   f32x4 wacc[TPW];
 #pragma unroll
   for (int j = 0; j < TPW; ++j) wacc[j] = (f32x4){0.f, 0.f, 0.f, 0.f};
 
   float imgv[256 / NTHR];
-  u32x4 v[ITER];
+  u32x4 v[POOLDY ? 1 : ITER];
+  u32x4 pv[POOLDY ? 5 : 1];
   uint2 ypre[RECOMP ? 1 : MW];
   constexpr int PPT = 256 / NTHR;
   short wraw[3] = {0, 0, 0};
@@ -540,13 +560,79 @@
     const int voff = (hy0 * a.W + hx0) * 32 + ch * 16;
     const __amdgpu_buffer_rsrc_t rs = rsrc(a.dy + (((long)n * a.H + (y0 - 1)) * a.W + (x0 - 1)) * 32);
 #pragma unroll
-    for (int k = 0; k < ITER; ++k) {
+    for (int k = 0; k < (POOLDY ? 0 : ITER); ++k) {
       bool inb = true;
       if (!interior) {
         const int gy = y0 - 1 + hy0 + RPI * k, gx = x0 - 1 + hx0;
         inb = gy >= 0 && gy < a.H && gx >= 0 && gx < a.W;
       }
       v[k] = __builtin_bit_cast(u32x4, __builtin_amdgcn_raw_buffer_load_b128(rs, inb ? voff : OOB, RPI * k * a.W * 32, 0));
+    }
+  };
+  auto pool_item = [&](const int t, const int rd, int& half, int& wy, int& wx) {
+    const int item = rd ? t + 64 : t;
+    half = item & 1;
+    const int w = item >> 1;
+    wy = w / 9;
+    wx = w - 9 * wy;
+    bool in = item < 162;
+    if (!interior) {
+      const int gy = y0 - 2 + 2 * wy, gx = x0 - 2 + 2 * wx;
+      in = in && gy >= 0 && gy < a.H && gx >= 0 && gx < a.W;
+    }
+    return in;
+  };
+  auto issue_pool = [&](const int n, const int rd, u32x4* r) {
+    int t = t0;
+    asm volatile("" : "+v"(t));
+    int half, wy, wx;
+    const bool in = pool_item(t, rd, half, wy, wx);
+    const int HP = a.H >> 1, WP = a.W >> 1;
+    const __amdgpu_buffer_rsrc_t ry = rsrc(a.yb + (((long)n * a.H + (y0 - 2)) * a.W + (x0 - 2)) * 32);
+    const __amdgpu_buffer_rsrc_t rp = rsrc(a.dpool + (((long)n * HP + ((y0 - 2) >> 1)) * WP + ((x0 - 2) >> 1)) * 32);
+    const int vy = in ? (2 * wy * a.W + 2 * wx) * 32 + half * 16 : OOB;
+    const int vp = in ? (wy * WP + wx) * 32 + half * 16 : OOB;
+    r[0] = __builtin_bit_cast(u32x4, __builtin_amdgcn_raw_buffer_load_b128(ry, vy, 0, 0));
+    r[1] = __builtin_bit_cast(u32x4, __builtin_amdgcn_raw_buffer_load_b128(ry, vy + 32, 0, 0));
+    r[2] = __builtin_bit_cast(u32x4, __builtin_amdgcn_raw_buffer_load_b128(ry, vy, a.W * 32, 0));
+    r[3] = __builtin_bit_cast(u32x4, __builtin_amdgcn_raw_buffer_load_b128(ry, vy + 32, a.W * 32, 0));
+    r[4] = __builtin_bit_cast(u32x4, __builtin_amdgcn_raw_buffer_load_b128(rp, vp, 0, 0));
+  };
+  auto stage_pool = [&](const int rd, const u32x4* r) {
+    int t = t0;
+    asm volatile("" : "+v"(t));
+    int half, wy, wx;
+    const bool in = pool_item(t, rd, half, wy, wx);
+    const float* cf = (const float*)(lds + R16_CF) + half * 8;
+    float cA[8], cB[8], sc[8], sh[8];
+#pragma unroll
+    for (int q = 0; q < 8; q += 4) {
+      *(f32x4*)&cA[q] = *(const f32x4*)(cf + q);
+      *(f32x4*)&cB[q] = *(const f32x4*)(cf + 16 + q);
+      *(f32x4*)&sc[q] = *(const f32x4*)(cf + 32 + q);
+      *(f32x4*)&sh[q] = *(const f32x4*)(cf + 48 + q);
+    }
+    u32x4 out[4];
+#pragma unroll
+    for (int wi = 0; wi < 4; ++wi) {
+      float o[4][2];
+#pragma unroll
+      for (int h = 0; h < 2; ++h) {
+        const int e = wi * 2 + h;
+        SPCL_POOL_WINDOW_DY(bf16_t, r, r[4], wi, h, sc[e], sh[e], cA[e], cB[e], o)
+      }
+#pragma unroll
+      for (int k = 0; k < 4; ++k) out[k][wi] = Word<bf16_t>::make(o[k]);
+    }
+    if (!interior && !in) {
+#pragma unroll
+      for (int k = 0; k < 4; ++k) out[k] = (u32x4){0u, 0u, 0u, 0u};
+    }
+    const bool real = rd == 0 || t < 98;
+#pragma unroll
+    for (int k = 0; k < 4; ++k) {
+      const int hy = 2 * wy - 1 + (k >> 1), hx = 2 * wx - 1 + (k & 1);
+      if (real && hy >= 0 && hy < HW_ && hx >= 0 && hx < HW_) *(u32x4*)(lds + R16_DY + (hy * RP + hx) * PS + half * 16) = out[k];
     }
   };
   auto issue_y2 = [&](const int n) {
@@ -567,7 +653,8 @@
   if (stamp) tc = __builtin_amdgcn_s_memtime();
   if (n_first < a.N) {
     issue_img(n_first);
-    issue_halo(n_first);
+    if (POOLDY) issue_pool(n_first, 0, pv);
+    else issue_halo(n_first);
     if (!RECOMP) issue_y2(n_first);
   }
   uint2 wfp = {0u, 0u};
@@ -652,6 +739,18 @@
     int t = t0;
     asm volatile("" : "+v"(t));
     const int lane = t & 63, r16 = t & 15, g = lane >> 4;
+    if (POOLDY) {
+      __builtin_amdgcn_sched_barrier(0);
+      stage_pool(0, pv);
+      __builtin_amdgcn_sched_barrier(0);
+      if (wave == 1) {
+        u32x4 pw[5];
+        issue_pool(n, 1, pw);
+        __builtin_amdgcn_sched_barrier(0);
+        stage_pool(1, pw);
+      }
+      __builtin_amdgcn_sched_barrier(0);
+    }
     u32x4 wall[NSTEPS];
 #pragma unroll
     for (int s = 0; s < NSTEPS; ++s)
@@ -679,7 +778,7 @@
         if (hc + e >= 2) imb[512 - 2] = hb;
       }
     }
-    {
+    if (!POOLDY) {
       const int ch = t & 1, q0 = t >> 1, hy0 = q0 / HW_, hx0 = q0 % HW_;
       unsigned char* const lp = lds + R16_DY + (hy0 * RP + hx0) * PS + ch * 16;
 #pragma unroll
@@ -758,7 +857,8 @@
       }
     }
     if (!(it + 1 < a.ipw && n + 1 < a.N)) break;
-    issue_halo(n + 1);
+    if (POOLDY) issue_pool(n + 1, 0, pv);
+    else issue_halo(n + 1);
     if (!RECOMP) issue_y2(n + 1);
     issue_img(n + 1);
     second_half(n);
@@ -834,12 +934,18 @@
   return cdiv(H, B16_TH) * cdiv(W, B16_TW) * cdiv(N, ipw);
 }
 
+struct Bwd16Pooled {
+  const void* y;
+  const void* dpool;
+  BnAccBwd bw;
+};
+
 static int conv16_bwd_fused_impl(const void* dy, int dtype, int N, int H, int W, const void* w_packed_dgrad,
                                  const void* y2, const void* w_packed_image, const float* scale2, const float* shift2,
                                  const float* mean2, const float* image, float* rows11, float* partial, float* dw_oihw,
                                  int Cin, int Cout, float* wg_rows, const float* acorr, int nacorr, float* acorr16,
-                                 void* stream) {
-  SPCL_CHECK_ARG(dy && w_packed_dgrad && (y2 || w_packed_image) && scale2 && shift2 && mean2 && image && partial && dw_oihw,
+                                 void* stream, const Bwd16Pooled* pooled = nullptr) {
+  SPCL_CHECK_ARG((dy != nullptr) != (pooled != nullptr) && w_packed_dgrad && (y2 || w_packed_image) && scale2 && shift2 && mean2 && image && partial && dw_oihw,
                  "conv16_bwd_fused: null pointer");
   SPCL_CHECK_ARG((rows11 != nullptr) != (wg_rows != nullptr), "conv16_bwd_fused: exactly one of rows11 / wg_rows");
   SPCL_CHECK_ARG(wg_rows == nullptr || (acorr && acorr16 && nacorr > 0), "conv16_bwd_fused: wg_rows comes with the autocorrelation rows");
@@ -861,6 +967,10 @@
   a.wp_img = (const u32x4*)w_packed_image;
   a.scale2 = scale2; a.shift2 = shift2; a.mean2 = mean2; a.img = image; a.rows11 = rows11; a.partial = partial;
   a.wg_rows = wg_rows; a.acorr_in = acorr; a.nacorr = nacorr; a.acorr_out = acorr16;
+  a.yb = nullptr; a.dpool = nullptr; a.bw = BnAccBwd{};
+  if (pooled != nullptr) {
+    a.yb = (const unsigned char*)pooled->y; a.dpool = (const unsigned char*)pooled->dpool; a.bw = pooled->bw;
+  }
   a.N = N; a.H = H; a.W = W; a.tilesX = cdiv(W, B16_TW); a.tilesY = cdiv(H, B16_TH);
   a.ipw = conv16_bwd_ipw(N, H, W);
   static const int env_remap = lab_env("SPCL_CONV_XCD_REMAP", 1);
@@ -869,7 +979,7 @@
   const int nz = cdiv(N, a.ipw), nsplit = a.tilesX * a.tilesY * nz;
   a.nwg = nsplit;
   const double px = (double)N * H * W;
-  prof_cost(px * 32.0 * (y2 != nullptr ? 2.0 : 1.0) + px * 4.0 + (double)nsplit * 9 * 256 * 4.0, 2.0 * px * 9.0 * 256 * 2.0 + 2.0 * px * 9.0 * 16);
+  prof_cost(px * 32.0 * ((pooled != nullptr ? 1.25 : 1.0) + (y2 != nullptr ? 1.0 : 0.0)) + px * 4.0 + (double)nsplit * 9 * 256 * 4.0, 2.0 * px * 9.0 * 256 * 2.0 + 2.0 * px * 9.0 * 16);
   a.stamps = nullptr;
   const bool want_stamps = SPCL_CONV16_STAMPS_BUILD && lab_flag("SPCL_CONV16_STAMPS");
   const size_t nwg = (size_t)nsplit;
@@ -888,7 +998,10 @@
     else if (wgr) B16_LAUNCH(true, NW_, true);              \
     else B16_LAUNCH(true, NW_, false);                      \
   }
-  if (y2 == nullptr) {
+  if (pooled != nullptr) {
+    if (wgr) SPCL_LAUNCH((conv16_bwd_rows_kernel<false, true, true, true>), grid, dim3(128), B16_LDS_POOLDY, st, a);
+    else SPCL_LAUNCH((conv16_bwd_rows_kernel<false, false, true, true>), grid, dim3(128), B16_LDS_POOLDY, st, a);
+  } else if (y2 == nullptr) {
     if (wgr) SPCL_LAUNCH((conv16_bwd_rows_kernel<false, true, true>), grid, dim3(128), B16_LDS_ROWS, st, a);
     else SPCL_LAUNCH((conv16_bwd_rows_kernel<false, false, true>), grid, dim3(128), B16_LDS_ROWS, st, a);
   } else if (nw == 2 && conv16_bwd_rowmap()) {
@@ -953,3 +1066,29 @@
   return conv16_bwd_fused_impl(dy, dtype, N, H, W, w_packed_dgrad, nullptr, w_packed_image, scale2, shift2, mean2, image, rows11,
                                partial, dw_oihw, Cin, Cout, wg_rows, acorr, nacorr, acorr16, stream);
 }
+
+extern "C" int spcl_conv16_bwd_fused_image_pooled_supported(int dtype, int N, int H, int W, int CinK, int CoutS, int training) {
+  return (training != 0 && spcl_conv16_bwd_fused_image_supported(dtype, N, H, W, CinK, CoutS)) ? 1 : 0;
+}
+
+extern "C" int spcl_conv16_bwd_fused_image_pooled(const void* y, const void* dpool, const float* rows, int nrows, int dtype, int N,
+                                                  int H, int W, const float* st4, int training, long long* acc, float* dgamma,
+                                                  float* dbeta, const void* w_packed_dgrad, const void* w_packed_image,
+                                                  const float* scale2, const float* shift2, const float* mean2,
+                                                  const float* image, float* rows11, float* partial, float* dw_oihw, int Cin,
+                                                  int Cout, float* wg_rows, const float* acorr, int nacorr, float* acorr16,
+                                                  void* stream) {
+  SPCL_CHECK_ARG(y && dpool && rows && nrows > 0 && st4 && acc && dgamma && dbeta && w_packed_image,
+                 "conv16_bwd_fused_image_pooled: null pointer");
+  if (!spcl_conv16_bwd_fused_image_pooled_supported(dtype, N, H, W, 16, 16, training)) {
+    set_error("conv16_bwd_fused_image_pooled: unsupported configuration (training, bf16, 16 -> 16 channels, H and W multiples "
+              "of 14, the row-mapped kernel)");
+    return SPCL_EUNSUPPORTED;
+  }
+  launch_bwd_rows_acc(rows, nrows, 16, acc, (hipStream_t)stream);
+  Bwd16Pooled p;
+  p.y = y; p.dpool = dpool;
+  p.bw = BnAccBwd{acc, st4, dgamma, dbeta, (float)((size_t)N * H * W), training, 16, 16};
+  return conv16_bwd_fused_impl(nullptr, dtype, N, H, W, w_packed_dgrad, nullptr, w_packed_image, scale2, shift2, mean2, image, rows11,
+                               partial, dw_oihw, Cin, Cout, wg_rows, acorr, nacorr, acorr16, stream, &p);
+}
diff --git a/self-paced-contrastive-learning_amd/csrc/pool_dy.hpp b/self-paced-contrastive-learning_amd/csrc/pool_dy.hpp
--- /dev/null
+++ b/self-paced-contrastive-learning_amd/csrc/pool_dy.hpp
@@ -0,0 +1,44 @@
+#pragma once
+#include "common.hpp"
+
+namespace spcl {
+
+typedef __attribute__((ext_vector_type(4))) uint32_t u32x4;
+
+template <typename T> struct Word;
+template <> struct Word<float> {
+  static constexpr int EPW = 1;
+  static __device__ __forceinline__ float get(uint32_t w, int) { return __uint_as_float(w); }
+  static __device__ __forceinline__ uint32_t make(const float* v) { return __float_as_uint(v[0]); }
+  static __device__ __forceinline__ uint32_t merge(const uint32_t* s) { return s[0]; }
+};
+template <> struct Word<bf16_t> {
+  static constexpr int EPW = 2;
+  static __device__ __forceinline__ float get(uint32_t w, int h) {
+    return __uint_as_float(h ? (w & 0xffff0000u) : (w << 16));
+  }
+  static __device__ __forceinline__ uint32_t make(const float* v) {
+    return (uint32_t)f32_to_bf16(v[0]) | ((uint32_t)f32_to_bf16(v[1]) << 16);
+  }
+  static __device__ __forceinline__ uint32_t merge(const uint32_t* s) { return (s[0] & 0x0000ffffu) | (s[1] & 0xffff0000u); }
+};
+
+#define SPCL_POOL_WINDOW_DY(T, RY, RDP, WI, H, SC, SH, A, B, O)                                          \
+  {                                                                                                      \
+    float yk[4], z[4];                                                                                   \
+    _Pragma("unroll") for (int k = 0; k < 4; ++k) {                                                      \
+      yk[k] = Word<T>::get((RY)[k][WI], H);                                                              \
+      z[k] = fmaf(SC, yk[k], SH);                                                                        \
+    }                                                                                                    \
+    float m = fmaxf(z[0], 0.f);                                                                          \
+    const bool s1 = z[1] > m;                                                                            \
+    m = fmaxf(m, z[1]);                                                                                  \
+    const bool s2 = z[2] > m;                                                                            \
+    m = fmaxf(m, z[2]);                                                                                  \
+    const bool s3 = z[3] > m;                                                                            \
+    const bool b[4] = {z[0] > 0.f && !s1 && !s2 && !s3, s1 && !s2 && !s3, s2 && !s3, s3};                \
+    const float dp = Word<T>::get((RDP)[WI], H);                                                         \
+    _Pragma("unroll") for (int k = 0; k < 4; ++k) (O)[k][H] = fmaf(SC, b[k] ? dp : 0.f, fmaf(A, yk[k], B)); \
+  }
+
+}
diff --git a/self-paced-contrastive-learning_amd/functional.py b/self-paced-contrastive-learning_amd/functional.py
--- a/self-paced-contrastive-learning_amd/functional.py
+++ b/self-paced-contrastive-learning_amd/functional.py
@@ -981,6 +981,7 @@
 
 
 _BLOCK1_RECOMPUTE = os.environ.get("SPCL_BLOCK1_RECOMPUTE", "1") != "0"
+_BLOCK1_POOLED_BWD = os.environ.get("SPCL_BLOCK1_POOLED_BWD", "1") != "0"
 
 
 def _conv_from_image(image, y_image, dt_code, dtype, N, H, W, cout_s, wp_image, scale, shift, wp, want_stats):
@@ -1384,10 +1385,12 @@
 _CONV16_WGROWS = os.environ.get("SPCL_CONV16_WGROWS", "1") != "0"
 
 
-def _conv16_bwd_fused(dy, wp_t, y2, st2, image, dt_code, N, H, W, cin, cout, cs, sink, acorr=None, wp_image=None):
-    dev = dy.device
+def _conv16_bwd_fused(dy, wp_t, y2, st2, image, dt_code, N, H, W, cin, cout, cs, sink, acorr=None, wp_image=None, pooled=None):
+    dev = image.device
     if y2 is None and wp_image is None:
         raise RuntimeError("conv16 backward: neither the first convolution's output nor its packed weights")
+    if (dy is None) != (pooled is not None) or (pooled is not None and y2 is not None):
+        raise RuntimeError("conv16 backward: exactly one of the gradient and the tensors it is formed from")
     nsplit = _n.call("spcl_conv16_bwd_fused_splits", N, H, W)
     if acorr is not None:
         rows = torch.empty(11 * cs * nsplit, dtype=torch.float32, device=dev)
@@ -1400,6 +1403,14 @@
     dw = _grad_buffer(sink, (cout, cin, 3, 3), dev)
 
     def launch():
+        if pooled is not None:
+            yb, dpool, prow, stb, acc, dgamma, dbeta, training = pooled
+            _n.call("spcl_conv16_bwd_fused_image_pooled", _n.ptr(yb), _n.ptr(dpool), _n.ptr(prow), prow.ntiles, dt_code, N, H, W,
+                    _n.ptr(stb), int(training), _n.ptr(acc), _n.ptr(dgamma), _n.ptr(dbeta), _n.ptr(wp_t), _n.ptr(wp_image),
+                    _n.ptr(st2[2]), _n.ptr(st2[3]), _n.ptr(st2[0]), _n.ptr(image), _n.ptr(rows) if not rows.wg else None,
+                    _n.ptr(ws), _n.ptr(dw), cin, cout, _n.ptr(rows) if rows.wg else None, _n.ptr(acorr),
+                    0 if acorr is None else acorr.shape[0], _n.ptr(rows.acorr16) if rows.wg else None, _n.stream())
+            return
         _n.call("spcl_conv16_bwd_fused" if y2 is not None else "spcl_conv16_bwd_fused_image", _n.ptr(dy), dt_code, N, H, W,
                 _n.ptr(wp_t), _n.ptr(y2 if y2 is not None else wp_image), _n.ptr(st2[2]),
                 _n.ptr(st2[3]), _n.ptr(st2[0]), _n.ptr(image), _n.ptr(rows) if not rows.wg else None, _n.ptr(ws), _n.ptr(dw),
@@ -1408,7 +1419,7 @@
 
     queue = sink_queue(sink)
     if queue is not None and _TAILS:
-        if queue.capture_tail(sink, (ws, dy, y2, image, rows, wp_image), launch):
+        if queue.capture_tail(sink, (ws, image, dy, y2, rows, wp_image, pooled), launch):
             return None, rows
         return dw, rows
     launch()
@@ -1694,6 +1705,7 @@
         sk = tuple(take_grad_sink(p, ng[i + 1]) for i, p in enumerate(ctx.params))
         lk = cfg.link_out
         la = getattr(cfg, "link_act", None)
+        pooled = None
         if la is not None and da_s is not None and dp_s is None and da_stride == 0 and la.fresh(da_s.data_ptr()):
             dyb, dgb, dbb = _bnrelu_bwd_rows(yb, da_s, None, la.rows, dtc, dtype, N, H, W, cout, cout_s, stb, cfg.training,
                                              sk[4:6])
@@ -1710,7 +1722,14 @@
                                                 sk[4:6], _take_acc(ctx, "acc_bwd_b"))
             else:
                 acc = _take_acc(ctx, "acc_bwd_b") if (_ACC_FILL and H % 2 == 0 and W % 2 == 0 and cout_s <= 256) else None
-                if acc is not None:
+                if (acc is not None and _BLOCK1_POOLED_BWD and ya is None and ctx.acorr is not None and ctx.wpa_fwd is not None
+                        and ctx.needs_input_grad[4] and cout == cout_s and dtype == torch.bfloat16
+                        and _n.call("spcl_conv16_bwd_fused_image_pooled_supported", dtc, N, H, W, cout_s, cout_s,
+                                    int(cfg.training))):
+                    dyb = None
+                    dgb, dbb = _grad_buffer(sk[4], (cout,), yb.device), _grad_buffer(sk[5], (cout,), yb.device)
+                    pooled = (yb, dp_s, lk.rows, stb, acc, dgb.view(cout), dbb.view(cout), cfg.training)
+                elif acc is not None:
                     dyb, dgb, dbb = _bnrelu_bwd_rows_acc(yb, None, dp_s, lk.rows, dtc, dtype, N, H, W, cout, cout_s, stb,
                                                          cfg.training, sk[4:6], acc)
                 else:
@@ -1739,9 +1758,12 @@
         if ya is None and not one_pass:
             raise RuntimeError("image block backward: the first convolution's output was not stored and the one-pass kernel "
                                "that forms it again is not available")
+        if pooled is not None and not one_pass:
+            raise RuntimeError("image block backward: the gradient behind the max-pool was not materialised and the one-pass "
+                               "kernel that forms it is not available")
         if one_pass:
             dwb, rows16 = _conv16_bwd_fused(dyb, wpb_t, ya, sta, xs, dtc, N, H, W, cout, cout, cout_s, sk[3],
-                                            acorr=ctx.acorr if _CONV16_WGROWS else None, wp_image=ctx.wpa_fwd)
+                                            acorr=ctx.acorr if _CONV16_WGROWS else None, wp_image=ctx.wpa_fwd, pooled=pooled)
         else:
             dwb = _wgrad(ya, dyb, dtc, N, H, W, cout, cout_s, cout_s, cout, cout_s, 1, sta[2], sta[3], sk[3]) \
                 if ctx.needs_input_grad[4] else None
diff --git a/self-paced-contrastive-learning_amd/native.py b/self-paced-contrastive-learning_amd/native.py
--- a/self-paced-contrastive-learning_amd/native.py
+++ b/self-paced-contrastive-learning_amd/native.py
@@ -127,6 +127,9 @@
     "spcl_conv16_bwd_fused_image_supported": (c_int, [c_int, c_int, c_int, c_int, c_int, c_int]),
     "spcl_conv16_bwd_fused_image": (c_int, [_P, c_int, c_int, c_int, c_int, _P, _P, _P, _P, _P, _P, _P, _P, _P, c_int, c_int,
                                             _P, _P, c_int, _P, _P]),
+    "spcl_conv16_bwd_fused_image_pooled_supported": (c_int, [c_int, c_int, c_int, c_int, c_int, c_int, c_int]),
+    "spcl_conv16_bwd_fused_image_pooled": (c_int, [_P, _P, _P, c_int, c_int, c_int, c_int, c_int, _P, c_int, _P, _P, _P, _P, _P,
+                                                   _P, _P, _P, _P, _P, _P, _P, c_int, c_int, _P, _P, c_int, _P, _P]),
     "spcl_conv16_bwd_fused_supported": (c_int, [c_int, c_int, c_int, c_int, c_int, c_int]),
     "spcl_conv16_bwd_fused_splits": (c_int, [c_int, c_int, c_int]),
     "spcl_conv16_bwd_fused": (c_int, [_P, c_int, c_int, c_int, c_int, _P, _P, _P, _P, _P, _P, _P, _P, _P, c_int, c_int,
@@ -299,13 +302,14 @@
                 ("nblk_co", c_int), ("CIB", c_int), ("COB", c_int), ("Cin", c_int), ("Cout", c_int)]
 
 
-ABI_VERSION = 24
+ABI_VERSION = 25
 WGRAD_BATCH_MAX = 16
 WGRAD_TAILS_MAX = 16
 _NO_STATUS = ("spcl_abi_version", "spcl_block1_recompute_supported", "spcl_block1_kernels_take", "spcl_conv16_bwd_fused_image_supported", "spcl_conv3x3_forward_image_acorr_rows", "spcl_image_autocorr_rows", "spcl_conv_dgrad_bnstats_image_supported", "spcl_conv16_bwd_fused_supported", "spcl_conv16_bwd_fused_splits", "spcl_conv_num_tiles", "spcl_conv_stat_rows", "spcl_conv_set_gemm", "spcl_conv_set_f32_split", "spcl_conv_get_f32_split", "spcl_supcon_unit_gradient_block", "spcl_conv_cat_supported", "spcl_conv_up2_supported", "spcl_conv_split_supported", "spcl_conv_split_bnstats_supported", "spcl_conv1x1_bwd_rows", "spcl_profile_count", "spcl_conv_dgrad_bnstats_supported", "spcl_conv_dgrad_poolstats_supported",
               "spcl_conv_wgrad_batched_supported", "spcl_conv_bn_acc_supported", "spcl_conv_dgrad_bnstats_acc_supported",
               "spcl_conv_dgrad_poolstats_acc_supported", "spcl_supcon_rows_supported", "spcl_bnrelu_gap_supported",
-              "spcl_conv_dgrad_poolmax_supported", "spcl_conv_dgrad_poolmax_acc_supported")
+              "spcl_conv_dgrad_poolmax_supported", "spcl_conv_dgrad_poolmax_acc_supported",
+              "spcl_conv16_bwd_fused_image_pooled_supported")
 
 
 class NativeLibraryError(RuntimeError):
```
